# ZhenlongYuan/TSAR-MVS

Measured on AMD Instinct MI355X. Metric: depthmap Mpixels/sec (ETH3D full-res, 8 iters), higher is better.
Workload: dtype f32

## Files before the change

include/tsar.h:

```cpp
#ifndef TSAR_H_
#define TSAR_H_

#include <stddef.h>
#include <stdint.h>

#ifdef __cplusplus
extern "C" {
#endif

#define TSAR_MAX_VIEWS 64
#define TSAR_MAXCOST 2.0f

#define TSAR_OK 0
#define TSAR_ERR_INVALID (-1)
#define TSAR_ERR_HIP (-2)
#define TSAR_ERR_STATE (-3)
#define TSAR_ERR_NOMEM (-4)

#define TSAR_MEM_HOST 0
#define TSAR_MEM_DEVICE 1

#define TSAR_COMB_ALL 0
#define TSAR_COMB_BEST_N 1
#define TSAR_COMB_ANGLE 2
#define TSAR_COMB_GOOD 3

#define TSAR_FLAG_FIX_DOWN_FAR_SEED  (1u << 0)
#define TSAR_FLAG_FIX_RIGHT_FAR_CMP  (1u << 1)
#define TSAR_FLAG_STRICT_DIV         (1u << 2)
#define TSAR_FLAG_NO_LINE_CLOSING    (1u << 4)

#define TSAR_FLAG_TEX_FILTER_8BIT    (1u << 5)

#define TSAR_FLAG_FIX_INIT_RADIUS     (1u << 6)

typedef struct tsar_ctx tsar_ctx;

typedef struct tsar_camera {
    float K[9];
    float R[9];
    float t[3];
} tsar_camera;

typedef struct tsar_params {
    int32_t box_hsize;
    int32_t box_vsize;
    int32_t n_best;
    int32_t cost_comb;
    float depth_min;
    float depth_max;
    float cam_scale;
    uint32_t flags;
    uint64_t seed;
} tsar_params;

typedef struct tsar_slic_settings {
    int32_t spixel_size;
    int32_t no_iters;
    float coh_weight;
    int32_t do_enforce_connectivity;
    int32_t color_space;
} tsar_slic_settings;

typedef struct tsar_kernel_timing {
    char name[48];
    int32_t launches;
    float total_ms;
} tsar_kernel_timing;

int tsar_create(int device, tsar_ctx** out);
int tsar_destroy(tsar_ctx* ctx);
const char* tsar_last_error(const tsar_ctx* ctx);
const char* tsar_version(void);
int tsar_get_stream(tsar_ctx* ctx, void** stream_out);
int tsar_synchronize(tsar_ctx* ctx);

void tsar_default_params(tsar_params* p);
int tsar_set_params(tsar_ctx* ctx, const tsar_params* p);
int tsar_set_views(tsar_ctx* ctx, int n_views, int w, int h, const float* const* gray, int mem,
                   const tsar_camera* cams);
int tsar_set_views_u8(tsar_ctx* ctx, int n_views, int w, int h, const uint8_t* const* gray, int mem,
                      const tsar_camera* cams);
int tsar_set_view_subset(tsar_ctx* ctx, int n, const int32_t* view_idx);

int tsar_pm_init(tsar_ctx* ctx);
int tsar_pm_iterate(tsar_ctx* ctx, int iters);
int tsar_pm_iterate_final(tsar_ctx* ctx, int iters, const float* text, int mem);
int tsar_pm_cost_planes(tsar_ctx* ctx, const float* planes, int mem, float* cost_out,
                        int32_t* beview_out, float* ratio_out);
int tsar_set_plane(tsar_ctx* ctx, const float* planes, const float* cost, int mem);
int tsar_pm_sweep(tsar_ctx* ctx, int colour, int do_prop, int do_refine);
int tsar_set_sweep_counter(tsar_ctx* ctx, int n);
int tsar_get_plane(tsar_ctx* ctx, float* planes, float* cost, int32_t* beview, float* ratio, int mem);

int tsar_load_planes(tsar_ctx* ctx, const float* depth, const float* normal_world, int mem);
int tsar_compute_disp(tsar_ctx* ctx);
int tsar_compute_disp_final(tsar_ctx* ctx, const float* resize_planes, const float* text, int mem);
int tsar_depth_to_plane(tsar_ctx* ctx);

int tsar_pyramid_views(tsar_ctx* coarse, const tsar_ctx* fine);
int tsar_upsample_planes(tsar_ctx* fine, const tsar_ctx* coarse);
int tsar_compute_disp_final_upsampled(tsar_ctx* ctx, const float* text, int mem);
int tsar_get_view_image(tsar_ctx* ctx, int view, float* out, int mem);

int tsar_set_geom_depths(tsar_ctx* ctx, int n_views, const float* const* depth, int mem, float weight, float clip);
int tsar_clear_geom(tsar_ctx* ctx);
int tsar_pm_rescore(tsar_ctx* ctx);
int tsar_get_geom_matrices(tsar_ctx* ctx, int view, float* forward, float* back);

int tsar_geom_pyramid(tsar_ctx* coarse, const tsar_ctx* fine);
int tsar_pyramid_planes(tsar_ctx* coarse, const tsar_ctx* fine);
int tsar_upsample_merge(tsar_ctx* fine, const tsar_ctx* coarse);

int tsar_get_result(tsar_ctx* ctx, float* depth, float* normal_world, float* cost, float* confid,
                    int mem);

int tsar_set_reliable_mask(tsar_ctx* ctx, const float* scale, int mem);
int tsar_get_reliable_mask(tsar_ctx* ctx, float* scale, int mem);
int tsar_lrdiff(tsar_ctx* ctx);
int tsar_getview(tsar_ctx* ctx);
int tsar_wmf(tsar_ctx* ctx, int iters, int final_pass);
int tsar_set_regions(tsar_ctx* ctx, const int32_t* labels, int n_regions, const float* region_text,
                     const float* region_size, int mem);
int tsar_detect_weak_texture(tsar_ctx* ctx, int32_t* labels_out, int mem, int* n_regions_out, float* text_out,
                             float* size_out, int cap);
int tsar_ransac_regions(tsar_ctx* ctx, float* region_planes_out, float* inlier_ratio_out);
int tsar_set_region_planes(tsar_ctx* ctx, const float* region_planes);
int tsar_fake_depth(tsar_ctx* ctx, float* fakedepth_out, int mem);
int tsar_fill_textureless(tsar_ctx* ctx);

void tsar_default_slic_settings(tsar_slic_settings* s);
int tsar_slic(tsar_ctx* ctx, const uint8_t* bgra, int w, int h, const tsar_slic_settings* s,
              int32_t* labels_out, int mem);

typedef struct tsar_fusion_params {
    int32_t num_consistent;
    float reproj_error;
    float depth_diff;
    float angle_deg;
    int32_t used_list;
} tsar_fusion_params;
void tsar_default_fusion_params(tsar_fusion_params* p);
int tsar_fuse_ctx(tsar_ctx* ctx, int n_views, int w, int h, const tsar_camera* cams, const float* const* depth,
                  const float* const* normal_world, const float* const* gray, int mem, const int32_t* src_off,
                  const int32_t* src_idx, const tsar_fusion_params* params, float* points_out, int64_t cap,
                  int64_t* n_points_out);
int tsar_fuse(int device, int n_views, int w, int h, const tsar_camera* cams, const float* const* depth,
              const float* const* normal_world, const float* const* gray, int mem, const int32_t* src_off,
              const int32_t* src_idx, const tsar_fusion_params* params, float* points_out, int64_t cap,
              int64_t* n_points_out);

void* tsar_host_alloc(size_t bytes);
void tsar_host_free(void* p);

void* tsar_device_alloc(int device, size_t bytes);
void tsar_device_free(int device, void* p);
int tsar_device_write(int device, void* dst, const void* host_src, size_t bytes);
int tsar_peer_copy(int dst_device, void* dst, int src_device, const void* src, size_t bytes);

int tsar_enable_kernel_timing(tsar_ctx* ctx, int enable);
int tsar_reset_kernel_timing(tsar_ctx* ctx);
int tsar_get_kernel_timing(tsar_ctx* ctx, tsar_kernel_timing* out, int cap, int* n_out);

int tsar_selftest_sqrt(tsar_ctx* ctx, int mode, uint64_t seed, uint64_t* mismatches_out);
int tsar_selftest_divide(tsar_ctx* ctx, const float* X, const float* Y, const float* Z, size_t n, float* u_out, float* v_out, int ieee);
int tsar_selftest_divide_random(tsar_ctx* ctx, int log2_triples, uint64_t seed, int mode, int guarded, uint64_t* mismatches_out,
                                uint64_t* outside_guard_out);
int tsar_selftest_sweep_census(tsar_ctx* ctx, int colour, uint64_t* out8);
int tsar_selftest_sweep_repeat(tsar_ctx* ctx, int colour, void* memo_dev, uint64_t* out8);
int tsar_selftest_slic_stage(tsar_ctx* ctx, int stage, int w, int h, int mw, int mh, const tsar_slic_settings* s, const void* in0,
                             const void* in1, void* inout);

#ifdef __cplusplus
}
#endif
#endif
```

tsar-mvs_amd/api.py:

```python
from __future__ import annotations

import ctypes as C
import os

import numpy as np

_HERE = os.path.dirname(os.path.abspath(__file__))
LIB_PATH = os.environ.get("TSAR_LIB") or os.path.join(_HERE, "libtsar_hip.so")

TSAR_OK = 0
TSAR_ERR_INVALID, TSAR_ERR_HIP, TSAR_ERR_STATE, TSAR_ERR_NOMEM = -1, -2, -3, -4
MEM_HOST, MEM_DEVICE = 0, 1
COMB_ALL, COMB_BEST_N, COMB_ANGLE, COMB_GOOD = 0, 1, 2, 3
FLAG_FIX_DOWN_FAR_SEED, FLAG_FIX_RIGHT_FAR_CMP, FLAG_STRICT_DIV = 1, 2, 4
FLAG_NO_LINE_CLOSING = 16
FLAG_TEX_FILTER_8BIT = 32
FLAG_FIX_INIT_RADIUS = 64
MAXCOST = 2.0
MAX_VIEWS = 64


class TsarError(RuntimeError):
    def __init__(self, code, msg):
        super().__init__(f"tsar error {code}: {msg}")
        self.code = code


class Camera(C.Structure):
    _fields_ = [("K", C.c_float * 9), ("R", C.c_float * 9), ("t", C.c_float * 3)]


class Params(C.Structure):
    _fields_ = [("box_hsize", C.c_int32), ("box_vsize", C.c_int32), ("n_best", C.c_int32), ("cost_comb", C.c_int32),
                ("depth_min", C.c_float), ("depth_max", C.c_float), ("cam_scale", C.c_float), ("flags", C.c_uint32),
                ("seed", C.c_uint64)]


class SlicSettings(C.Structure):
    _fields_ = [("spixel_size", C.c_int32), ("no_iters", C.c_int32), ("coh_weight", C.c_float),
                ("do_enforce_connectivity", C.c_int32), ("color_space", C.c_int32)]


class FusionParams(C.Structure):
    _fields_ = [("num_consistent", C.c_int32), ("reproj_error", C.c_float), ("depth_diff", C.c_float), ("angle_deg", C.c_float),
                ("used_list", C.c_int32)]


class KernelTiming(C.Structure):
    _fields_ = [("name", C.c_char * 48), ("launches", C.c_int32), ("total_ms", C.c_float)]


SPIXEL_DTYPE = np.dtype([("center", np.float32, 2), ("color", np.float32, 4), ("id", np.int32), ("n", np.int32)])

ABI_SYMBOLS = [
    "tsar_create", "tsar_destroy", "tsar_last_error", "tsar_version", "tsar_get_stream", "tsar_synchronize",
    "tsar_default_params", "tsar_set_params", "tsar_set_views", "tsar_set_views_u8", "tsar_set_view_subset",
    "tsar_pm_init", "tsar_pm_iterate", "tsar_pm_iterate_final", "tsar_pm_sweep", "tsar_set_sweep_counter", "tsar_pm_cost_planes", "tsar_set_plane", "tsar_get_plane",
    "tsar_load_planes", "tsar_compute_disp", "tsar_compute_disp_final", "tsar_depth_to_plane", "tsar_get_result",
    "tsar_pyramid_views", "tsar_upsample_planes", "tsar_compute_disp_final_upsampled", "tsar_get_view_image",
    "tsar_set_geom_depths", "tsar_clear_geom", "tsar_pm_rescore", "tsar_get_geom_matrices",
    "tsar_geom_pyramid", "tsar_pyramid_planes", "tsar_upsample_merge",
    "tsar_set_reliable_mask", "tsar_get_reliable_mask", "tsar_lrdiff", "tsar_getview", "tsar_wmf", "tsar_set_regions", "tsar_detect_weak_texture", "tsar_ransac_regions",
    "tsar_set_region_planes", "tsar_fake_depth", "tsar_fill_textureless",
    "tsar_default_slic_settings", "tsar_slic", "tsar_default_fusion_params", "tsar_fuse", "tsar_fuse_ctx",
    "tsar_host_alloc", "tsar_host_free", "tsar_device_alloc", "tsar_device_free", "tsar_device_write", "tsar_peer_copy", "tsar_enable_kernel_timing", "tsar_reset_kernel_timing", "tsar_get_kernel_timing",
    "tsar_selftest_divide", "tsar_selftest_divide_random", "tsar_selftest_sqrt", "tsar_selftest_sweep_census", "tsar_selftest_sweep_repeat", "tsar_selftest_slic_stage",
]

_lib = None


def load_library(path: str = LIB_PATH):
    global _lib
    if _lib is not None:
        return _lib
    if not os.path.exists(path):
        raise ImportError(f"{path} not found: build it with `make -C tsar-mvs_amd/csrc` "
                          "(or __graft_entry__.build()); there is no CPU fallback")
    L = C.CDLL(path)
    L.tsar_last_error.restype = C.c_char_p
    L.tsar_last_error.argtypes = [C.c_void_p]
    L.tsar_version.restype = C.c_char_p
    L.tsar_create.argtypes = [C.c_int, C.POINTER(C.c_void_p)]
    L.tsar_destroy.argtypes = [C.c_void_p]
    L.tsar_default_params.restype = None
    L.tsar_default_params.argtypes = [C.POINTER(Params)]
    L.tsar_default_slic_settings.restype = None
    L.tsar_default_slic_settings.argtypes = [C.POINTER(SlicSettings)]
    L.tsar_set_params.argtypes = [C.c_void_p, C.POINTER(Params)]
    L.tsar_set_views.argtypes = [C.c_void_p, C.c_int, C.c_int, C.c_int, C.POINTER(C.c_void_p), C.c_int, C.POINTER(Camera)]
    L.tsar_set_views_u8.argtypes = L.tsar_set_views.argtypes
    L.tsar_set_view_subset.argtypes = [C.c_void_p, C.c_int, C.c_void_p]
    L.tsar_pm_init.argtypes = [C.c_void_p]
    L.tsar_pm_iterate.argtypes = [C.c_void_p, C.c_int]
    L.tsar_pm_iterate_final.argtypes = [C.c_void_p, C.c_int, C.c_void_p, C.c_int]
    L.tsar_pm_sweep.argtypes = [C.c_void_p, C.c_int, C.c_int, C.c_int]
    L.tsar_set_sweep_counter.argtypes = [C.c_void_p, C.c_int]
    L.tsar_pm_cost_planes.argtypes = [C.c_void_p, C.c_void_p, C.c_int, C.c_void_p, C.c_void_p, C.c_void_p]
    L.tsar_set_plane.argtypes = [C.c_void_p, C.c_void_p, C.c_void_p, C.c_int]
    L.tsar_get_plane.argtypes = [C.c_void_p, C.c_void_p, C.c_void_p, C.c_void_p, C.c_void_p, C.c_int]
    L.tsar_load_planes.argtypes = [C.c_void_p, C.c_void_p, C.c_void_p, C.c_int]
    L.tsar_compute_disp.argtypes = [C.c_void_p]
    L.tsar_compute_disp_final.argtypes = [C.c_void_p, C.c_void_p, C.c_void_p, C.c_int]
    L.tsar_depth_to_plane.argtypes = [C.c_void_p]
    L.tsar_pyramid_views.argtypes = [C.c_void_p, C.c_void_p]
    L.tsar_upsample_planes.argtypes = [C.c_void_p, C.c_void_p]
    L.tsar_compute_disp_final_upsampled.argtypes = [C.c_void_p, C.c_void_p, C.c_int]
    L.tsar_get_view_image.argtypes = [C.c_void_p, C.c_int, C.c_void_p, C.c_int]
    L.tsar_set_geom_depths.argtypes = [C.c_void_p, C.c_int, C.POINTER(C.c_void_p), C.c_int, C.c_float, C.c_float]
    L.tsar_clear_geom.argtypes = [C.c_void_p]
    L.tsar_pm_rescore.argtypes = [C.c_void_p]
    L.tsar_get_geom_matrices.argtypes = [C.c_void_p, C.c_int, C.c_void_p, C.c_void_p]
    L.tsar_geom_pyramid.argtypes = [C.c_void_p, C.c_void_p]
    L.tsar_pyramid_planes.argtypes = [C.c_void_p, C.c_void_p]
    L.tsar_upsample_merge.argtypes = [C.c_void_p, C.c_void_p]
    L.tsar_get_result.argtypes = [C.c_void_p, C.c_void_p, C.c_void_p, C.c_void_p, C.c_void_p, C.c_int]
    L.tsar_set_reliable_mask.argtypes = [C.c_void_p, C.c_void_p, C.c_int]
    L.tsar_get_reliable_mask.argtypes = [C.c_void_p, C.c_void_p, C.c_int]
    L.tsar_host_alloc.restype = C.c_void_p
    L.tsar_host_alloc.argtypes = [C.c_size_t]
    L.tsar_host_free.restype = None
    L.tsar_host_free.argtypes = [C.c_void_p]
    L.tsar_device_alloc.restype = C.c_void_p
    L.tsar_device_alloc.argtypes = [C.c_int, C.c_size_t]
    L.tsar_device_free.restype = None
    L.tsar_device_free.argtypes = [C.c_int, C.c_void_p]
    L.tsar_device_write.argtypes = [C.c_int, C.c_void_p, C.c_void_p, C.c_size_t]
    L.tsar_peer_copy.argtypes = [C.c_int, C.c_void_p, C.c_int, C.c_void_p, C.c_size_t]
    L.tsar_lrdiff.argtypes = [C.c_void_p]
    L.tsar_getview.argtypes = [C.c_void_p]
    L.tsar_wmf.argtypes = [C.c_void_p, C.c_int, C.c_int]
    L.tsar_set_regions.argtypes = [C.c_void_p, C.c_void_p, C.c_int, C.c_void_p, C.c_void_p, C.c_int]
    L.tsar_detect_weak_texture.argtypes = [C.c_void_p, C.c_void_p, C.c_int, C.POINTER(C.c_int), C.c_void_p, C.c_void_p, C.c_int]
    L.tsar_ransac_regions.argtypes = [C.c_void_p, C.c_void_p, C.c_void_p]
    L.tsar_set_region_planes.argtypes = [C.c_void_p, C.c_void_p]
    L.tsar_fake_depth.argtypes = [C.c_void_p, C.c_void_p, C.c_int]
    L.tsar_fill_textureless.argtypes = [C.c_void_p]
    L.tsar_slic.argtypes = [C.c_void_p, C.c_void_p, C.c_int, C.c_int, C.POINTER(SlicSettings), C.c_void_p, C.c_int]
    L.tsar_default_fusion_params.restype = None
    L.tsar_default_fusion_params.argtypes = [C.POINTER(FusionParams)]
    L.tsar_fuse.argtypes = [C.c_int, C.c_int, C.c_int, C.c_int, C.POINTER(Camera), C.POINTER(C.c_void_p), C.POINTER(C.c_void_p), C.POINTER(C.c_void_p), C.c_int,
                            C.c_void_p, C.c_void_p, C.POINTER(FusionParams), C.c_void_p, C.c_int64, C.POINTER(C.c_int64)]
    L.tsar_fuse_ctx.argtypes = [C.c_void_p] + list(L.tsar_fuse.argtypes[1:])
    L.tsar_get_stream.argtypes = [C.c_void_p, C.POINTER(C.c_void_p)]
    L.tsar_synchronize.argtypes = [C.c_void_p]
    L.tsar_enable_kernel_timing.argtypes = [C.c_void_p, C.c_int]
    L.tsar_reset_kernel_timing.argtypes = [C.c_void_p]
    L.tsar_get_kernel_timing.argtypes = [C.c_void_p, C.POINTER(KernelTiming), C.c_int, C.POINTER(C.c_int)]
    L.tsar_selftest_divide.argtypes = [C.c_void_p, C.c_void_p, C.c_void_p, C.c_void_p, C.c_size_t, C.c_void_p, C.c_void_p, C.c_int]
    L.tsar_selftest_sweep_census.argtypes = [C.c_void_p, C.c_int, C.POINTER(C.c_uint64)]
    L.tsar_selftest_sweep_repeat.argtypes = [C.c_void_p, C.c_int, C.c_void_p, C.POINTER(C.c_uint64)]
    L.tsar_selftest_sqrt.argtypes = [C.c_void_p, C.c_int, C.c_uint64, C.POINTER(C.c_uint64)]
    L.tsar_selftest_divide_random.argtypes = [C.c_void_p, C.c_int, C.c_uint64, C.c_int, C.c_int, C.POINTER(C.c_uint64), C.POINTER(C.c_uint64)]
    L.tsar_selftest_slic_stage.argtypes = [C.c_void_p, C.c_int, C.c_int, C.c_int, C.c_int, C.c_int, C.POINTER(SlicSettings), C.c_void_p, C.c_void_p, C.c_void_p]
    _lib = L
    return L


def default_params(**kw) -> Params:
    p = Params()
    load_library().tsar_default_params(C.byref(p))
    for k, v in kw.items():
        setattr(p, k, v)
    return p


def _is_torch(a) -> bool:
    return type(a).__module__.startswith("torch")


def _ptr(a):
    if a is None:
        return None, MEM_HOST
    if _is_torch(a):
        assert a.is_contiguous(), "tensor must be contiguous"
        if a.is_cuda:
            import torch
            torch.cuda.current_stream(a.device).synchronize()
        return C.c_void_p(a.data_ptr()), (MEM_DEVICE if a.is_cuda else MEM_HOST)
    assert a.flags["C_CONTIGUOUS"], "array must be C-contiguous"
    return a.ctypes.data_as(C.c_void_p), MEM_HOST


class Matcher:

    def __init__(self, device: int = 0):
        self.L = load_library()
        self._ctx = C.c_void_p()
        rc = self.L.tsar_create(device, C.byref(self._ctx))
        if rc != TSAR_OK:
            raise TsarError(rc, "tsar_create failed (is a HIP device visible?)")
        self.w = self.h = self.n_views = 0
        self.device = device
        self._keep = []

    def close(self):
        if self._ctx:
            self.L.tsar_destroy(self._ctx)
            self._ctx = C.c_void_p()

    def __del__(self):
        try:
            self.close()
        except Exception:
            pass

    def _chk(self, rc):
        if rc != TSAR_OK:
            raise TsarError(rc, self.L.tsar_last_error(self._ctx).decode())

    def set_params(self, params: Params):
        self._chk(self.L.tsar_set_params(self._ctx, C.byref(params)))
        self.params = params

    def set_views(self, images, K, R, t, u8: bool = False):
        n = len(images)
        first = images[0]
        h, w = int(first.shape[0]), int(first.shape[1])
        ptrs = (C.c_void_p * n)()
        kinds = set()
        for i, im in enumerate(images):
            assert tuple(im.shape) == (h, w)
            if not _is_torch(im):
                im = np.ascontiguousarray(im, dtype=np.uint8 if u8 else np.float32)
                self._keep.append(im)
            elif u8:
                assert str(im.dtype) == "torch.uint8" and im.is_contiguous()
            p, kind = _ptr(im)
            ptrs[i] = p
            kinds.add(kind)
        assert len(kinds) == 1, "all images must live in the same memory space"
        cams = (Camera * n)()
        K = np.asarray(K, np.float32).reshape(n, 9)
        R = np.asarray(R, np.float32).reshape(n, 9)
        t = np.asarray(t, np.float32).reshape(n, 3)
        for i in range(n):
            cams[i].K[:] = K[i].tolist()
            cams[i].R[:] = R[i].tolist()
            cams[i].t[:] = t[i].tolist()
        self._chk((self.L.tsar_set_views_u8 if u8 else self.L.tsar_set_views)(self._ctx, n, w, h, ptrs, kinds.pop(), cams))
        self._keep.clear()
        self.w, self.h, self.n_views = w, h, n

    def set_view_subset(self, idx):
        a = np.ascontiguousarray(idx, np.int32)
        self._chk(self.L.tsar_set_view_subset(self._ctx, len(a), a.ctypes.data_as(C.c_void_p)))

    def pm_init(self):
        self._chk(self.L.tsar_pm_init(self._ctx))

    def pm_iterate(self, iters: int):
        self._chk(self.L.tsar_pm_iterate(self._ctx, iters))

    def pm_iterate_final(self, iters: int, text):
        t = text if _is_torch(text) else np.ascontiguousarray(text, np.float32)
        p, kind = _ptr(t)
        self._chk(self.L.tsar_pm_iterate_final(self._ctx, iters, p, kind))

    def pm_sweep(self, colour: int, do_prop: bool = True, do_refine: bool = True):
        self._chk(self.L.tsar_pm_sweep(self._ctx, colour, int(do_prop), int(do_refine)))

    def set_sweep_counter(self, n: int):
        self._chk(self.L.tsar_set_sweep_counter(self._ctx, n))

    def pm_cost_planes(self, planes):
        planes = np.ascontiguousarray(planes, np.float32)
        cost = np.empty((self.h, self.w), np.float32)
        bv = np.empty((self.h, self.w), np.int32)
        rt = np.empty((self.h, self.w), np.float32)
        self._chk(self.L.tsar_pm_cost_planes(self._ctx, _ptr(planes)[0], MEM_HOST, _ptr(cost)[0], _ptr(bv)[0], _ptr(rt)[0]))
        return cost, bv, rt

    def set_plane(self, planes, cost):
        planes = np.ascontiguousarray(planes, np.float32)
        cost = np.ascontiguousarray(cost, np.float32)
        self._chk(self.L.tsar_set_plane(self._ctx, _ptr(planes)[0], _ptr(cost)[0], MEM_HOST))

    def get_plane(self):
        planes = np.empty((self.h, self.w, 4), np.float32)
        cost = np.empty((self.h, self.w), np.float32)
        bv = np.empty((self.h, self.w), np.int32)
        rt = np.empty((self.h, self.w), np.float32)
        self._chk(self.L.tsar_get_plane(self._ctx, _ptr(planes)[0], _ptr(cost)[0], _ptr(bv)[0], _ptr(rt)[0], MEM_HOST))
        return planes, cost, bv, rt

    def load_planes(self, depth, normal_world):
        d, kd = _ptr(depth if _is_torch(depth) else np.ascontiguousarray(depth, np.float32))
        depth_keep = depth if _is_torch(depth) else np.ascontiguousarray(depth, np.float32)
        normal_keep = normal_world if _is_torch(normal_world) else np.ascontiguousarray(normal_world, np.float32)
        d, kd = _ptr(depth_keep)
        n, kn = _ptr(normal_keep)
        assert kd == kn
        self._chk(self.L.tsar_load_planes(self._ctx, d, n, kd))

    def compute_disp(self):
        self._chk(self.L.tsar_compute_disp(self._ctx))

    def compute_disp_final(self, resize_planes, text):
        r = np.ascontiguousarray(resize_planes, np.float32)
        t = np.ascontiguousarray(text, np.float32)
        self._chk(self.L.tsar_compute_disp_final(self._ctx, _ptr(r)[0], _ptr(t)[0], MEM_HOST))

    def depth_to_plane(self):
        self._chk(self.L.tsar_depth_to_plane(self._ctx))

    def pyramid_from(self, fine: "Matcher"):
        self._chk(self.L.tsar_pyramid_views(self._ctx, fine._ctx))
        self.w, self.h, self.n_views = (fine.w + 1) // 2, (fine.h + 1) // 2, fine.n_views
        self.params = fine.params

    def upsample_planes(self, coarse: "Matcher"):
        self._chk(self.L.tsar_upsample_planes(self._ctx, coarse._ctx))

    def get_view_image(self, view: int):
        out = np.empty((self.h, self.w), np.float32)
        self._chk(self.L.tsar_get_view_image(self._ctx, view, _ptr(out)[0], MEM_HOST))
        return out

    def compute_disp_final_upsampled(self, text):
        t = text if _is_torch(text) else np.ascontiguousarray(text, np.float32)
        p, kind = _ptr(t)
        self._chk(self.L.tsar_compute_disp_final_upsampled(self._ctx, p, kind))

    def set_geom_depths(self, depths, weight: float = 0.2, clip: float = 3.0):
        n = len(depths)
        ptrs = (C.c_void_p * n)()
        keep, kinds = [], set()
        for v, d in enumerate(depths):
            if v == 0 or d is None:
                continue
            if not _is_torch(d):
                d = np.ascontiguousarray(d, np.float32)
            assert tuple(d.shape) == (self.h, self.w), "depth map %d has shape %s, the views are %dx%d" % (v, tuple(d.shape), self.w, self.h)
            keep.append(d)
            p, kind = _ptr(d)
            ptrs[v] = p
            kinds.add(kind)
        assert len(kinds) <= 1, "all depth maps must live in the same memory space"
        self._chk(self.L.tsar_set_geom_depths(self._ctx, n, ptrs, kinds.pop() if kinds else MEM_HOST, float(weight), float(clip)))

    def clear_geom(self):
        self._chk(self.L.tsar_clear_geom(self._ctx))

    def rescore(self):
        self._chk(self.L.tsar_pm_rescore(self._ctx))

    def get_geom_matrices(self, view: int):
        f = np.empty((3, 4), np.float32)
        b = np.empty((3, 4), np.float32)
        self._chk(self.L.tsar_get_geom_matrices(self._ctx, view, _ptr(f)[0], _ptr(b)[0]))
        return f, b

    def geom_pyramid_from(self, fine: "Matcher"):
        self._chk(self.L.tsar_geom_pyramid(self._ctx, fine._ctx))

    def pyramid_planes_from(self, fine: "Matcher"):
        self._chk(self.L.tsar_pyramid_planes(self._ctx, fine._ctx))

    def upsample_merge(self, coarse: "Matcher"):
        self._chk(self.L.tsar_upsample_merge(self._ctx, coarse._ctx))

    def get_result(self, want=("depth", "normal", "cost", "confid"), pinned=False, out=None):
        shapes = {"depth": (self.h, self.w), "normal": (self.h, self.w, 3), "cost": (self.h, self.w), "confid": (self.h, self.w)}
        empty = pinned_empty if pinned else np.empty
        res = {}
        for k in ("depth", "normal", "cost", "confid"):
            if out is not None and k in out:
                a = out[k]
                assert a.dtype == np.float32 and tuple(a.shape) == shapes[k] and a.flags["C_CONTIGUOUS"]
                res[k] = a
            elif out is None and k in want:
                res[k] = empty(shapes[k], np.float32)
        self._chk(self.L.tsar_get_result(self._ctx, _ptr(res.get("depth"))[0], _ptr(res.get("normal"))[0], _ptr(res.get("cost"))[0],
                                         _ptr(res.get("confid"))[0], MEM_HOST))
        return res

    def get_result_device(self, depth=None, normal=None, cost=None, confid=None):
        self._chk(self.L.tsar_get_result(self._ctx, _ptr(depth)[0], _ptr(normal)[0], _ptr(cost)[0], _ptr(confid)[0], MEM_DEVICE))

    def set_reliable_mask(self, scale):
        s = np.ascontiguousarray(scale, np.float32)
        self._chk(self.L.tsar_set_reliable_mask(self._ctx, _ptr(s)[0], MEM_HOST))

    def get_reliable_mask(self):
        s = np.empty((self.h, self.w), np.float32)
        self._chk(self.L.tsar_get_reliable_mask(self._ctx, _ptr(s)[0], MEM_HOST))
        return s

    def lrdiff(self):
        self._chk(self.L.tsar_lrdiff(self._ctx))

    def selftest_divide(self, X, Y, Z, ieee: bool = False, mode: int | None = None):
        X, Y, Z = (np.ascontiguousarray(a, dtype=np.float32) for a in (X, Y, Z))
        assert X.shape == Y.shape == Z.shape
        u, v = np.empty_like(X), np.empty_like(X)
        self._chk(self.L.tsar_selftest_divide(self._ctx, _ptr(X)[0], _ptr(Y)[0], _ptr(Z)[0], X.size, _ptr(u)[0], _ptr(v)[0], int(ieee) if mode is None else mode))
        return u, v

    def selftest_sqrt(self, mode: int, seed: int = 0) -> int:
        bad = C.c_uint64(0)
        self._chk(self.L.tsar_selftest_sqrt(self._ctx, mode, seed, C.byref(bad)))
        return bad.value

    def selftest_sweep_census(self, colour: int) -> dict:
        out = (C.c_uint64 * 8)()
        self._chk(self.L.tsar_selftest_sweep_census(self._ctx, colour, out))
        keys = ("waves", "arms_any_lane", "max_lane_survivors", "max_lane_survivors_nodup", "lane_survivors", "lane_survivors_nodup", "pixels", "arms_present")
        return dict(zip(keys, [int(v) for v in out]))

    def selftest_divide_random(self, log2_triples: int, seed: int, mode: int, guarded: bool = True):
        bad, out = C.c_uint64(0), C.c_uint64(0)
        self._chk(self.L.tsar_selftest_divide_random(self._ctx, log2_triples, seed, mode, int(guarded), C.byref(bad), C.byref(out)))
        return bad.value, out.value

    def _slic_stage(self, stage, w, h, mw, mh, settings, in0, in1, inout):
        p1 = _ptr(in1)[0] if in1 is not None else None
        self._chk(self.L.tsar_selftest_slic_stage(self._ctx, stage, w, h, mw, mh, C.byref(settings), _ptr(in0)[0], p1, _ptr(inout)[0]))
        return inout

    def slic_convert(self, bgra, color_space=0):
        img = np.ascontiguousarray(bgra, np.uint8).reshape(-1, 4)
        return self._slic_stage(0, img.shape[0], 1, 0, 0, SlicSettings(20, 0, 5.0, 0, color_space), img, None, np.zeros((img.shape[0], 4), np.float32))

    def slic_init_centers(self, lab, mw, mh, S):
        lab = np.ascontiguousarray(lab, np.float32)
        h, w = lab.shape[:2]
        return self._slic_stage(1, w, h, mw, mh, SlicSettings(S, 0, 5.0, 0, 0), lab, None, np.zeros(mw * mh, SPIXEL_DTYPE))

    def slic_find_association(self, lab, centres, mw, mh, S, weight, labels_before=None):
        lab = np.ascontiguousarray(lab, np.float32)
        h, w = lab.shape[:2]
        labels = np.zeros((h, w), np.int32) if labels_before is None else np.ascontiguousarray(labels_before, np.int32).copy()
        return self._slic_stage(2, w, h, mw, mh, SlicSettings(S, 0, weight, 0, 0), lab, np.ascontiguousarray(centres), labels)

    def slic_update_centers(self, lab, labels, S):
        lab = np.ascontiguousarray(lab, np.float32)
        h, w = lab.shape[:2]
        return self._slic_stage(3, w, h, w // S, h // S, SlicSettings(S, 0, 5.0, 0, 0), lab, np.ascontiguousarray(labels, np.int32), np.zeros((w // S) * (h // S), SPIXEL_DTYPE))

    def slic_connectivity(self, labels):
        labels = np.ascontiguousarray(labels, np.int32)
        h, w = labels.shape
        return self._slic_stage(4, w, h, 0, 0, SlicSettings(20, 0, 5.0, 0, 0), labels, None, np.zeros((h, w), np.int32))

    def getview(self):
        self._chk(self.L.tsar_getview(self._ctx))

    def wmf(self, iters: int, final_pass: bool):
        self._chk(self.L.tsar_wmf(self._ctx, iters, int(final_pass)))

    def set_regions(self, labels, region_text, region_size=None):
        tx = np.ascontiguousarray(region_text, np.float32)
        sz = np.ascontiguousarray(region_size, np.float32) if region_size is not None else None
        if _is_torch(labels) and labels.is_cuda:
            import torch
            assert labels.dtype == torch.int32
            txd = torch.from_numpy(tx).to(labels.device)
            szd = torch.from_numpy(sz).to(labels.device) if sz is not None else None
            self._chk(self.L.tsar_set_regions(self._ctx, _ptr(labels)[0], len(tx), _ptr(txd)[0], _ptr(szd)[0], MEM_DEVICE))
        else:
            lb = np.ascontiguousarray(labels, np.int32)
            self._chk(self.L.tsar_set_regions(self._ctx, _ptr(lb)[0], len(tx), _ptr(tx)[0], _ptr(sz)[0], MEM_HOST))
        self.n_regions = len(tx)

    def detect_weak_texture(self, cap: int = 1 << 16, want_labels: bool = True):
        labels = np.empty((self.h, self.w), np.int32) if want_labels else None
        text = np.empty(cap, np.float32)
        size = np.empty(cap, np.float32)
        n = C.c_int(0)
        self._chk(self.L.tsar_detect_weak_texture(self._ctx, _ptr(labels)[0] if want_labels else None, MEM_HOST, C.byref(n), _ptr(text)[0], _ptr(size)[0], cap))
        self.n_regions = n.value
        k = min(n.value, cap)
        return labels, text[:k].copy(), size[:k].copy()

    def ransac_regions(self):
        planes = np.empty((self.n_regions, 4), np.float32)
        ratio = np.empty((self.n_regions,), np.float32)
        self._chk(self.L.tsar_ransac_regions(self._ctx, _ptr(planes)[0], _ptr(ratio)[0]))
        return planes, ratio

    def set_region_planes(self, planes):
        pl = np.ascontiguousarray(planes, np.float32)
        self._chk(self.L.tsar_set_region_planes(self._ctx, _ptr(pl)[0]))

    def fake_depth(self):
        out = np.empty((self.h, self.w), np.float32)
        self._chk(self.L.tsar_fake_depth(self._ctx, _ptr(out)[0], MEM_HOST))
        return out

    def fill_textureless(self):
        self._chk(self.L.tsar_fill_textureless(self._ctx))

    def slic(self, bgra, settings: SlicSettings | None = None):
        img = np.ascontiguousarray(bgra, np.uint8)
        h, w = img.shape[:2]
        if settings is None:
            settings = SlicSettings()
            self.L.tsar_default_slic_settings(C.byref(settings))
        labels = np.empty((h, w), np.int32)
        self._chk(self.L.tsar_slic(self._ctx, _ptr(img)[0], w, h, C.byref(settings), _ptr(labels)[0], MEM_HOST))
        return labels

    @property
    def stream(self) -> int:
        s = C.c_void_p()
        self._chk(self.L.tsar_get_stream(self._ctx, C.byref(s)))
        return s.value or 0

    def synchronize(self):
        self._chk(self.L.tsar_synchronize(self._ctx))

    def enable_kernel_timing(self, on: bool = True):
        self._chk(self.L.tsar_enable_kernel_timing(self._ctx, int(on)))

    def reset_kernel_timing(self):
        self._chk(self.L.tsar_reset_kernel_timing(self._ctx))

    def kernel_timing(self):
        buf = (KernelTiming * 32)()
        n = C.c_int(0)
        self._chk(self.L.tsar_get_kernel_timing(self._ctx, buf, 32, C.byref(n)))
        return {buf[i].name.decode(): (buf[i].launches, buf[i].total_ms) for i in range(min(n.value, 32))}


def matcher_from_scene(scene, box=11, n_best=1, cost_comb=COMB_BEST_N, flags=0, seed=2024, device=0, subset=None, box_v=None) -> Matcher:
    m = Matcher(device)
    m.set_params(default_params(box_hsize=box, box_vsize=box if box_v is None else box_v, n_best=n_best, cost_comb=cost_comb, depth_min=scene.depth_min,
                                depth_max=scene.depth_max, flags=flags, seed=seed))
    m.set_views(scene.images, scene.K, scene.R, scene.t)
    if subset is not None:
        m.set_view_subset(subset)
    return m


def run_multiscale(matcher: Matcher, levels: int, coarse_iters: int, fine_iters: int, coarse=None):
    if levels < 0 or coarse_iters < 0 or fine_iters < 0:
        raise ValueError("levels and iteration counts must be >= 0")
    coarse = list(coarse or [])
    while len(coarse) < levels:
        coarse.append(Matcher(matcher.device))
    chain = [matcher] + coarse[:levels]
    for finer, coarser in zip(chain[:-1], chain[1:]):
        coarser.pyramid_from(finer)
    chain[-1].pm_init()
    chain[-1].pm_iterate(coarse_iters)
    for k in range(levels - 1, -1, -1):
        chain[k].upsample_planes(chain[k + 1])
        chain[k].pm_iterate(fine_iters)
    return coarse


def run_geom_pass(matcher: Matcher, own_depth, own_normal_world, src_depths, iters: int, weight: float = 0.2, clip: float = 3.0):
    if iters < 0:
        raise ValueError("iters must be >= 0")
    matcher.load_planes(own_depth, own_normal_world)
    matcher.set_geom_depths(src_depths, weight=weight, clip=clip)
    matcher.rescore()
    matcher.pm_iterate(iters)
    matcher.compute_disp()


def run_geom_pass_multiscale(matcher: Matcher, own_depth, own_normal_world, src_depths, levels: int, coarse_iters: int, fine_iters: int,
                             weight: float = 0.2, clip: float = 3.0, coarse=None):
    if levels < 0 or coarse_iters < 0 or fine_iters < 0:
        raise ValueError("levels and iteration counts must be >= 0")
    if levels == 0:
        run_geom_pass(matcher, own_depth, own_normal_world, src_depths, fine_iters, weight=weight, clip=clip)
        return list(coarse or [])
    coarse = list(coarse or [])
    while len(coarse) < levels:
        coarse.append(Matcher(matcher.device))
    chain = [matcher] + coarse[:levels]
    for m in chain:
        m.clear_geom()
    for finer, coarser in zip(chain[:-1], chain[1:]):
        coarser.pyramid_from(finer)
    matcher.load_planes(own_depth, own_normal_world)
    matcher.set_geom_depths(src_depths, weight=weight, clip=clip)
    for finer, coarser in zip(chain[:-1], chain[1:]):
        coarser.geom_pyramid_from(finer)
        coarser.pyramid_planes_from(finer)
    chain[-1].pm_iterate(coarse_iters)
    for k in range(levels - 1, -1, -1):
        chain[k].upsample_merge(chain[k + 1])
        chain[k].pm_iterate(fine_iters)
    matcher.compute_disp()
    return coarse


def fuse(depths, normals, grays, K, R, t, pairs, params: FusionParams | None = None, cap: int | None = None, device: int = 0, matcher=None):
    L = load_library()
    n = len(depths)
    h, w = int(depths[0].shape[0]), int(depths[0].shape[1])
    if params is None:
        params = FusionParams()
        L.tsar_default_fusion_params(C.byref(params))
    keep, kinds = [], set()

    def ptrs(seq, shape):
        arr = (C.c_void_p * n)()
        for i, a in enumerate(seq):
            if not _is_torch(a):
                a = np.ascontiguousarray(a, np.float32)
                keep.append(a)
            assert tuple(a.shape) == shape
            p, kind = _ptr(a)
            arr[i] = p
            kinds.add(kind)
        return arr
    pd, pn, pg = ptrs(depths, (h, w)), ptrs(normals, (h, w, 3)), ptrs(grays, (h, w))
    assert len(kinds) == 1
    cams = (Camera * n)()
    K = np.asarray(K, np.float32).reshape(n, 9); R = np.asarray(R, np.float32).reshape(n, 9); t = np.asarray(t, np.float32).reshape(n, 3)
    for i in range(n):
        cams[i].K[:] = K[i].tolist(); cams[i].R[:] = R[i].tolist(); cams[i].t[:] = t[i].tolist()
    lists = [list(pairs[v]) for v in range(n)]
    off = np.zeros(n + 1, np.int32)
    off[1:] = np.cumsum([len(x) for x in lists])
    idx = np.asarray([s for x in lists for s in x] or [0], np.int32)
    if cap is None:
        cap = n * h * w
    out = np.empty((cap, 9), np.float32)
    cnt = C.c_int64(0)
    tail = (n, w, h, cams, pd, pn, pg, kinds.pop(), off.ctypes.data_as(C.c_void_p), idx.ctypes.data_as(C.c_void_p), C.byref(params),
            out.ctypes.data_as(C.c_void_p), cap, C.byref(cnt))
    rc = L.tsar_fuse_ctx(matcher._ctx, *tail) if matcher is not None else L.tsar_fuse(device, *tail)
    if rc != TSAR_OK:
        raise TsarError(rc, L.tsar_last_error(matcher._ctx).decode() if matcher is not None else "tsar_fuse failed")
    return out[: min(cnt.value, cap)].copy()


def pinned_empty(shape, dtype=np.float32):
    import weakref
    L = load_library()
    dt = np.dtype(dtype)
    n = int(np.prod(shape)) * dt.itemsize
    p = L.tsar_host_alloc(n)
    if not p:
        raise MemoryError(f"tsar_host_alloc({n}) failed")
    buf = (C.c_char * n).from_address(p)
    weakref.finalize(buf, L.tsar_host_free, p)
    return np.frombuffer(buf, dtype=dt).reshape(shape)
```

tsar-mvs_amd/csrc/pm_core.h:

```cpp
#pragma once
#include <type_traits>

#include "tsar_device_math.h"

#define PM_BLOCK 256
#define PM_RW 32

typedef const uint32_t __attribute__((address_space(1)))* global_u32_ptr;
typedef const float __attribute__((address_space(1)))* global_f32_ptr;

template <bool QUAD, bool DIFF = false>
DEVFN float sample_bilinear(const DevView& vw, int w, int h, int qpitch, float u, float v, bool q8 = false) {
    u = fminf(fmaxf(u, -1.0f), (float)w);
    v = fminf(fmaxf(v, -1.0f), (float)h);
    const float fu = floorf(u), fv = floorf(v);
    float ax = u - fu, ay = v - fv;
    if (q8) { ax = rintf(ax * 256.0f) * 0.00390625f; ay = rintf(ay * 256.0f) * 0.00390625f; }
    const int iu = (int)fu, iv = (int)fv;
    float t00, t10, t01, t11;
    if (QUAD) {
        const uint32_t off = (uint32_t)(__mul24(iv + 1, qpitch) + iu + 1) * 4u;
        const uint32_t q = *(global_u32_ptr)((const char __attribute__((address_space(1)))*)vw.quad + off);
        t00 = (float)(q & 0xffu);
        t10 = (float)((q >> 8) & 0xffu);
        t01 = (float)((q >> 16) & 0xffu);
        t11 = (float)(q >> 24);
    } else {
        const int x0 = min(max(iu, 0), w - 1), x1 = min(max(iu + 1, 0), w - 1);
        const int y0 = min(max(iv, 0), h - 1), y1 = min(max(iv + 1, 0), h - 1);
        const global_f32_ptr r0 = (global_f32_ptr)vw.img + (size_t)y0 * w;
        const global_f32_ptr r1 = (global_f32_ptr)vw.img + (size_t)y1 * w;
        t00 = r0[x0]; t10 = r0[x1]; t01 = r1[x0]; t11 = r1[x1];
    }
    if (DIFF) {
        const float d1 = t10 - t00, d2 = t01 - t00, d3 = (t11 - t01) - d1;
        return fma_(ay, fma_(ax, d3, d2), fma_(ax, d1, t00));
    }
    const float top = fma_(ax, t10 - t00, t00);
    const float bot = fma_(ax, t11 - t01, t01);
    return fma_(ay, bot - top, top);
}

struct PixelRef {
    float inv_wsum;
    float mean_ref;
    float var_ref;
    bool textured;
};

template <bool QUAD> struct TileOf { typedef float type; };
template <> struct TileOf<true> { typedef unsigned short type; };
DEVFN float tile_value(float t) { return t; }
DEVFN float tile_value(unsigned short t) { return __uint_as_float((uint32_t)t << 16); }
DEVFN void tile_store(float* t, float v) { *t = v; }
DEVFN void tile_store(unsigned short* t, float v) { *t = (unsigned short)(__float_as_uint(v) >> 16); }
template <bool QUAD>
__host__ __device__ constexpr size_t tile_bytes(int tw, int th) {
    return ((size_t)tw * th * sizeof(typename TileOf<QUAD>::type) + 15) & ~(size_t)15;
}

template <int RH, typename TileT, int BLK = PM_BLOCK, int RW = PM_RW>
DEVFN void stage_ref_tile(const DevScene* __restrict__ sc, TileT* tile, int x0, int y0, int hr, int vr, int pad_rows = 0) {
    const int tw = RW + 2 * hr, th = RH + 2 * vr + pad_rows;
    const global_f32_ptr img = (global_f32_ptr)sc->view[0].img;
    const int w = sc->w, h = sc->h;
    for (int k = threadIdx.x; k < tw * th; k += BLK) {
        const int ty = k / tw, tx = k - ty * tw;
        const int gx = min(max(x0 + tx - hr, 0), w - 1), gy = min(max(y0 + ty - vr, 0), h - 1);
        tile_store(&tile[k], img[(size_t)gy * w + gx]);
    }
}

template <int HR, typename TileT, int BLK = PM_BLOCK>
DEVFN PixelRef hoist_reference(const TileT* tile, int tw, int own, float* wts, int hr_rt, int vr_rt) {
    const int hr = HR > 0 ? HR : hr_rt, vr = HR > 0 ? HR : vr_rt;
    const float cen = tile_value(tile[own]);
    float sum_ref = 0.f, sum_ref_ref = 0.f, wsum = 0.f;
    int tap = 0;
#pragma unroll
    for (int i = -hr; i <= hr; i += 2) {
#pragma unroll
        for (int j = -vr; j <= vr; j += 2) {
            const float r = tile_value(tile[own + j * tw + i]);
            const float sd = sqrtf((float)(i * i + j * j));
            const float cd = fabsf(r - cen);
            const float wt = tsar_expf(-sd / 50.0f - cd / 18.0f);
            wts[tap * BLK] = wt;
            const float wr = wt * r;
            sum_ref += wr;
            sum_ref_ref = fma_(wr, r, sum_ref_ref);
            wsum += wt;
            ++tap;
        }
    }
    PixelRef pr;
    pr.inv_wsum = 1.0f / wsum;
    sum_ref *= pr.inv_wsum;
    sum_ref_ref *= pr.inv_wsum;
    pr.mean_ref = sum_ref;
    pr.var_ref = sum_ref_ref - sum_ref * sum_ref;
    pr.textured = !(pr.var_ref < 1e-5f);
    return pr;
}

template <int HR, bool STRICT, bool QUAD, int BLK = PM_BLOCK>
DEVFN float view_cost_generic(const DevScene* __restrict__ sc, const DevView& vw, const typename TileOf<QUAD>::type* tile, int tw, int own, const float* wts,
                              const PixelRef& pr, int x, int y, const float4& n4) {
    const int hr = HR > 0 ? HR : sc->hrad, vr = HR > 0 ? HR : sc->vrad;
    const int w = sc->w, h = sc->h, qp = sc->quad_pitch;
    float H[9];
    if (STRICT) plane_homography(sc->ref, vw, n4, H, sc->k_sparse != 0);
    else plane_homography_fast(sc->ref, vw, n4, H);
    float sum_src = 0.f, sum_src_src = 0.f, sum_ref_src = 0.f;
    int tap = 0;
#pragma unroll 1
    for (int i = -hr; i <= hr; i += 2) {
        const float xi = (float)(x + i);
        const float bx = STRICT ? H[0] * xi : fma_(H[0], xi, H[2]), by = STRICT ? H[3] * xi : fma_(H[3], xi, H[5]), bz = STRICT ? H[6] * xi : fma_(H[6], xi, H[8]);
#pragma unroll
        for (int j = -vr; j <= vr; j += 2) {
            const float yj = (float)(y + j);
            float X = fma_(H[1], yj, bx), Y = fma_(H[4], yj, by), Z = fma_(H[7], yj, bz);
            if (STRICT) { X += H[2]; Y += H[5]; Z += H[8]; }
            float u, v;
            if (STRICT) {
                persp_divide_exact<true>(X, Y, Z, u, v);
            } else {
                const float rz = __builtin_amdgcn_rcpf(Z);
                u = X * rz;
                v = Y * rz;
            }
            const float s = sample_bilinear<QUAD, !STRICT>(vw, w, h, qp, u, v, (sc->flags & TSAR_FLAG_TEX_FILTER_8BIT) != 0);
            const float r = tile_value(tile[own + j * tw + i]);
            const float wt = wts[tap * BLK];
            const float ws = wt * s;
            sum_src += ws;
            sum_src_src = fma_(ws, s, sum_src_src);
            if (STRICT) sum_ref_src = fma_(wt * r, s, sum_ref_src);
            else sum_ref_src = fma_(ws, r, sum_ref_src);
            ++tap;
        }
    }
    sum_src *= pr.inv_wsum;
    sum_src_src *= pr.inv_wsum;
    sum_ref_src *= pr.inv_wsum;
    const float var_src = sum_src_src - sum_src * sum_src;
    if (var_src < 1e-5f) return TSAR_MAXCOST;
    const float covar = sum_ref_src - pr.mean_ref * sum_src;
    const float vrs = sqrtf(pr.var_ref * var_src);
    return fmaxf(0.0f, fminf(TSAR_MAXCOST, 1.0f - covar / vrs));
}

#include "pm_tap_r5.h"
#include "pm_core_lut.h"

DEVFN float geom_term(const DevScene* __restrict__ sc, const DevView& vw, int vi, int x, int y, float D) {
    const float* dm = sc->geom_depth[vi];
    if (dm == nullptr) return 0.0f;
    const int w = sc->w, h = sc->h;
    const float xf = (float)x, yf = (float)y;
    const float xd = xf * D, yd = yf * D;
    const float a = ((vw.A[0] * xd + vw.A[1] * yd) + vw.A[2] * D) + vw.b[0];
    const float b = ((vw.A[3] * xd + vw.A[4] * yd) + vw.A[5] * D) + vw.b[1];
    const float s = ((vw.A[6] * xd + vw.A[7] * yd) + vw.A[8] * D) + vw.b[2];
    float u, v;
    persp_divide_exact<true>(a, b, s, u, v);
    const float cf = floorf(u + 0.5f), rf = floorf(v + 0.5f);
    const bool inside = s > 0.0f && cf >= 0.0f && cf <= (float)(w - 1) && rf >= 0.0f && rf <= (float)(h - 1);
    float Dv = 0.0f;
    if (inside) Dv = ((global_f32_ptr)dm)[(int)rf * w + (int)cf];
    const float* M = sc->geom_back[vi];
    const float cd = cf * Dv, rd = rf * Dv;
    const float p0 = ((M[0] * cd + M[1] * rd) + M[2] * Dv) + M[3];
    const float p1 = ((M[4] * cd + M[5] * rd) + M[6] * Dv) + M[7];
    const float p2 = ((M[8] * cd + M[9] * rd) + M[10] * Dv) + M[11];
    float xq, yq;
    persp_divide_exact<true>(p0, p1, p2, xq, yq);
    const float dx = xq - xf, dy = yq - yf;
    const float e2 = dx * dx + dy * dy;
    const float tau = sc->geom_clip;
    const float r = sqrt_rsq_exact(fminf(fmaxf(e2, 0x1p-100f), 0x1p100f));
    float e = e2 < 0x1p-100f ? 0.0f : r;
    e = (inside && Dv > 0.0f && p2 > 0.0f && e2 < sc->geom_clip_sq) ? fminf(e, tau) : tau;
    return sc->geom_weight * e;
}

template <int NB, int HR, bool STRICT, bool QUAD, int V = 0, int BLK = PM_BLOCK>
DEVFN float multiview_cost(const DevScene* __restrict__ sc, const typename TileOf<QUAD>::type* tile, int tw, int own, const float* wts, const PixelRef& pr,
                           int x, int y, const float4& n4, int& beview, float& ratio) {
    constexpr bool GEOM = (V & TSAR_V_GEOM) != 0;
    constexpr int VT = V & ~(TSAR_V_GEOM | TSAR_V_REDRAW);
    float best[NB];
#pragma unroll
    for (int k = 0; k < NB; k++) best[k] = __builtin_inff();
    const int num = sc->n_sel;
    int valid = 0, bv = -1;
    float cmin = __builtin_inff();
    float depth_h = 0.0f;
    if constexpr (GEOM) depth_h = plane_depth(sc->ref, n4, x, y);
    int vi_next = sc->sel[0];
    for (int i = 0; i < num; i++) {
        const int vi = vi_next;
        vi_next = sc->sel[i + 1 < num ? i + 1 : i];
        float c;
        if constexpr ((VT & 1024) != 0) c = view_cost_lut<STRICT, (VT >> 11) & 7, (VT & 131072) != 0 && !STRICT, (VT & 2097152) != 0 && !STRICT>(sc, sc->view[vi], tile, tw, own, wts, pr, x, y, n4);
        else if constexpr (QUAD && HR == 5 && r5_production_variant(VT))
            c = view_cost_r5<STRICT, (VT & 128) != 0 && !STRICT, (VT & 8) != 0, (VT & 131072) != 0, (VT & 2097152) != 0, BLK>(sc, sc->view[vi], tile, tw, own, wts, pr, x, y, n4);
#ifdef TSAR_EXPERIMENTS
        else if constexpr (QUAD && HR == 5 && r5_diag_variant(VT))
            c = view_cost_r5<false, true, true, true, true, BLK, (VT & 4194304) ? 1 : 2>(sc, sc->view[vi], tile, tw, own, wts, pr, x, y, n4);
#endif
        else {
            static_assert(VT == 0, "unknown tap-loop variant");
            c = view_cost_generic<HR, STRICT, QUAD, BLK>(sc, sc->view[vi], tile, tw, own, wts, pr, x, y, n4);
        }
        auto vmin = [](float a, float b) { float r; asm("v_min_f32 %0, %1, %2" : "=v"(r) : "v"(a), "v"(b)); return r; };
        auto vmax = [](float a, float b) { float r; asm("v_max_f32 %0, %1, %2" : "=v"(r) : "v"(a), "v"(b)); return r; };
        c = vmin(c, TSAR_MAXCOST);
        valid -= (int32_t)__float_as_uint(c - TSAR_MAXCOST) >> 31;
        if constexpr (GEOM) c = c + geom_term(sc, sc->view[vi], vi, x, y, depth_h);
        {
            const uint32_t worse = (uint32_t)((int32_t)__float_as_uint(cmin - c) >> 31);
            asm("v_bfi_b32 %0, %1, %2, %3" : "=v"(bv) : "v"(worse), "v"(bv), "s"(vi));
            cmin = vmin(cmin, c);
        }
        float v = c;
#pragma unroll
        for (int k = 0; k < NB; k++) {
            const float lo = vmin(best[k], v), hi = vmax(best[k], v);
            best[k] = lo;
            v = hi;
        }
    }
    int nb = valid;
    if (sc->cost_comb == TSAR_COMB_BEST_N) nb = min(nb, sc->n_best);
    if (nb <= 0) { beview = -1; ratio = 0.f; return TSAR_MAXCOST; }
    float cost = 0.f;
#pragma unroll
    for (int k = 0; k < NB; k++)
        if (k < nb) cost += best[k];
    cost = cost / (float)nb;
    ratio = num >= 2 ? best[0] / best[1] : 0.f;
    beview = bv;
    return cost;
}

DEVFN void strip_tile(int t, int tiles_x, int tiles_y, int sw, int& tx, int& ty) {
    if (sw <= 0) { ty = t / tiles_x; tx = t - ty * tiles_x; return; }
    const int per_strip = sw * tiles_y;
    const int strip = t / per_strip, within = t - strip * per_strip;
    const int width = min(sw, tiles_x - strip * sw);
    ty = within / width;
    tx = strip * sw + within - ty * width;
}

static inline int strip_width(int requested, int tiles_x) {
    if (requested >= 0) return requested;
    const int sw = (tiles_x + 7) / 8;
    return sw < 8 ? 8 : sw;
}

DEVFN int xcd_tile(int bid, int n) {
    const int chunk = n >> 3, rem = n & 7;
    const int xcd = bid & 7, slot = bid >> 3;
    return xcd * chunk + min(xcd, rem) + slot;
}
```

tsar-mvs_amd/csrc/pm_sweep_impl.h:

```cpp
#pragma once
#include "pm_core.h"

#define SWEEP_SMALL_IMAGE_TILES 3072

#define CAND_SAME (1 << 30)

DEVFN void select_candidates(const DevScene* __restrict__ sc, const float* __restrict__ c_same, const float* __restrict__ c_other,
                             int x, int y, int cand[8]) {
    const int col = sc->w, row = sc->h;
    const int p = y * col + x;
    const bool fix_seed = sc->flags & TSAR_FLAG_FIX_DOWN_FAR_SEED, fix_cmp = sc->flags & TSAR_FLAG_FIX_RIGHT_FAR_CMP;
    float cmin;
    int cp, cs;
#pragma unroll
    for (int k = 0; k < 8; k++) cand[k] = -1;
    if (y > 2) {
        cp = p - 3 * col; cmin = c_other[cp];
#pragma unroll
        for (int i = 1; i < 11; ++i)
            if (y > 2 + 2 * i) { const int q = p - (3 + 2 * i) * col; const float v = c_other[q]; if (v < cmin) { cmin = v; cp = q; } }
        cand[0] = cp;
    }
    if (y < row - 3) {
        cp = p + 3 * col;
        cmin = (fix_seed || y <= 2) ? c_other[cp] : c_other[p - 3 * col];
#pragma unroll
        for (int i = 1; i < 11; ++i)
            if (y < row - 3 - 2 * i) { const int q = p + (3 + 2 * i) * col; const float v = c_other[q]; if (v < cmin) { cmin = v; cp = q; } }
        cand[1] = cp;
    }
    if (x > 2) {
        cp = p - 3; cmin = c_other[cp];
#pragma unroll
        for (int i = 1; i < 11; ++i)
            if (x > 2 + 2 * i) { const int q = p - 3 - 2 * i; const float v = c_other[q]; if (v < cmin) { cmin = v; cp = q; } }
        cand[2] = cp;
    }
    if (x < col - 3) {
        cp = p + 3; cmin = c_other[cp];
#pragma unroll
        for (int i = 1; i < 11; ++i)
            if (x < col - 3 - 2 * i) {
                const int q = p + 3 + 2 * i;
                const float v = c_other[q];
                const bool take = fix_cmp ? (v < cmin) : (cmin < v);
                if (take) { cmin = v; cp = q; }
            }
        cand[3] = cp;
    }
    if (y > 0) {
        cp = p - col; cs = 0; cmin = c_other[cp];
#pragma unroll
        for (int i = 0; i < 3; ++i) {
            if (y > 1 + i && x > i) { const int q = p - (2 + i) * col - i; const float v = c_same[q]; if (v < cmin) { cmin = v; cp = q; cs = 1; } }
            if (y > 1 + i && x < col - 1 - i) { const int q = p - (2 + i) * col + i; const float v = c_same[q]; if (v < cmin) { cmin = v; cp = q; cs = 1; } }
        }
        cand[4] = cs ? (cp | CAND_SAME) : cp;
    }
    if (y < row - 1) {
        cp = p + col; cs = 0; cmin = c_other[cp];
#pragma unroll
        for (int i = 0; i < 3; ++i) {
            if (y < row - 2 - i && x > i) { const int q = p + (2 + i) * col - i; const float v = c_same[q]; if (v < cmin) { cmin = v; cp = q; cs = 1; } }
            if (y < row - 2 - i && x < col - 1 - i) { const int q = p + (2 + i) * col + i; const float v = c_same[q]; if (v < cmin) { cmin = v; cp = q; cs = 1; } }
        }
        cand[5] = cs ? (cp | CAND_SAME) : cp;
    }
    if (x > 0) {
        cp = p - 1; cs = 0; cmin = c_other[cp];
#pragma unroll
        for (int i = 0; i < 3; ++i) {
            if (x > 1 + i && y > i) { const int q = p - (2 + i) - i * col; const float v = c_same[q]; if (v < cmin) { cmin = v; cp = q; cs = 1; } }
            if (x > 1 + i && y < row - 1 - i) { const int q = p - (2 + i) + i * col; const float v = c_same[q]; if (v < cmin) { cmin = v; cp = q; cs = 1; } }
        }
        cand[6] = cs ? (cp | CAND_SAME) : cp;
    }
    if (x < col - 1) {
        cp = p + 1; cs = 0; cmin = c_other[cp];
#pragma unroll
        for (int i = 0; i < 3; ++i) {
            if (x < col - 2 - i && y > i) { const int q = p + (2 + i) - i * col; const float v = c_same[q]; if (v < cmin) { cmin = v; cp = q; cs = 1; } }
            if (x < col - 2 - i && y < row - 1 - i) { const int q = p + (2 + i) + i * col; const float v = c_same[q]; if (v < cmin) { cmin = v; cp = q; cs = 1; } }
        }
        cand[7] = cs ? (cp | CAND_SAME) : cp;
    }
}

DEVFN bool same_bits(const float4& a, const float4& b) {
    return __float_as_uint(a.x) == __float_as_uint(b.x) && __float_as_uint(a.y) == __float_as_uint(b.y) &&
           __float_as_uint(a.z) == __float_as_uint(b.z) && __float_as_uint(a.w) == __float_as_uint(b.w);
}

struct SweepMemo {
    int32_t* cand;
    uint32_t* seq;
    uint32_t* changed;
    uint32_t launch, valid_from;
    int mode;
    int slot_off;
};

template <int NB, int HR, bool STRICT, bool QUAD, int V = 0, int BLK = PM_BLOCK, bool CMP = false>
__global__ __launch_bounds__(BLK) void pm_sweep_kernel(const DevScene* __restrict__ sc, int colour,
                                                            const float* __restrict__ c_same, const float4* __restrict__ n_same,
                                                            const float* __restrict__ c_other, const float4* __restrict__ n_other,
                                                            float* c_out, float4* n_out, float* __restrict__ ratio_out,
                                                            int32_t* __restrict__ beview_out, uint32_t stream_id, int do_prop,
                                                            int do_refine, int tiles_x, int n_tiles, int cost_consistent, int strip_w,
                                                            const float* __restrict__ final_text, SweepMemo memo) {
    extern __shared__ __attribute__((aligned(16))) unsigned char lds_raw[];
    typedef typename TileOf<QUAD>::type TileT;
    constexpr int RW = PM_RW;
    constexpr int SWEEP_RH = 2 * BLK / RW;
    const int hr = HR > 0 ? HR : sc->hrad, vr = HR > 0 ? HR : sc->vrad;
    const int tw = RW + 2 * hr, th = SWEEP_RH + 2 * vr;
    constexpr bool LUTW = (V & 1024) != 0;
    const size_t lut_bytes = LUTW ? (size_t)(sc->lut_classes + 1) * 1024 : 0;
    TileT* tile = (TileT*)(lds_raw + lut_bytes);
    float* const wts_base = LUTW ? (float*)lds_raw : (float*)(lds_raw + tile_bytes<QUAD>(tw, th));
    float* wts = LUTW ? wts_base : wts_base + threadIdx.x;
    if constexpr (LUTW) build_weight_lut<BLK>(sc, wts);

    const int t = xcd_tile(blockIdx.x, n_tiles);
    int tix, tiy;
    strip_tile(t, tiles_x, n_tiles / tiles_x, strip_w, tix, tiy);
    const int ty0 = tiy * SWEEP_RH, tx0 = tix * RW;
    stage_ref_tile<SWEEP_RH, TileT, BLK, RW>(sc, tile, tx0, ty0, hr, vr, LUTW ? LUT_TILE_PAD_ROWS : 0);
    __syncthreads();

    const int ly = threadIdx.x >> 4, k = threadIdx.x & 15;
    const int y = ty0 + ly;
    const int lx = 2 * k + ((colour + y) & 1);
    const int x = tx0 + lx;
    const int w = sc->w, h = sc->h;
    bool mine = x < w && y < h;
    if (!CMP && !mine) return;
    const int p = mine ? y * w + x : 0;
    const int own = (ly + vr) * tw + lx + hr;

    float cost_now = TSAR_MAXCOST;
    float4 n_now = {0.f, 0.f, 0.f, 0.f};
    if (mine) { cost_now = c_same[p]; n_now = n_same[p]; }
    if (mine && final_text && final_text[p] == -1.0f) {
        c_out[p] = cost_now; n_out[p] = n_now;
        if (!CMP) return;
        mine = false;
    }
    PixelRef pr;
    pr.inv_wsum = 0.f; pr.mean_ref = 0.f; pr.var_ref = 0.f; pr.textured = false;
    if (mine) {
        if constexpr (LUTW) pr = hoist_reference_lut(sc, tile, tw, own, wts);
        else pr = hoist_reference<HR, TileT, BLK>(tile, tw, own, wts, hr, vr);
    }
    bool wrote = false;
    float ratio_w = 0.f;
    int beview_w = 0;
    const DevRef& rf = sc->ref;
    const bool work = mine && pr.textured;
    int cand[8] = {-1, -1, -1, -1, -1, -1, -1, -1};
    if (work && do_prop) {
        select_candidates(sc, c_same, c_other, x, y, cand);
        if (memo.mode) {
            const uint32_t m_seq = memo.seq[p];
            const bool have = m_seq >= memo.valid_from && cost_consistent;
            const int4* mc = (const int4*)(memo.cand + (size_t)p * 8);
            int prev[8];
            if (have) {
                const int4 a0 = mc[0], a1 = mc[1];
                prev[0] = a0.x; prev[1] = a0.y; prev[2] = a0.z; prev[3] = a0.w; prev[4] = a1.x; prev[5] = a1.y; prev[6] = a1.z; prev[7] = a1.w;
            }
            int4 w0, w1;
            w0.x = cand[0]; w0.y = cand[1]; w0.z = cand[2]; w0.w = cand[3]; w1.x = cand[4]; w1.y = cand[5]; w1.z = cand[6]; w1.w = cand[7];
            ((int4*)(memo.cand + (size_t)p * 8))[0] = w0;
            ((int4*)(memo.cand + (size_t)p * 8))[1] = w1;
            memo.seq[p] = memo.launch;
            if (have) {
#pragma unroll
                for (int a = 0; a < 8; a++)
                    if (cand[a] >= 0 && cand[a] == prev[a] && memo.changed[cand[a] & 0x3fffffff] < m_seq) cand[a] = -1;
            }
        }
    }
    float depth_now = 0.f;
    float vv[3] = {0.f, 0.f, 0.f};
    if (work) { depth_now = plane_depth(rf, n_now, x, y); view_vector(rf, x, y, vv); }
    const float4 n_first = n_now;
    float deltaN = 1.0f;
    float deltaZ = sc->max_disp / 2.0f;
    const float fb = rf.f * rf.baseline;
    const int n_ref = do_refine ? sc->refine_steps : 0;

    if constexpr (!CMP) {
        if (work) {
            const int h_end = 8 + n_ref;
#pragma unroll 1
            for (int h = do_prop ? 0 : 8; h < h_end; h++) {
                float4 n_t;
                float depth_t;
                if (h < 8) {
                    int ci = cand[0];
#pragma unroll
                    for (int a = 1; a < 8; a++) ci = (h == a) ? cand[a] : ci;
                    if (ci < 0) continue;
                    const int idx = ci & 0x3fffffff;
                    n_t = (ci >> 30) ? n_same[idx] : n_other[idx];
                    if (cost_consistent && (same_bits(n_t, n_now) || same_bits(n_t, n_first))) continue;
                    depth_t = plane_depth(rf, n_t, x, y);
                    if (!(depth_t >= rf.depthMin && depth_t <= rf.depthMax)) continue;
                } else {
                    const Rand4 rn = philox_uniform4((uint32_t)p, stream_id, (uint32_t)(h - 8), sc->seed_lo, sc->seed_hi);
                    const float disp = fb / depth_now;
                    const float minDelta = -fminf(deltaZ, sc->min_disp + disp);
                    const float maxDelta = fminf(deltaZ, sc->max_disp - disp);
                    const float dz = between(rn.u[0], minDelta, maxDelta);
                    const float dispOut = fminf(fmaxf(disp + dz, sc->min_disp), sc->max_disp);
                    depth_t = fb / dispOut;
                    float nt[3];
                    nt[0] = n_now.x + between(rn.u[1], -deltaN, deltaN);
                    nt[1] = n_now.y + between(rn.u[2], -deltaN, deltaN);
                    nt[2] = n_now.z + between(rn.u[3], -deltaN, deltaN);
                    const float inv = 1.0f / sqrtf(dot3(nt, nt));
                    nt[0] *= inv; nt[1] *= inv; nt[2] *= inv;
                    if (dot3(nt, vv) > 0.0f) { nt[0] = -nt[0]; nt[1] = -nt[1]; nt[2] = -nt[2]; }
                    n_t.x = nt[0]; n_t.y = nt[1]; n_t.z = nt[2];
                    n_t.w = plane_offset(rf, nt, x, y, depth_t);
                    deltaN = deltaN / 4.0f;
                    deltaZ = deltaZ / 10.0f;
                }
                int bv; float rt;
                const float cost_t = multiview_cost<NB, HR, STRICT, QUAD, V, BLK>(sc, tile, tw, own, wts, pr, x, y, n_t, bv, rt);
                if (cost_t < cost_now) {
                    cost_now = cost_t; n_now = n_t; depth_now = depth_t;
                    ratio_w = rt; beview_w = bv; wrote = true;
                }
            }
        }
    } else {
        const int lane = threadIdx.x & 63, wave0 = threadIdx.x & ~63;
        volatile int32_t* slot_ci = (volatile int32_t*)(lds_raw + memo.slot_off) + wave0;
        volatile unsigned short* slot_src = (volatile unsigned short*)(lds_raw + memo.slot_off + 4 * BLK) + wave0;
        auto pixel_of = [&](int tid, int& px, int& py, int& pown) {
            const int sly = tid >> 4, sk = tid & 15;
            py = ty0 + sly;
            const int slx = 2 * sk + ((colour + py) & 1);
            px = tx0 + slx;
            pown = (sly + vr) * tw + slx + hr;
        };
        auto my_tid = []() { int t = threadIdx.x; asm volatile("" : "+v"(t)); return t; };
        uint32_t fresh = 0;
        if (work && do_prop) {
#pragma unroll
            for (int a = 0; a < 8; a++)
                if (cand[a] >= 0) fresh |= 1u << a;
        }
        if (!work) fresh = 0;
        uint32_t flags = fresh | (work ? 256u : 0u) | (mine ? 512u : 0u);
        int total = 0;
#pragma unroll
        for (int a = 0; a < 8; a++) total += __popcll(__ballot((flags >> a) & 1u));
        const int trips = (total + 63) >> 6;
        auto arms_of_trip = [&](int lo, auto&& f) {
            asm volatile("" : "+v"(flags));
            int b0 = 0;
#pragma unroll
            for (int a = 0; a < 8; a++) {
                const uint64_t bal = __ballot((flags >> a) & 1u);
                const int n = __popcll(bal);
                if (b0 + n > lo && b0 < lo + 64) {
                    const int j = b0 + (int)__builtin_amdgcn_mbcnt_hi((uint32_t)(bal >> 32), __builtin_amdgcn_mbcnt_lo((uint32_t)bal, 0u)) - lo;
                    f(a, j, ((flags >> a) & 1u) && j >= 0 && j < 64);
                }
                b0 += n;
            }
        };
        int acc_arm = -1;
        const float start_dz = sc->max_disp / 2.0f;
#pragma unroll 1
        for (int it = 0; it < trips + n_ref; it++) {
            float4 n_t = {0.f, 0.f, 0.f, 0.f};
            float depth_t = 0.f;
            int ex, ey, eown, etid = my_tid();
            PixelRef epr = pr;
            bool go;
            const int lo = it << 6;
            if (it < trips) {
                {
                    int mx, my, mown;
                    pixel_of(my_tid(), mx, my, mown);
                    const int32_t* mc = memo.cand + (size_t)(my * w + mx) * 8;
                    arms_of_trip(lo, [&](int a, int j, bool has) {
                        if (has) { slot_ci[j] = mc[a]; slot_src[j] = (unsigned short)(lane | (a << 6)); }
                    });
                }
                __builtin_amdgcn_wave_barrier();
                go = lane < total - lo;
                int src = 0, ci = 0;
                if (go) { src = slot_src[lane]; ci = slot_ci[lane]; }
                __builtin_amdgcn_wave_barrier();
                const int s = src & 63;
                epr.inv_wsum = __int_as_float(__builtin_amdgcn_ds_bpermute(s << 2, __float_as_int(pr.inv_wsum)));
                epr.mean_ref = __int_as_float(__builtin_amdgcn_ds_bpermute(s << 2, __float_as_int(pr.mean_ref)));
                epr.var_ref = __int_as_float(__builtin_amdgcn_ds_bpermute(s << 2, __float_as_int(pr.var_ref)));
                if (go) {
                    const int idx = ci & 0x3fffffff;
                    n_t = (ci >> 30) ? n_same[idx] : n_other[idx];
                    etid = wave0 + s;
                }
                pixel_of(etid, ex, ey, eown);
                if (go) {
                    const float d = plane_depth(rf, n_t, ex, ey);
                    go = d >= rf.depthMin && d <= rf.depthMax;
                }
            } else {
                pixel_of(etid, ex, ey, eown);
                if (it == trips && acc_arm >= 0) {
                    const int ci = memo.cand[(size_t)(ey * w + ex) * 8 + acc_arm];
                    const int idx = ci & 0x3fffffff;
                    n_now = (ci >> 30) ? n_same[idx] : n_other[idx];
                    depth_now = plane_depth(rf, n_now, ex, ey);
                    acc_arm = -1;
                }
                go = (flags >> 8) & 1u;
                if (go) {
                    const int step = it - trips;
                    float dN = 1.0f, dZ = start_dz;
                    for (int q = 0; q < step; q++) { dN = dN / 4.0f; dZ = dZ / 10.0f; }
                    float ev[3];
                    view_vector(rf, ex, ey, ev);
                    const Rand4 rn = philox_uniform4((uint32_t)(ey * w + ex), stream_id, (uint32_t)step, sc->seed_lo, sc->seed_hi);
                    const float disp = fb / depth_now;
                    const float minDelta = -fminf(dZ, sc->min_disp + disp);
                    const float maxDelta = fminf(dZ, sc->max_disp - disp);
                    const float dz = between(rn.u[0], minDelta, maxDelta);
                    const float dispOut = fminf(fmaxf(disp + dz, sc->min_disp), sc->max_disp);
                    depth_t = fb / dispOut;
                    float nt[3];
                    nt[0] = n_now.x + between(rn.u[1], -dN, dN);
                    nt[1] = n_now.y + between(rn.u[2], -dN, dN);
                    nt[2] = n_now.z + between(rn.u[3], -dN, dN);
                    const float inv = 1.0f / sqrtf(dot3(nt, nt));
                    nt[0] *= inv; nt[1] *= inv; nt[2] *= inv;
                    if (dot3(nt, ev) > 0.0f) { nt[0] = -nt[0]; nt[1] = -nt[1]; nt[2] = -nt[2]; }
                    n_t.x = nt[0]; n_t.y = nt[1]; n_t.z = nt[2];
                    n_t.w = plane_offset(rf, nt, ex, ey, depth_t);
                }
            }
            const float* ewts = LUTW ? wts_base : wts_base + etid;
            int bv = -1;
            float rt = 0.f, cost_t = TSAR_MAXCOST;
            if (go) cost_t = multiview_cost<NB, HR, STRICT, QUAD, V, BLK>(sc, tile, tw, eown, ewts, epr, ex, ey, n_t, bv, rt);
            if (it < trips) {
                arms_of_trip(lo, [&](int a, int j, bool has) {
                    const float c = __int_as_float(__builtin_amdgcn_ds_bpermute((j & 63) << 2, __float_as_int(cost_t)));
                    const float r = __int_as_float(__builtin_amdgcn_ds_bpermute((j & 63) << 2, __float_as_int(rt)));
                    const int b = __builtin_amdgcn_ds_bpermute((j & 63) << 2, bv);
                    if (has && c < cost_now) {
                        cost_now = c; acc_arm = a;
                        ratio_w = r; beview_w = b;
                    }
                });
            } else if (go && cost_t < cost_now) {
                cost_now = cost_t; n_now = n_t; depth_now = depth_t;
                ratio_w = rt; beview_w = bv;
            }
        }
        {
            int mx, my, mown;
            pixel_of(my_tid(), mx, my, mown);
            if (!((flags >> 9) & 1u)) return;
            const int pp = my * w + mx;
            if (acc_arm >= 0) {
                const int ci = memo.cand[(size_t)pp * 8 + acc_arm];
                const int idx = ci & 0x3fffffff;
                n_now = (ci >> 30) ? n_same[idx] : n_other[idx];
            }
            const bool changed = cost_now < c_same[pp];
            c_out[pp] = cost_now;
            n_out[pp] = n_now;
            if (changed && !final_text) { ratio_out[pp] = ratio_w; beview_out[pp] = beview_w; }
            if (changed && memo.mode) memo.changed[pp] = memo.launch;
            return;
        }
    }
    c_out[p] = cost_now;
    n_out[p] = n_now;
    if (wrote && !final_text) { ratio_out[p] = ratio_w; beview_out[p] = beview_w; }
    if (wrote && memo.mode) memo.changed[p] = memo.launch;
}


template <int HR, bool QUAD, int V>
constexpr bool sweep_has_packed_form() { return QUAD && ((HR == 5 && r5_production_variant(V & ~TSAR_V_GEOM)) || (V & 1024) != 0); }

template <int NB, int HR, bool STRICT, bool QUAD, int V = 0, int BLK = PM_BLOCK>
static int launch_sweep_t(tsar_ctx* ctx, int colour, const PlaneBuf& same_in, const PlaneBuf& other, const PlaneBuf& same_out,
                          uint32_t stream_id, int do_prop, int do_refine) {
    const DevScene& hs = ctx->hscene;
    constexpr int RW = PM_RW;
    constexpr int SWEEP_RH = 2 * BLK / RW;
    const int tiles_x = (hs.w + RW - 1) / RW, tiles_y = (hs.h + SWEEP_RH - 1) / SWEEP_RH;
    const int n_tiles = tiles_x * tiles_y;
#ifdef TSAR_EXPERIMENTS
    const size_t lds_pad = ctx->lds_pad;
#else
    constexpr size_t lds_pad = 0;
#endif
    size_t lds = tile_bytes<QUAD>(RW + 2 * hs.hrad, SWEEP_RH + 2 * hs.vrad + ((V & 1024) ? LUT_TILE_PAD_ROWS : 0)) + lds_pad +
                 ((V & 1024) ? (size_t)(hs.lut_classes + 1) * 1024 : sizeof(float) * (size_t)(hs.hrad + 1) * (hs.vrad + 1) * BLK);
    SweepMemo memo;
    memo.cand = ctx->memo_cand; memo.seq = ctx->memo_seq; memo.changed = ctx->changed_seq;
    memo.launch = ctx->launch_seq; memo.valid_from = ctx->memo_valid_from;
    memo.mode = (ctx->memo_mode && ctx->memo_cand && ctx->cost_consistent && !ctx->final_text) ? 1 : 0;
    memo.slot_off = 0;
    bool packed = false;
    if constexpr (sweep_has_packed_form<HR, QUAD, V>())
        packed = memo.mode && do_prop && ctx->compact_from >= 0 && ctx->call_launch >= ctx->compact_from;
    auto kern = pm_sweep_kernel<NB, HR, STRICT, QUAD, V, BLK, false>;
    if constexpr (sweep_has_packed_form<HR, QUAD, V>()) {
        if (packed) {
            kern = pm_sweep_kernel<NB, HR, STRICT, QUAD, V, BLK, true>;
            memo.slot_off = (int)lds;
            lds += 6 * (size_t)BLK;
        }
    }
    if (lds > 64 * 1024) TSAR_HIP_TRY(ctx, hipFuncSetAttribute((const void*)kern, hipFuncAttributeMaxDynamicSharedMemorySize, (int)lds));
    {
        ScopedKernelTimer tm(ctx, (V & TSAR_V_GEOM) ? "pm_sweep_geom" : "pm_sweep");
        ScopedKernelTimer tm_packed(ctx, packed ? "pm_sweep_packed" : nullptr);
        hipLaunchKernelGGL(kern, dim3(n_tiles), dim3(BLK), lds, ctx->stream, ctx->dscene, colour, same_in.c, same_in.n4, other.c,
                           other.n4, same_out.c, same_out.n4, ctx->ratio, ctx->beview, stream_id, do_prop, do_refine, tiles_x, n_tiles,
                           ctx->cost_consistent ? 1 : 0, strip_width(ctx->strip_w, tiles_x), ctx->final_text, memo);
    }
    TSAR_HIP_TRY(ctx, hipGetLastError());
    return TSAR_OK;
}

template <int NB, int HR, bool STRICT, bool QUAD, int V = 0, int BLK = PM_BLOCK>
static int launch_sweep_g(tsar_ctx* ctx, int colour, const PlaneBuf& same_in, const PlaneBuf& other, const PlaneBuf& same_out,
                          uint32_t stream_id, int do_prop, int do_refine) {
    if (ctx->hscene.geom_on) return launch_sweep_t<NB, HR, STRICT, QUAD, V | TSAR_V_GEOM, BLK>(ctx, colour, same_in, other, same_out, stream_id, do_prop, do_refine);
    return launch_sweep_t<NB, HR, STRICT, QUAD, V, BLK>(ctx, colour, same_in, other, same_out, stream_id, do_prop, do_refine);
}
```

tsar-mvs_amd/csrc/pm_tap_r5.h:

```cpp
#pragma once

template <bool STRICT, bool ROW, bool D16, bool BUF, bool MIX, int BLK, int DIAG = 0>
DEVFN float view_cost_r5(const DevScene* __restrict__ sc, const DevView& vw, const unsigned short* tile, int tw, int own, const float* wts,
                         const PixelRef& pr, int x, int y, const float4& n4) {
    static_assert(!(STRICT && ROW), "the row-wise walk changes the summation order: fast mode only");
    static_assert(!MIX || (BUF && !STRICT), "the half-float difference texture serves the fast arithmetic's blend through buffer loads");
    const int w = sc->w, h = sc->h, qp = sc->quad_pitch;
    const int qorg = (qp + 1) << 2;
    float H[9];
    if (STRICT) plane_homography(sc->ref, vw, n4, H, sc->k_sparse != 0);
    else plane_homography_fast(sc->ref, vw, n4, H);
    float sum_src = 0.f, sum_src_src = 0.f, sum_ref_src = 0.f;
    bool need_clamp;
    if (!STRICT) {
        const float xc = (float)x, yc = (float)y;
        const float Xc = fma_(H[1], yc, fma_(H[0], xc, H[2])), Yc = fma_(H[4], yc, fma_(H[3], xc, H[5])), Zc = fma_(H[7], yc, fma_(H[6], xc, H[8]));
        const float a = fabsf(H[0]) + fabsf(H[1]), b = fabsf(H[3]) + fabsf(H[4]), c = fabsf(H[6]) + fabsf(H[7]);
        const float Zmin = fma_(-5.0f, c, Zc);
        const float r = __builtin_amdgcn_rcpf(Zmin * Zc);
        const float r5 = 5.0f * r, rc = Zmin * r;
        const float du = fma_(a, Zc, fabsf(Xc) * c) * r5, dv = fma_(b, Zc, fabsf(Yc) * c) * r5;
        const float uc = Xc * rc, vc = Yc * rc;
        const bool inside = Zmin > 0.0f && fminf(uc - du, vc - dv) >= 1.5f && uc + du <= (float)(w - 1) - 1.5f && vc + dv <= (float)(h - 1) - 1.5f;
        need_clamp = !__all(inside);
    } else {
        bool inside = true;
        float zmin = __builtin_inff(), zmax = 0.0f;
#pragma unroll
        for (int c = 0; c < 4; c++) {
            const float xi = (float)(x + ((c & 1) ? 5 : -5)), yj = (float)(y + ((c & 2) ? 5 : -5));
            const float X = fma_(H[1], yj, fma_(H[0], xi, H[2])), Y = fma_(H[4], yj, fma_(H[3], xi, H[5])), Z = fma_(H[7], yj, fma_(H[6], xi, H[8]));
            const float rz = __builtin_amdgcn_rcpf(Z);
            const float u = X * rz, v = Y * rz;
            inside = inside && Z > 0.0f && u >= 1.0f && u <= (float)(w - 1) - 1.0f && v >= 1.0f && v <= (float)(h - 1) - 1.0f;
            if (STRICT) { zmin = fminf(zmin, Z); zmax = fmaxf(zmax, Z); }
        }
        if (STRICT) {
            const float cm = (float)(max(w, h) + 32);
            const float sz = fma_(fabsf(H[6]) + fabsf(H[7]), cm, fabsf(H[8]));
            const float sx = fma_(fabsf(H[0]) + fabsf(H[1]), cm, fabsf(H[2]));
            const float sy = fma_(fabsf(H[3]) + fabsf(H[4]), cm, fabsf(H[5]));
            inside = inside && zmin >= 3.814697265625e-06f && zmax <= 131072.0f && sz * cm <= 524288.0f * zmin && fmaxf(sx, sy) <= 262144.0f * zmin;
        }
        need_clamp = !__all(inside);
    }
    uint32_t qb_lo = 0, qb_hi = 0;
    if (!BUF) {
        const uint64_t qa = (uint64_t)(uintptr_t)vw.quad + (uint32_t)qorg;
        qb_lo = __builtin_amdgcn_readfirstlane((uint32_t)qa);
        qb_hi = __builtin_amdgcn_readfirstlane((uint32_t)(qa >> 32));
        asm volatile("" : "+s"(qb_lo), "+s"(qb_hi));
    }
    typedef uint32_t u32x4s __attribute__((ext_vector_type(4)));
    u32x4s rsrc = {0u, 0u, 0u, 0u};
    if (BUF) {
        if (MIX) {
            const uint64_t da = (uint64_t)(uintptr_t)vw.dquad + 2 * (uint64_t)(uint32_t)qorg;
            rsrc.x = __builtin_amdgcn_readfirstlane((uint32_t)da);
            rsrc.y = __builtin_amdgcn_readfirstlane(((uint32_t)(da >> 32) & 0xffffu) | (8u << 16));
        } else {
        const uint64_t qa = (uint64_t)(uintptr_t)vw.quad + (uint32_t)qorg;
        rsrc.x = __builtin_amdgcn_readfirstlane((uint32_t)qa);
        rsrc.y = __builtin_amdgcn_readfirstlane(((uint32_t)(qa >> 32) & 0xffffu) | (4u << 16));
        }
        rsrc.z = __builtin_amdgcn_readfirstlane((uint32_t)(qp * (h + 1) - 1));
        rsrc.w = 0x00020000u;
        asm volatile("" : "+s"(rsrc));
    }
    typedef float f32x2 __attribute__((ext_vector_type(2)));
    auto line6 = [&](int i, auto clamp_tag, auto unr_tag) {
        constexpr bool CLAMP = decltype(clamp_tag)::value;
        constexpr bool UNR = decltype(unr_tag)::value;
        static_assert(!UNR || (ROW && D16), "the unrolled form is written for the row-wise walk with D16 window loads");
        const float xi = (float)((ROW ? y : x) + i);
        const float bx = STRICT ? H[0] * xi : fma_(H[ROW ? 1 : 0], xi, H[2]), by = STRICT ? H[3] * xi : fma_(H[ROW ? 4 : 3], xi, H[5]),
                    bz = STRICT ? H[6] * xi : fma_(H[ROW ? 7 : 6], xi, H[8]);
        const int line = (i + 5) >> 1;
        float rcol[6];
        f32x2 wcol[3];
        {
            constexpr int U = BLK / 64, S = ROW ? 6 : 1;
            const uint32_t wa = (uint32_t)(uintptr_t)(const __attribute__((address_space(3))) float*)(wts + (UNR ? 0 : (ROW ? line : 6 * line) * BLK));
#pragma unroll
            for (int k = 0; k < 3; k++)
                asm("ds_read2st64_b32 %0, %1 offset0:%2 offset1:%3" : "=v"(wcol[k]) : "v"(wa), "n"(2 * U * S * k + (UNR ? U * line : 0)), "n"(2 * U * S * k + U * S + (UNR ? U * line : 0)), "v"(bz));
        }
        if (D16) {
            const uint32_t a0 = (uint32_t)(uintptr_t)(const __attribute__((address_space(3))) unsigned short*)(UNR ? tile + own - 5 * tw - 5 : ROW ? tile + own + i * tw - 5 : tile + own + i - 5 * tw);
#pragma unroll
            for (int jj = 0; jj < 6; jj++)
                asm("ds_read_u16_d16_hi %0, %1 offset:%2" : "=v"(rcol[jj]) : "v"(a0), "n"((ROW ? jj * 4 : jj * 2 * (PM_RW + 10) * 2) + (UNR ? line * 2 * (PM_RW + 10) * 2 : 0)), "v"(bz));
        }
        float ax[6], ay[6];
        uint32_t q[6];
        uint64_t q2[6];
        __builtin_amdgcn_s_setprio(3);
#pragma unroll
        for (int jj = 0; jj < 6; jj++) {
            const float yj = (float)((ROW ? x : y) + 2 * jj - 5);
            float X = fma_(H[ROW ? 0 : 1], yj, bx), Y = fma_(H[ROW ? 3 : 4], yj, by), Z = fma_(H[ROW ? 6 : 7], yj, bz);
            if (STRICT) { X += H[2]; Y += H[5]; Z += H[8]; }
            float u, v;
            const float uhi = (float)(w - 1), vhi = (float)(h - 1);
            if (STRICT) {
                persp_divide_exact<CLAMP>(X, Y, Z, u, v);
                if (CLAMP) {
                    u = fminf(fmaxf(u, 0.0f), uhi);
                    v = fminf(fmaxf(v, 0.0f), vhi);
                }
            } else {
                const float rz = __builtin_amdgcn_rcpf(Z);
                u = X * rz;
                v = Y * rz;
                if (CLAMP) {
                    u = __builtin_amdgcn_fmed3f(u, 0.0f, uhi);
                    v = __builtin_amdgcn_fmed3f(v, 0.0f, vhi);
                }
            }
            int iu, iv;
            ax[jj] = __builtin_amdgcn_fractf(u);
            ay[jj] = __builtin_amdgcn_fractf(v);
            asm("v_cvt_flr_i32_f32 %0, %1" : "=v"(iu) : "v"(u));
            asm("v_cvt_flr_i32_f32 %0, %1" : "=v"(iv) : "v"(v));
            int lin;
            asm("v_mad_i32_i24 %0, %1, %2, %3" : "=v"(lin) : "v"(iv), "s"(qp), "v"(iu));
            if (MIX && DIAG == 1) {
                q2[jj] = ((uint64_t)(uint32_t)~lin << 32) | (uint32_t)lin;
            } else if (MIX && DIAG == 2) {
                uint32_t la;
                asm("v_bfe_u32 %0, %1, 0, 12" : "=v"(la) : "v"(lin));
                asm volatile("ds_read_b64 %0, %1" : "=v"(q2[jj]) : "v"(la << 3));
            } else if (MIX) {
                asm volatile("buffer_load_dwordx2 %0, %1, %2, 0 idxen" : "=v"(q2[jj]) : "v"(lin), "s"(rsrc));
            } else if (BUF) {
                asm volatile("buffer_load_dword %0, %1, %2, 0 idxen" : "=v"(q[jj]) : "v"(lin), "s"(rsrc));
            } else {
                const uint32_t off2 = (uint32_t)lin << 2;
                q[jj] = *(global_u32_ptr)((const char __attribute__((address_space(1)))*)(uintptr_t)(((uint64_t)qb_hi << 32) | qb_lo) + off2);
            }
        }
        __builtin_amdgcn_sched_barrier(0);
        __builtin_amdgcn_s_setprio(0);
        __builtin_amdgcn_sched_barrier(0);
#pragma unroll
        for (int jj = 0; jj < 6; jj++) {
            float t00, t10, t01, t11;
            if (MIX && DIAG == 1) {
            } else if (MIX && DIAG == 2) {
                if (jj == 0) asm("s_waitcnt lgkmcnt(5)" : "+v"(q2[0]), "+v"(rcol[0]), "+v"(rcol[1]), "+v"(rcol[2]), "+v"(rcol[3]), "+v"(rcol[4]), "+v"(rcol[5]),
                                 "+v"(wcol[0]), "+v"(wcol[1]), "+v"(wcol[2]) : "v"(q2[5]));
                else asm("s_waitcnt lgkmcnt(%2)" : "+v"(q2[jj]), "+v"(sum_src_src) : "n"(5 - jj), "v"(q2[5]));
            } else if (MIX) {
                if (jj == 0) asm("s_waitcnt vmcnt(5)" : "+v"(q2[0]) : "v"(q2[5]));
                if (jj == 1) asm("s_waitcnt vmcnt(4)" : "+v"(q2[1]), "+v"(sum_src_src) : "v"(q2[5]));
                if (jj == 2) asm("s_waitcnt vmcnt(3)" : "+v"(q2[2]), "+v"(sum_src_src) : "v"(q2[5]));
                if (jj == 3) asm("s_waitcnt vmcnt(2)" : "+v"(q2[3]), "+v"(sum_src_src) : "v"(q2[5]));
                if (jj == 4) asm("s_waitcnt vmcnt(1)" : "+v"(q2[4]), "+v"(sum_src_src) : "v"(q2[5]));
                if (jj == 5) asm("s_waitcnt vmcnt(0)" : "+v"(q2[5]), "+v"(sum_src_src));
            } else if (BUF) {
                if (jj == 0) asm("s_waitcnt vmcnt(5)" : "+v"(q[0]) : "v"(q[5]));
                if (jj == 1) asm("s_waitcnt vmcnt(4)" : "+v"(q[1]), "+v"(sum_src_src) : "v"(q[5]));
                if (jj == 2) asm("s_waitcnt vmcnt(3)" : "+v"(q[2]), "+v"(sum_src_src) : "v"(q[5]));
                if (jj == 3) asm("s_waitcnt vmcnt(2)" : "+v"(q[3]), "+v"(sum_src_src) : "v"(q[5]));
                if (jj == 4) asm("s_waitcnt vmcnt(1)" : "+v"(q[4]), "+v"(sum_src_src) : "v"(q[5]));
                if (jj == 5) asm("s_waitcnt vmcnt(0)" : "+v"(q[5]), "+v"(sum_src_src));
            }
            float s;
            if (MIX) {
                const uint32_t lo = (uint32_t)q2[jj], hi = (uint32_t)(q2[jj] >> 32);
                float ta, tb;
                asm("v_fma_mix_f32 %0, %1, %2, %2 op_sel:[0,1,0] op_sel_hi:[0,1,1]" : "=v"(ta) : "v"(ax[jj]), "v"(lo));
                asm("v_fma_mix_f32 %0, %1, %2, %2 op_sel:[0,1,0] op_sel_hi:[0,1,1]" : "=v"(tb) : "v"(ax[jj]), "v"(hi));
                s = fma_(ay[jj], tb, ta);
            } else {
            asm("v_cvt_f32_ubyte0 %0, %1" : "=v"(t00) : "v"(q[jj]));
            asm("v_cvt_f32_ubyte1 %0, %1" : "=v"(t10) : "v"(q[jj]));
            asm("v_cvt_f32_ubyte2 %0, %1" : "=v"(t01) : "v"(q[jj]));
            asm("v_cvt_f32_ubyte3 %0, %1" : "=v"(t11) : "v"(q[jj]));
            if (STRICT) {
                const float top = fma_(ax[jj], t10 - t00, t00);
                const float bot = fma_(ax[jj], t11 - t01, t01);
                s = fma_(ay[jj], bot - top, top);
            } else {
                const float d1 = t10 - t00, d2 = t01 - t00, d3 = (t11 - t01) - d1;
                s = fma_(ay[jj], fma_(ax[jj], d3, d2), fma_(ax[jj], d1, t00));
            }
            }
            if (jj == 0 && DIAG != 2) {
                if (D16)
                    asm("s_waitcnt lgkmcnt(0)" : "+v"(rcol[0]), "+v"(rcol[1]), "+v"(rcol[2]), "+v"(rcol[3]), "+v"(rcol[4]), "+v"(rcol[5]),
                        "+v"(wcol[0]), "+v"(wcol[1]), "+v"(wcol[2]), "+v"(s));
                else
                    asm("s_waitcnt lgkmcnt(0)" : "+v"(wcol[0]), "+v"(wcol[1]), "+v"(wcol[2]), "+v"(s));
            }
            const float r = D16 ? rcol[jj] : tile_value(ROW ? tile[own + i * tw + (2 * jj - 5)] : tile[own + (2 * jj - 5) * tw + i]);
            const float wt = wcol[jj >> 1][jj & 1];
            const float ws = wt * s;
            sum_src += ws;
            sum_src_src = fma_(ws, s, sum_src_src);
            if (STRICT) sum_ref_src = fma_(wt * r, s, sum_ref_src);
            else sum_ref_src = fma_(ws, r, sum_ref_src);
        }
    };
    if (need_clamp) {
#pragma unroll 1
        for (int i = -5; i <= 5; i += 2) line6(i, std::true_type(), std::false_type());
    } else if constexpr (MIX) {
#pragma unroll
        for (int i = -5; i <= 5; i += 2) line6(i, std::false_type(), std::true_type());
    } else {
#pragma unroll 1
        for (int i = -5; i <= 5; i += 2) line6(i, std::false_type(), std::false_type());
    }
    sum_src *= pr.inv_wsum;
    sum_src_src *= pr.inv_wsum;
    sum_ref_src *= pr.inv_wsum;
    const float var_src = sum_src_src - sum_src * sum_src;
    if (var_src < 1e-5f) return TSAR_MAXCOST;
    const float covar = sum_ref_src - pr.mean_ref * sum_src;
    const float vrs = sqrt_rsq_exact(pr.var_ref * var_src);
    return fmaxf(0.0f, fminf(TSAR_MAXCOST, 1.0f - covar / vrs));
}

__host__ __device__ constexpr bool r5_diag_variant(int V) { return V == (250 | 131072 | 2097152 | 4194304) || V == (250 | 131072 | 2097152 | 8388608); }
__host__ __device__ constexpr bool r5_production_variant(int V) { return V == 114 || V == 122 || V == 250 || V == (114 | 131072) || V == (122 | 131072) || V == (250 | 131072) || V == (250 | 131072 | 2097152); }
```

tsar-mvs_amd/csrc/selftest_kernels.hip:

```cpp
#include "tsar_device_math.h"

#define ST_BLOCK 256

__global__ __launch_bounds__(ST_BLOCK) void divide_arrays_kernel(const float* __restrict__ X, const float* __restrict__ Y, const float* __restrict__ Z,
                                                                 size_t n, float* __restrict__ u, float* __restrict__ v, int ieee) {
    const size_t i = (size_t)blockIdx.x * ST_BLOCK + threadIdx.x;
    if (i >= n) return;
    float a, b;
    if (ieee == 2) { const float rz = __builtin_amdgcn_rcpf(Z[i]); a = X[i] * rz; b = Y[i] * rz; }
    else if (ieee) { a = X[i] / Z[i]; b = Y[i] / Z[i]; }
    else persp_divide_exact<true>(X[i], Y[i], Z[i], a, b);
    u[i] = a;
    v[i] = b;
}

DEVFN bool same_quotient(float a, float b) { return __float_as_uint(a) == __float_as_uint(b) || (a != a && b != b); }

__global__ __launch_bounds__(ST_BLOCK) void divide_random_kernel(uint32_t per_thread, uint32_t seed_lo, uint32_t seed_hi, int mode, int guarded,
                                                                 unsigned long long* out) {
    const uint32_t tid = blockIdx.x * ST_BLOCK + threadIdx.x;
    uint32_t bad = 0, fell_back = 0;
    for (uint32_t k = 0; k < per_thread; k++) {
        const Rand4 rn = philox_uniform4(tid, k, 0x5eedu, seed_lo, seed_hi);
        const Rand4 rm = philox_uniform4(tid, k, 0x5eeeu, seed_lo, seed_hi);
        float X, Y, Z;
        if (mode == 0) {
            Z = __builtin_ldexpf(1.0f + rn.u[0], (int)(rn.u[1] * 8.0f) - 4);
            X = between(rn.u[2], -64.0f, 8256.0f) * Z;
            Y = between(rn.u[3], -64.0f, 8256.0f) * Z;
        } else {
            const uint32_t b0 = (uint32_t)(rn.u[0] * 16777216.0f) - 1u, b1 = (uint32_t)(rn.u[1] * 16777216.0f) - 1u, b2 = (uint32_t)(rn.u[2] * 16777216.0f) - 1u;
            const uint32_t e0 = (uint32_t)(rm.u[0] * 16777216.0f) - 1u, e1 = (uint32_t)(rm.u[1] * 16777216.0f) - 1u, e2 = (uint32_t)(rm.u[2] * 16777216.0f) - 1u;
            auto make = [&](uint32_t m, uint32_t e) {
                const uint32_t ex = mode == 1 ? 107u + (e >> 1) % 58u : (e >> 1) & 0xffu;
                return __uint_as_float(((e & 1u) << 31) | (ex << 23) | (m & 0x7fffffu));
            };
            X = make(b0, e0); Y = make(b1, e1); Z = make(b2, e2);
        }
        float a, b;
        if (guarded) persp_divide_exact<true>(X, Y, Z, a, b);
        else div_pair_rcp_exact(X, Y, Z, a, b);
        bad += !same_quotient(a, X / Z);
        bad += !same_quotient(b, Y / Z);
        fell_back += !div_guard_ok(X, Y, Z);
    }
    for (int o = 32; o; o >>= 1) { bad += __shfl_down(bad, o); fell_back += __shfl_down(fell_back, o); }
    if ((threadIdx.x & 63) == 0) {
        atomicAdd(&out[0], (unsigned long long)bad);
        atomicAdd(&out[1], (unsigned long long)fell_back);
    }
}

__global__ __launch_bounds__(ST_BLOCK) void sqrt_enumerate_kernel(int mode, uint32_t seed_lo, uint32_t seed_hi, unsigned long long* out) {
    const uint32_t i = blockIdx.x * ST_BLOCK + threadIdx.x;
    float x;
    if (mode == 0 || mode == 2) x = __uint_as_float(0x3f800000u + i);
    else if (mode == 3) {
        const Rand4 rn = philox_uniform4(i, 0u, 0x5a18u, seed_lo, seed_hi);
        const uint32_t m = (uint32_t)(rn.u[0] * 16777216.0f) - 1u, e = 93u + i % 67u;
        x = __uint_as_float((e << 23) | (m & 0x7fffffu));
    } else {
        const Rand4 rn = philox_uniform4(i, 0u, 0x5a17u, seed_lo, seed_hi);
        const uint32_t m = (uint32_t)(rn.u[0] * 16777216.0f) - 1u, e = 27u + (uint32_t)(rn.u[1] * 200.0f) % 200u;
        x = __uint_as_float((e << 23) | (m & 0x7fffffu));
    }
    const float got = mode == 2 ? x * __builtin_amdgcn_rsqf(x) : sqrt_rsq_exact(x);
    uint32_t bad = __float_as_uint(got) != __float_as_uint(sqrtf(x));
    for (int o = 32; o; o >>= 1) bad += __shfl_down(bad, o);
    if ((threadIdx.x & 63) == 0 && bad) atomicAdd(&out[0], (unsigned long long)bad);
}
int launch_selftest_sqrt(tsar_ctx* ctx, int mode, uint64_t seed, unsigned long long* dcounts) {
    hipLaunchKernelGGL(sqrt_enumerate_kernel, dim3((1u << 24) / ST_BLOCK), dim3(ST_BLOCK), 0, ctx->stream, mode, (uint32_t)seed, (uint32_t)(seed >> 32), dcounts);
    TSAR_HIP_TRY(ctx, hipGetLastError());
    return TSAR_OK;
}

int launch_selftest_divide(tsar_ctx* ctx, const float* X, const float* Y, const float* Z, size_t n, float* u, float* v, int ieee) {
    hipLaunchKernelGGL(divide_arrays_kernel, dim3((unsigned)((n + ST_BLOCK - 1) / ST_BLOCK)), dim3(ST_BLOCK), 0, ctx->stream, X, Y, Z, n, u, v, ieee);
    TSAR_HIP_TRY(ctx, hipGetLastError());
    return TSAR_OK;
}

int launch_selftest_divide_random(tsar_ctx* ctx, int log2_pairs, uint64_t seed, int mode, int guarded, unsigned long long* dcounts) {
    const int lt = log2_pairs < 20 ? log2_pairs : 20;
    const uint32_t threads = 1u << lt, per_thread = 1u << (log2_pairs - lt);
    hipLaunchKernelGGL(divide_random_kernel, dim3((threads + ST_BLOCK - 1) / ST_BLOCK), dim3(threads < ST_BLOCK ? threads : ST_BLOCK), 0, ctx->stream, per_thread,
                       (uint32_t)seed, (uint32_t)(seed >> 32), mode, guarded, dcounts);
    TSAR_HIP_TRY(ctx, hipGetLastError());
    return TSAR_OK;
}

#include "pm_sweep_impl.h"
__global__ __launch_bounds__(256) void sweep_census_kernel(const DevScene* __restrict__ sc, int colour, const float* __restrict__ c, const float4* __restrict__ n4,
                                                           int tiles_x, int cost_consistent, unsigned long long* out) {
    const int tix = blockIdx.x % tiles_x, tiy = blockIdx.x / tiles_x;
    const int ly = threadIdx.x >> 4, k = threadIdx.x & 15;
    const int y = tiy * 16 + ly;
    const int x = tix * 32 + 2 * k + ((colour + y) & 1);
    const int w = sc->w, h = sc->h;
    const bool live = x < w && y < h;
    uint32_t alive = 0, alive_nodup = 0, present = 0;
    if (live) {
        const DevRef& rf = sc->ref;
        int cand[8];
        select_candidates(sc, c, c, x, y, cand);
        const float4 n_first = n4[y * w + x];
        float4 pl[8];
#pragma unroll
        for (int a = 0; a < 8; a++) {
            if (cand[a] < 0) continue;
            present |= 1u << a;
            pl[a] = n4[cand[a] & 0x3fffffff];
            if (cost_consistent && same_bits(pl[a], n_first)) continue;
            const float d = plane_depth(rf, pl[a], x, y);
            if (!(d >= rf.depthMin && d <= rf.depthMax)) continue;
            alive |= 1u << a;
            bool dup = false;
#pragma unroll
            for (int b = 0; b < 8; b++)
                if (b < a && ((alive_nodup >> b) & 1u) && same_bits(pl[a], pl[b])) dup = true;
            if (!dup) alive_nodup |= 1u << a;
        }
    }
    int arms_any = 0;
#pragma unroll
    for (int a = 0; a < 8; a++) arms_any += __any((alive >> a) & 1u) ? 1 : 0;
    int mx = __popc(alive), mxn = __popc(alive_nodup), sm = mx, smn = mxn, px = live ? 1 : 0, pr = __popc(present);
    for (int o = 32; o; o >>= 1) {
        mx = max(mx, __shfl_xor(mx, o)); mxn = max(mxn, __shfl_xor(mxn, o));
        sm += __shfl_xor(sm, o); smn += __shfl_xor(smn, o); px += __shfl_xor(px, o); pr += __shfl_xor(pr, o);
    }
    if ((threadIdx.x & 63) == 0 && px > 0) {
        atomicAdd(&out[0], 1ull); atomicAdd(&out[1], (unsigned long long)arms_any); atomicAdd(&out[2], (unsigned long long)mx);
        atomicAdd(&out[3], (unsigned long long)mxn); atomicAdd(&out[4], (unsigned long long)sm); atomicAdd(&out[5], (unsigned long long)smn);
        atomicAdd(&out[6], (unsigned long long)px); atomicAdd(&out[7], (unsigned long long)pr);
    }
}

__global__ __launch_bounds__(256) void sweep_repeat_kernel(const DevScene* __restrict__ sc, int colour, const float* __restrict__ c, const float4* __restrict__ n4,
                                                           int tiles_x, int cost_consistent, unsigned long long* __restrict__ memo, unsigned long long* out) {
    const int tix = blockIdx.x % tiles_x, tiy = blockIdx.x / tiles_x;
    const int ly = threadIdx.x >> 4, k = threadIdx.x & 15;
    const int y = tiy * 16 + ly;
    const int x = tix * 32 + 2 * k + ((colour + y) & 1);
    const int w = sc->w, h = sc->h;
    const bool live = x < w && y < h;
    uint32_t alive = 0, rep_same = 0, rep_any = 0;
    if (live) {
        const DevRef& rf = sc->ref;
        int cand[8];
        select_candidates(sc, c, c, x, y, cand);
        const size_t p = (size_t)y * w + x;
        const float4 n_first = n4[p];
        unsigned long long prev[8], now[8];
#pragma unroll
        for (int a = 0; a < 8; a++) { prev[a] = memo[p * 8 + a]; now[a] = 0; }
#pragma unroll
        for (int a = 0; a < 8; a++) {
            if (cand[a] < 0) continue;
            const float4 pl = n4[cand[a] & 0x3fffffff];
            if (cost_consistent && same_bits(pl, n_first)) continue;
            const float d = plane_depth(rf, pl, x, y);
            if (!(d >= rf.depthMin && d <= rf.depthMax)) continue;
            alive |= 1u << a;
            unsigned long long hsh = ((unsigned long long)__float_as_uint(pl.x) | ((unsigned long long)__float_as_uint(pl.y) << 32)) * 0x9E3779B97F4A7C15ull;
            hsh ^= ((unsigned long long)__float_as_uint(pl.z) | ((unsigned long long)__float_as_uint(pl.w) << 32)) * 0xC2B2AE3D27D4EB4Full;
            hsh |= 1ull;
            now[a] = hsh;
            if (prev[a] == hsh) rep_same |= 1u << a;
#pragma unroll
            for (int b = 0; b < 8; b++)
                if (prev[b] == hsh) rep_any |= 1u << a;
        }
#pragma unroll
        for (int a = 0; a < 8; a++) memo[p * 8 + a] = now[a];
    }
    int pairs = 0, pairs_skippable = 0;
#pragma unroll
    for (int a = 0; a < 8; a++) {
        const bool al = (alive >> a) & 1u, fresh = al && !((rep_any >> a) & 1u);
        if (__any(al)) { pairs++; if (!__any(fresh)) pairs_skippable++; }
    }
    int sa = __popc(alive), ss = __popc(rep_same), sy = __popc(rep_any), mx = sa, mf = __popc(alive & ~rep_any), sf = mf;
    for (int o = 32; o; o >>= 1) {
        sa += __shfl_xor(sa, o); ss += __shfl_xor(ss, o); sy += __shfl_xor(sy, o); sf += __shfl_xor(sf, o);
        mx = max(mx, __shfl_xor(mx, o)); mf = max(mf, __shfl_xor(mf, o));
    }
    if ((threadIdx.x & 63) == 0) {
        atomicAdd(&out[0], (unsigned long long)sa); atomicAdd(&out[1], (unsigned long long)ss); atomicAdd(&out[2], (unsigned long long)sy);
        atomicAdd(&out[3], (unsigned long long)pairs); atomicAdd(&out[4], (unsigned long long)pairs_skippable);
        atomicAdd(&out[5], (unsigned long long)mx); atomicAdd(&out[6], (unsigned long long)mf);
        atomicAdd(&out[7], (unsigned long long)((sf + 63) >> 6));
    }
}
int launch_sweep_repeat(tsar_ctx* ctx, int colour, unsigned long long* memo, unsigned long long* dout) {
    const DevScene& hs = ctx->hscene;
    const int tiles_x = (hs.w + 31) / 32, tiles_y = (hs.h + 15) / 16;
    hipLaunchKernelGGL(sweep_repeat_kernel, dim3(tiles_x * tiles_y), dim3(256), 0, ctx->stream, ctx->dscene, colour, ctx->buf[0].c, ctx->buf[0].n4, tiles_x,
                       ctx->cost_consistent ? 1 : 0, memo, dout);
    TSAR_HIP_TRY(ctx, hipGetLastError());
    return TSAR_OK;
}

int launch_sweep_census(tsar_ctx* ctx, int colour, unsigned long long* dout) {
    const DevScene& hs = ctx->hscene;
    const int tiles_x = (hs.w + 31) / 32, tiles_y = (hs.h + 15) / 16;
    hipLaunchKernelGGL(sweep_census_kernel, dim3(tiles_x * tiles_y), dim3(256), 0, ctx->stream, ctx->dscene, colour, ctx->buf[0].c, ctx->buf[0].n4, tiles_x,
                       ctx->cost_consistent ? 1 : 0, dout);
    TSAR_HIP_TRY(ctx, hipGetLastError());
    return TSAR_OK;
}
```

tsar-mvs_amd/csrc/tsar_api.hip:

```cpp
#include <math.h>
#include <stdio.h>
#include <stdlib.h>
#include <string.h>

#include <algorithm>

#include "tsar_dev.h"

ScopedKernelTimer::ScopedKernelTimer(tsar_ctx* c, const char* name) : ctx(c) {
    if (!ctx->timing || !name) return;
    for (size_t k = 0; k < ctx->timers.size(); k++)
        if (ctx->timers[k].name == name) ti = (int)k;
    if (ti < 0) {
        ctx->timers.emplace_back();
        ctx->timers.back().name = name;
        ti = (int)ctx->timers.size() - 1;
    }
    if (hipEventCreate(&e0) != hipSuccess) { ti = -1; return; }
    if (hipEventCreate(&e1) != hipSuccess) { hipEventDestroy(e0); ti = -1; return; }
    hipEventRecord(e0, ctx->stream);
}
ScopedKernelTimer::~ScopedKernelTimer() {
    if (ti < 0) return;
    hipEventRecord(e1, ctx->stream);
    ctx->timers[ti].pending.emplace_back(e0, e1);
}
static void drain_timers(tsar_ctx* ctx) {
    for (auto& k : ctx->timers) {
        for (auto& pr : k.pending) {
            float ms = 0.f;
            if (hipEventSynchronize(pr.second) == hipSuccess && hipEventElapsedTime(&ms, pr.first, pr.second) == hipSuccess) {
                k.total_ms += ms;
                k.launches++;
            }
            hipEventDestroy(pr.first);
            hipEventDestroy(pr.second);
        }
        k.pending.clear();
    }
}

static int fail(tsar_ctx* ctx, int code, const char* msg) {
    if (ctx) ctx->err = msg;
    return code;
}
template <typename T>
static int dev_alloc(tsar_ctx* ctx, T** p, size_t n) {
    if (*p) { hipFree(*p); *p = nullptr; }
    hipError_t e = hipMalloc((void**)p, n * sizeof(T));
    if (e != hipSuccess) { ctx->err = std::string("hipMalloc: ") + hipGetErrorString(e); return e == hipErrorOutOfMemory ? TSAR_ERR_NOMEM : TSAR_ERR_HIP; }
    return TSAR_OK;
}
template <typename T>
static void dev_free(T*& p) {
    if (p) hipFree(p);
    p = nullptr;
}
static hipMemcpyKind in_kind(int mem) { return mem == TSAR_MEM_DEVICE ? hipMemcpyDeviceToDevice : hipMemcpyHostToDevice; }
static hipMemcpyKind out_kind(int mem) { return mem == TSAR_MEM_DEVICE ? hipMemcpyDeviceToDevice : hipMemcpyDeviceToHost; }
#define CHECK_CTX(ctx) \
    if (!(ctx)) return TSAR_ERR_INVALID; \
    if (hipSetDevice((ctx)->device) != hipSuccess) return fail(ctx, TSAR_ERR_HIP, "hipSetDevice failed")
#define NEED_VIEWS(ctx) if (!(ctx)->have_views) return fail(ctx, TSAR_ERR_STATE, "tsar_set_views has not been called")
#define NEED_SOURCES(ctx) if ((ctx)->hscene.n_sel < 1) return fail(ctx, TSAR_ERR_STATE, "no source views: tsar_set_views was given the reference view only")
#define NEED_STATE(ctx) if (!(ctx)->have_state) return fail(ctx, TSAR_ERR_STATE, "no plane state: call tsar_pm_init, tsar_load_planes or tsar_set_plane first")
#define TRY(expr) do { int rc_ = (expr); if (rc_ != TSAR_OK) return rc_; } while (0)

template <typename T>
struct TmpIn {
    tsar_ctx* ctx;
    const T* d = nullptr;
    T* owned = nullptr;
    int rc = TSAR_OK;
    TmpIn(tsar_ctx* c, const T* src, size_t n, int mem, ScratchScope* scratch = nullptr) : ctx(c) {
        if (!src) return;
        if (mem == TSAR_MEM_DEVICE) { d = src; return; }
        T* staging = nullptr;
        if (scratch) {
            staging = (T*)scratch->alloc(n * sizeof(T));
            if (!staging) rc = fail(ctx, TSAR_ERR_NOMEM, "hipMalloc failed");
        } else {
            rc = dev_alloc(ctx, &owned, n);
            staging = owned;
        }
        if (rc == TSAR_OK && hipMemcpyAsync(staging, src, n * sizeof(T), hipMemcpyHostToDevice, ctx->stream) != hipSuccess) rc = fail(ctx, TSAR_ERR_HIP, "H2D failed");
        d = staging;
    }
    ~TmpIn() {
        if (owned) { hipStreamSynchronize(ctx->stream); hipFree(owned); }
    }
};

static void inv3(const double* m, double* o) {
    const double c00 = m[4] * m[8] - m[5] * m[7], c01 = m[5] * m[6] - m[3] * m[8], c02 = m[3] * m[7] - m[4] * m[6];
    const double det = m[0] * c00 + m[1] * c01 + m[2] * c02;
    const double s = 1.0 / det;
    o[0] = c00 * s; o[1] = (m[2] * m[7] - m[1] * m[8]) * s; o[2] = (m[1] * m[5] - m[2] * m[4]) * s;
    o[3] = c01 * s; o[4] = (m[0] * m[8] - m[2] * m[6]) * s; o[5] = (m[2] * m[3] - m[0] * m[5]) * s;
    o[6] = c02 * s; o[7] = (m[1] * m[6] - m[0] * m[7]) * s; o[8] = (m[0] * m[4] - m[1] * m[3]) * s;
}
static void mul3(const double* a, const double* b, double* o) {
    for (int r = 0; r < 3; r++)
        for (int c = 0; c < 3; c++) o[3 * r + c] = a[3 * r] * b[c] + a[3 * r + 1] * b[3 + c] + a[3 * r + 2] * b[6 + c];
}
static void scale_k(const float* K, double s, double* o) {
    for (int i = 0; i < 9; i++) o[i] = K[i];
    o[0] /= s; o[4] /= s; o[2] /= s; o[5] /= s;
}

static void derive_cameras(tsar_ctx* ctx, const tsar_camera* cams) {
    DevScene& sc = ctx->hscene;
    const double s = ctx->params.cam_scale > 0 ? ctx->params.cam_scale : 1.0;
    double K0[9], R0t[9], t0[3];
    scale_k(cams[0].K, s, K0);
    for (int r = 0; r < 3; r++) {
        t0[r] = cams[0].t[r];
        for (int c = 0; c < 3; c++) R0t[3 * r + c] = cams[0].R[3 * c + r];
    }
    for (int v = 0; v < ctx->n_views; v++) {
        double Kv[9], Rv[9], Rrel[9], trel[3];
        scale_k(cams[v].K, s, Kv);
        for (int i = 0; i < 9; i++) Rv[i] = cams[v].R[i];
        mul3(Rv, R0t, Rrel);
        for (int r = 0; r < 3; r++) trel[r] = cams[v].t[r] - (Rrel[3 * r] * t0[0] + Rrel[3 * r + 1] * t0[1] + Rrel[3 * r + 2] * t0[2]);
        if (v == 0) {
            for (int i = 0; i < 9; i++) Rrel[i] = (i % 4 == 0) ? 1.0 : 0.0;
            trel[0] = trel[1] = trel[2] = 0.0;
        }
        DevView& dv = sc.view[v];
        for (int i = 0; i < 9; i++) { dv.K[i] = (float)Kv[i]; dv.R[i] = (float)Rrel[i]; }
        for (int r = 0; r < 3; r++) dv.t[r] = (float)trel[r];
        dv.t_abs_lo = std::min(std::min(fabsf(dv.t[0]), fabsf(dv.t[1])), fabsf(dv.t[2]));
        dv.t_abs_hi = std::max(std::max(fabsf(dv.t[0]), fabsf(dv.t[1])), fabsf(dv.t[2]));
        {
            double K0inv[9], KR[9], A[9];
            inv3(K0, K0inv);
            mul3(Kv, Rrel, KR);
            mul3(KR, K0inv, A);
            for (int i = 0; i < 9; i++) dv.A[i] = (float)A[i];
            for (int r = 0; r < 3; r++) dv.b[r] = (float)(Kv[3 * r] * trel[0] + Kv[3 * r + 1] * trel[1] + Kv[3 * r + 2] * trel[2]);
        }
        {
            double Kvinv[9], RT[9], K0RT[9], B[9];
            inv3(Kv, Kvinv);
            for (int r = 0; r < 3; r++)
                for (int c = 0; c < 3; c++) RT[3 * r + c] = Rrel[3 * c + r];
            mul3(K0, RT, K0RT);
            mul3(K0RT, Kvinv, B);
            float* G = sc.geom_back[v];
            for (int r = 0; r < 3; r++) {
                for (int c = 0; c < 3; c++) G[4 * r + c] = (float)B[3 * r + c];
                G[4 * r + 3] = (float)(-(K0RT[3 * r] * trel[0] + K0RT[3 * r + 1] * trel[1] + K0RT[3 * r + 2] * trel[2]));
            }
        }
        if (v == 0) {
            DevRef& rf = sc.ref;
            double Kinv[9], M[9], Minv[9];
            inv3(Kv, Kinv);
            mul3(K0, Rrel, M);
            inv3(M, Minv);
            for (int i = 0; i < 9; i++) {
                rf.K[i] = (float)Kv[i]; rf.Kinv[i] = (float)Kinv[i]; rf.Minv[i] = (float)Minv[i];
                rf.Rorig[i] = cams[0].R[i];
            }
            for (int r = 0; r < 3; r++)
                for (int c = 0; c < 3; c++) rf.RorigInv[3 * r + c] = cams[0].R[3 * c + r];
            for (int r = 0; r < 3; r++) {
                rf.P34[r] = (float)(K0[3 * r] * trel[0] + K0[3 * r + 1] * trel[1] + K0[3 * r + 2] * trel[2]);
                rf.C[r] = (float)(-(Rrel[r] * trel[0] + Rrel[3 + r] * trel[1] + Rrel[6 + r] * trel[2]));
            }
            rf.fx = (float)K0[0];
            rf.f = (float)K0[0];
            rf.alpha = (float)K0[0] / (float)K0[4];
            rf.baseline = 1.0f;
            rf.depthMin = ctx->params.depth_min;
            rf.depthMax = ctx->params.depth_max;
        }
    }
    auto sparse3 = [](const float* K) { return K[1] == 0.f && K[3] == 0.f && K[6] == 0.f && K[7] == 0.f && K[8] == 1.f; };
    sc.k_sparse = sparse3(sc.ref.Kinv) ? 1 : 0;
    for (int v = 0; v < ctx->n_views; v++) sc.k_sparse &= sparse3(sc.view[v].K) ? 1 : 0;
    sc.min_disp = sc.ref.f * sc.ref.baseline / ctx->params.depth_max;
    sc.max_disp = sc.ref.f * sc.ref.baseline / ctx->params.depth_min;
    int steps = 0;
    for (float dz = sc.max_disp / 2.0f; dz >= 0.01f; dz = dz / 10.0f) steps++;
    sc.refine_steps = steps;
}

static bool init_window_differs(const tsar_ctx* ctx) {
    const tsar_params& p = ctx->params;
    return !(p.flags & TSAR_FLAG_FIX_INIT_RADIUS) && (p.box_hsize / 2 != (p.box_hsize - 1) / 2 || p.box_vsize / 2 != (p.box_vsize - 1) / 2);
}
static void fill_scene_params(tsar_ctx* ctx, bool for_init = false) {
    DevScene& sc = ctx->hscene;
    const tsar_params& p = ctx->params;
    const bool init_radius = for_init && !(p.flags & TSAR_FLAG_FIX_INIT_RADIUS);
    sc.hrad = init_radius ? p.box_hsize / 2 : (p.box_hsize - 1) / 2;
    sc.vrad = init_radius ? p.box_vsize / 2 : (p.box_vsize - 1) / 2;
    sc.n_best = p.n_best;
    sc.cost_comb = p.cost_comb;
    sc.flags = p.flags;
    sc.seed_lo = (uint32_t)p.seed;
    sc.seed_hi = (uint32_t)(p.seed >> 32);
    sc.lut_row_major = (p.flags & TSAR_FLAG_STRICT_DIV) ? 0 : 1;
    std::vector<int> d2;
    for (int i = -sc.hrad; i <= sc.hrad; i += 2)
        for (int j = -sc.vrad; j <= sc.vrad; j += 2) d2.push_back(i * i + j * j);
    std::sort(d2.begin(), d2.end());
    d2.erase(std::unique(d2.begin(), d2.end()), d2.end());
    sc.lut_classes = (int)d2.size() <= TSAR_LUT_MAX_CLASSES ? (int)d2.size() : 0;
    for (int k = 0; k < sc.lut_classes; k++) sc.lut_d2[k] = d2[k];
    const int rl = sc.lut_row_major ? sc.vrad : sc.hrad, rt = sc.lut_row_major ? sc.hrad : sc.vrad;
    sc.lut_chunk = lut_chunk_taps(rt + 1);
    sc.lut_pad_taps = (rt + sc.lut_chunk) / sc.lut_chunk * sc.lut_chunk;
    for (uint32_t& r : sc.tap_row) r = (uint32_t)sc.lut_classes * 1024u;
    for (int l = 0; l <= rl && sc.lut_classes; l++)
        for (int t = 0; t <= rt; t++) {
            const int a = 2 * l - rl, b = 2 * t - rt;
            sc.tap_row[l * sc.lut_pad_taps + t] = 1024u * (uint32_t)(std::lower_bound(d2.begin(), d2.end(), a * a + b * b) - d2.begin());
        }
}
static int upload_scene(tsar_ctx* ctx) {
    if (!ctx->dscene) TRY(dev_alloc(ctx, &ctx->dscene, 1));
    TSAR_HIP_TRY(ctx, hipMemcpyAsync(ctx->dscene, &ctx->hscene, sizeof(DevScene), hipMemcpyHostToDevice, ctx->stream));
    TSAR_HIP_TRY(ctx, hipStreamSynchronize(ctx->stream));
    return TSAR_OK;
}

extern "C" const char* tsar_version(void) {
#ifdef TSAR_EXPERIMENTS
    return "tsar-mvs_amd 0.2.0 (gfx950) +experiments";
#else
    return "tsar-mvs_amd 0.2.0 (gfx950)";
#endif
}

static void read_knobs(tsar_ctx* ctx) {
    auto num = [](const char* name, int dflt) { const char* e = getenv(name); return e && e[0] ? atoi(e) : dflt; };
    auto on = [](const char* name, bool dflt) { const char* e = getenv(name); return e && e[0] ? e[0] != '0' : dflt; };
    ctx->variant = num("TSAR_VARIANT", ctx->variant);
    ctx->buffer_gather = on("TSAR_BUFFER_GATHER", true);
    ctx->mix_gather = on("TSAR_MIX_GATHER", true);
    ctx->strip_w = num("TSAR_STRIP", -1);
    ctx->buffer_from = num("TSAR_BUFFER_FROM", 1);
    ctx->force_block = num("TSAR_BLOCK", 0);
    ctx->memo_mode = num("TSAR_MEMO", 1);
    ctx->compact_from = num("TSAR_COMPACT_FROM", 6);
    ctx->lut_mode = num("TSAR_LUT", 1);
    ctx->ransac_wgs = num("TSAR_RANSAC_WGS", 8);
    ctx->ransac_chain = num("TSAR_RANSAC_CHAIN", 8);
    ctx->ransac_lookahead = num("TSAR_RANSAC_LOOKAHEAD", 0);
    ctx->ransac_poll_limit = num("TSAR_RANSAC_POLL_LIMIT", 1 << 15);
    ctx->ransac_cooperative = on("TSAR_RANSAC_COOPERATIVE", true);
    ctx->ransac_force_fallback = on("TSAR_RANSAC_FORCE_FALLBACK", false);
    ctx->trace_host = getenv("TSAR_TRACE_HOST") != nullptr;
#ifdef TSAR_EXPERIMENTS
    ctx->lds_pad = (size_t)num("TSAR_LDS_PAD", 0);
#endif
}

extern "C" int tsar_create(int device, tsar_ctx** out) {
    if (!out) return TSAR_ERR_INVALID;
    *out = nullptr;
    int n = 0;
    if (hipGetDeviceCount(&n) != hipSuccess || n <= 0) return TSAR_ERR_HIP;
    if (device < 0 || device >= n) return TSAR_ERR_INVALID;
    if (hipSetDevice(device) != hipSuccess) return TSAR_ERR_HIP;
    tsar_ctx* ctx = new (std::nothrow) tsar_ctx();
    if (!ctx) return TSAR_ERR_NOMEM;
    ctx->device = device;
    if (hipStreamCreateWithFlags(&ctx->stream, hipStreamNonBlocking) != hipSuccess) { delete ctx; return TSAR_ERR_HIP; }
    tsar_default_params(&ctx->params);
    ctx->variant = probe_d16_hi_zeroes(ctx) ? 250 : 114;
    read_knobs(ctx);
    *out = ctx;
    return TSAR_OK;
}

static void free_views(tsar_ctx* ctx) {
    for (auto& p : ctx->img) dev_free(p);
    for (auto& p : ctx->quad) dev_free(p);
    for (auto& p : ctx->dquad) dev_free(p);
    ctx->img.clear();
    ctx->quad.clear();
    ctx->dquad.clear();
}
static void free_geom(tsar_ctx* ctx) {
    for (auto& p : ctx->geom_maps) dev_free(p);
    ctx->geom_maps.clear();
    for (auto& p : ctx->hscene.geom_depth) p = nullptr;
    ctx->hscene.geom_on = 0;
}
static void free_planes(tsar_ctx* ctx) {
    for (int b = 0; b < 2; b++) { dev_free(ctx->buf[b].c); dev_free(ctx->buf[b].n4); }
    dev_free(ctx->ratio); dev_free(ctx->depth); dev_free(ctx->scale); dev_free(ctx->lrdiff); dev_free(ctx->confid);
    dev_free(ctx->fakedepth); dev_free(ctx->beview); dev_free(ctx->canny); dev_free(ctx->out4);
    dev_free(ctx->memo_cand); dev_free(ctx->memo_seq); dev_free(ctx->changed_seq);
    dev_free(ctx->resize4);
    ctx->have_resize = false;
}

extern "C" int tsar_destroy(tsar_ctx* ctx) {
    if (!ctx) return TSAR_OK;
    hipSetDevice(ctx->device);
    if (ctx->stream) hipStreamSynchronize(ctx->stream);
    drain_timers(ctx);
    free_views(ctx);
    free_planes(ctx);
    free_geom(ctx);
    dev_free(ctx->dscene); dev_free(ctx->region_text); dev_free(ctx->region_size); dev_free(ctx->region_n4);
    if (ctx->scratch.base) hipFree(ctx->scratch.base);
    if (ctx->stream) hipStreamDestroy(ctx->stream);
    delete ctx;
    return TSAR_OK;
}
extern "C" const char* tsar_last_error(const tsar_ctx* ctx) { return ctx ? ctx->err.c_str() : "null context"; }
extern "C" int tsar_get_stream(tsar_ctx* ctx, void** stream_out) {
    if (!ctx || !stream_out) return TSAR_ERR_INVALID;
    *stream_out = (void*)ctx->stream;
    return TSAR_OK;
}
extern "C" int tsar_synchronize(tsar_ctx* ctx) {
    CHECK_CTX(ctx);
    TSAR_HIP_TRY(ctx, hipStreamSynchronize(ctx->stream));
    return TSAR_OK;
}

extern "C" void tsar_default_params(tsar_params* p) {
    if (!p) return;
    memset(p, 0, sizeof(*p));
    p->box_hsize = 19;
    p->box_vsize = 19;
    p->n_best = 2;
    p->cost_comb = TSAR_COMB_BEST_N;
    p->depth_min = 2.0f;
    p->depth_max = 20.0f;
    p->cam_scale = 1.0f;
    p->flags = 0;
    p->seed = 0;
}

extern "C" int tsar_set_params(tsar_ctx* ctx, const tsar_params* p) {
    CHECK_CTX(ctx);
    if (!p) return fail(ctx, TSAR_ERR_INVALID, "params is NULL");
    if (p->box_hsize < 1 || p->box_vsize < 1 || p->box_hsize > 63 || p->box_vsize > 63) return fail(ctx, TSAR_ERR_INVALID, "box size must be in 1..63");
    if (p->n_best < 1 || p->n_best > TSAR_MAX_SELECTED) return fail(ctx, TSAR_ERR_INVALID, "n_best must be in 1..32 (the reference's costVector holds 32 views, gipuma.cu:467)");
    if (p->cost_comb < TSAR_COMB_ALL || p->cost_comb > TSAR_COMB_GOOD) return fail(ctx, TSAR_ERR_INVALID, "cost_comb must be one of TSAR_COMB_ALL / BEST_N / ANGLE / GOOD");
    if (!(p->depth_min > 0.f) || !(p->depth_max > p->depth_min)) return fail(ctx, TSAR_ERR_INVALID, "need 0 < depth_min < depth_max");
    if (!(p->cam_scale > 0.f)) return fail(ctx, TSAR_ERR_INVALID, "cam_scale must be > 0");
    ctx->params = *p;
    ctx->have_params = true;
    fill_scene_params(ctx);
    if (ctx->have_views) {
        ctx->have_views = false;
        ctx->have_state = false;
    }
    return TSAR_OK;
}

static int probe_exact_divide(tsar_ctx* ctx) {
    if (ctx->exact_div_probe != 0) return ctx->exact_div_probe;
    uint64_t bad = 0, total = 0;
    for (int mode = 0; mode < 2; mode++) {
        if (tsar_selftest_divide_random(ctx, 22, 0x5EEDD1F1DE5ull + (uint64_t)mode, mode, 0, &bad, nullptr) != TSAR_OK) return 0;
        total += bad;
    }
    ctx->exact_div_probe = total == 0 ? 1 : -1;
    return ctx->exact_div_probe;
}
static int probe_exact_sqrt(tsar_ctx* ctx) {
    if (ctx->exact_sqrt_probe != 0) return ctx->exact_sqrt_probe;
    uint64_t bad = 0, bad_range = 0;
    if (tsar_selftest_sqrt(ctx, 0, 0, &bad) != TSAR_OK) return 0;
    if (tsar_selftest_sqrt(ctx, 3, 0x5EED5A17ull, &bad_range) != TSAR_OK) return 0;
    ctx->exact_sqrt_probe = (bad | bad_range) == 0 ? 1 : -1;
    return ctx->exact_sqrt_probe;
}

static int set_views_impl(tsar_ctx* ctx, int n_views, int w, int h, const void* const* gray, int elem, int mem, const tsar_camera* cams) {
    CHECK_CTX(ctx);
    if (!ctx->have_params) return fail(ctx, TSAR_ERR_STATE, "tsar_set_params must be called before tsar_set_views");
    if (ctx->params.flags & TSAR_FLAG_STRICT_DIV) {
        const int pr = probe_exact_divide(ctx);
        if (pr == 0) return TSAR_ERR_HIP;
        if (pr < 0) return fail(ctx, TSAR_ERR_HIP, "TSAR_FLAG_STRICT_DIV: this device's v_rcp_f32 does not give correctly rounded quotients through the short division "
                                                   "sequence (tsar_selftest_divide_random found mismatches against IEEE division); strict mode is refused rather than run inexactly");
    }
    if (n_views < 1 || n_views > TSAR_MAX_VIEWS) return fail(ctx, TSAR_ERR_INVALID, "n_views must be in 1..TSAR_MAX_VIEWS");
    if (w < 8 || h < 8 || (int64_t)w * h > (int64_t)1 << 28) return fail(ctx, TSAR_ERR_INVALID, "image size out of range");
    if (w + 2 >= (1 << 23) || h + 2 >= (1 << 23)) return fail(ctx, TSAR_ERR_INVALID, "image side too long for the 24-bit quad addressing (w + 2, h + 2 < 2^23)");
    if (!gray || !cams) return fail(ctx, TSAR_ERR_INVALID, "gray/cams is NULL");
    for (int v = 0; v < n_views; v++)
        if (!gray[v]) return fail(ctx, TSAR_ERR_INVALID, "gray[v] is NULL");
    ctx->have_views = false;
    ctx->have_state = false;
    ctx->have_out = false;
    ctx->have_resize = false;
    free_geom(ctx);
    const size_t np = (size_t)w * h;
    if (w != ctx->w || h != ctx->h) { free_views(ctx); free_planes(ctx); }
    ctx->w = w; ctx->h = h; ctx->n_views = n_views;
    DevScene& sc = ctx->hscene;
    sc.w = w; sc.h = h; sc.quad_pitch = w + 2;
    if ((int)ctx->img.size() < n_views) ctx->img.resize(n_views, nullptr);
    if ((int)ctx->quad.size() < n_views) ctx->quad.resize(n_views, nullptr);
    if ((int)ctx->dquad.size() < n_views) ctx->dquad.resize(n_views, nullptr);
    struct DevInt {
        int* p = nullptr;
        ~DevInt() { if (p) hipFree(p); }
    } dflag_owner;
    TRY(dev_alloc(ctx, &dflag_owner.p, 1));
    int* const dflag = dflag_owner.p;
    hipMemsetAsync(dflag, 0, sizeof(int), ctx->stream);
    for (int v = 0; v < n_views; v++) {
        if (!ctx->img[v]) TRY(dev_alloc(ctx, &ctx->img[v], np));
        if (!ctx->quad[v]) TRY(dev_alloc(ctx, &ctx->quad[v], (size_t)(w + 2) * (h + 2)));
        if (elem == 4) {
            TSAR_HIP_TRY(ctx, hipMemcpyAsync(ctx->img[v], gray[v], np * sizeof(float), in_kind(mem), ctx->stream));
        } else if (mem == TSAR_MEM_DEVICE) {
            TRY(launch_expand_u8(ctx, (const uint8_t*)gray[v], ctx->img[v], np));
        } else {
            uint8_t* stage = (uint8_t*)ctx->quad[v];
            TSAR_HIP_TRY(ctx, hipMemcpyAsync(stage, gray[v], np, hipMemcpyHostToDevice, ctx->stream));
            TRY(launch_expand_u8(ctx, stage, ctx->img[v], np));
        }
        TRY(launch_build_quad(ctx, ctx->img[v], ctx->quad[v], w, h, dflag));
    }
    int hflag = 0;
    TSAR_HIP_TRY(ctx, hipMemcpyAsync(&hflag, dflag, sizeof(int), hipMemcpyDeviceToHost, ctx->stream));
    TSAR_HIP_TRY(ctx, hipStreamSynchronize(ctx->stream));
    sc.use_quad = hflag ? 0 : 1;
    if (sc.use_quad) {
        const int ps = probe_exact_sqrt(ctx);
        if (ps == 0) return TSAR_ERR_HIP;
        if (ps < 0) return fail(ctx, TSAR_ERR_HIP, "this device's v_rsq_f32 does not give correctly rounded square roots through the one-correction sequence of the cost's tail "
                                                   "(tsar_selftest_sqrt found mismatches against sqrtf): refused rather than run with costs that differ from the oracle's");
    }
    for (int v = 0; v < n_views; v++) { sc.view[v].img = ctx->img[v]; sc.view[v].quad = ctx->quad[v]; sc.view[v].dquad = nullptr; }
    if (!sc.use_quad)
        for (auto& q : ctx->quad) dev_free(q);
    const bool want_dquad = sc.use_quad && !(ctx->params.flags & TSAR_FLAG_STRICT_DIV) && ctx->buffer_gather && ctx->mix_gather && ctx->variant == 250;
    for (int v = 1; v < n_views; v++) {
        if (!want_dquad) { dev_free(ctx->dquad[v]); continue; }
        if (!ctx->dquad[v]) TRY(dev_alloc(ctx, &ctx->dquad[v], (size_t)(w + 2) * (h + 2)));
        TRY(launch_build_dquad(ctx, ctx->quad[v], ctx->dquad[v], w, h));
        sc.view[v].dquad = ctx->dquad[v];
    }
    TSAR_HIP_TRY(ctx, hipStreamSynchronize(ctx->stream));
    derive_cameras(ctx, cams);
    ctx->cams.assign(cams, cams + n_views);
    ctx->views_u8 = elem == 1;
    auto window_problem = [&](bool for_init) -> const char* {
        fill_scene_params(ctx, for_init);
        if (lut_path_applies(ctx)) return nullptr;
        const size_t lds = (size_t)(sc.hrad + 1) * (sc.vrad + 1) * 1024 + (size_t)(32 + 2 * sc.hrad) * (16 + 2 * sc.vrad) * 4 + 16;
        if (lds <= 160 * 1024) return nullptr;
        if (!sc.use_quad) return "box too large for images that are not 8-bit: the per-thread weight table does not fit the 160 KiB of LDS per CU (largest square box: 23)";
        if (sc.lut_classes == 0) return "this rectangular box has more than 144 distinct tap distances (radii of mixed parity): the shared weight table cannot hold them and the per-thread table does not fit LDS; use radii of equal parity, or a box of at most 23";
        return "box too large for fast mode on this device: the D16 LDS-load probe failed, so the general-window loop is not available; use TSAR_FLAG_STRICT_DIV, or a box of at most 23";
    };
    const char* problem = n_views > 1 ? window_problem(false) : nullptr;
    if (!problem && n_views > 1 && init_window_differs(ctx)) problem = window_problem(true);
    fill_scene_params(ctx);
    if (problem) return fail(ctx, TSAR_ERR_INVALID, problem);
    sc.n_sel = std::min(n_views - 1, TSAR_MAX_SELECTED);
    for (int i = 0; i < sc.n_sel; i++) sc.sel[i] = i + 1;
    for (int b = 0; b < 2; b++) {
        if (!ctx->buf[b].c) TRY(dev_alloc(ctx, &ctx->buf[b].c, np));
        if (!ctx->buf[b].n4) TRY(dev_alloc(ctx, &ctx->buf[b].n4, np));
    }
    float** fplanes[] = {&ctx->ratio, &ctx->depth, &ctx->scale, &ctx->lrdiff, &ctx->confid, &ctx->fakedepth};
    for (float** fp : fplanes) {
        if (!*fp) TRY(dev_alloc(ctx, fp, np));
        TSAR_HIP_TRY(ctx, hipMemsetAsync(*fp, 0, np * sizeof(float), ctx->stream));
    }
    if (!ctx->beview) TRY(dev_alloc(ctx, &ctx->beview, np));
    if (!ctx->canny) TRY(dev_alloc(ctx, &ctx->canny, np));
    if (!ctx->out4) TRY(dev_alloc(ctx, &ctx->out4, np));
    TSAR_HIP_TRY(ctx, hipMemsetAsync(ctx->beview, 0, np * sizeof(int32_t), ctx->stream));
    TSAR_HIP_TRY(ctx, hipMemsetAsync(ctx->canny, 0, np * sizeof(int32_t), ctx->stream));
    TRY(upload_scene(ctx));
    ctx->have_views = true;
    return TSAR_OK;
}

extern "C" int tsar_set_views(tsar_ctx* ctx, int n_views, int w, int h, const float* const* gray, int mem, const tsar_camera* cams) {
    return set_views_impl(ctx, n_views, w, h, (const void* const*)gray, 4, mem, cams);
}
extern "C" int tsar_set_views_u8(tsar_ctx* ctx, int n_views, int w, int h, const uint8_t* const* gray, int mem, const tsar_camera* cams) {
    return set_views_impl(ctx, n_views, w, h, (const void* const*)gray, 1, mem, cams);
}

extern "C" int tsar_set_view_subset(tsar_ctx* ctx, int n, const int32_t* view_idx) {
    CHECK_CTX(ctx);
    NEED_VIEWS(ctx);
    if (n < 1 || n > TSAR_MAX_SELECTED || !view_idx) return fail(ctx, TSAR_ERR_INVALID, "subset size must be in 1..32 (the reference's viewSelectionSubset / costVector hold 32, gipuma.cu:467)");
    for (int i = 0; i < n; i++)
        if (view_idx[i] < 1 || view_idx[i] >= ctx->n_views) return fail(ctx, TSAR_ERR_INVALID, "view index must be in 1..n_views-1");
    ctx->hscene.n_sel = n;
    for (int i = 0; i < n; i++) ctx->hscene.sel[i] = view_idx[i];
    if (ctx->have_state) ctx->cost_consistent = false;
    return upload_scene(ctx);
}

extern "C" int tsar_pm_init(tsar_ctx* ctx) {
    CHECK_CTX(ctx);
    NEED_VIEWS(ctx);
    NEED_SOURCES(ctx);
    const bool own_window = init_window_differs(ctx);
    int rc = TSAR_OK;
    if (own_window) {
        fill_scene_params(ctx, true);
        rc = upload_scene(ctx);
    }
    if (rc == TSAR_OK) rc = launch_pm_init(ctx);
    if (hipStreamSynchronize(ctx->stream) != hipSuccess && rc == TSAR_OK) rc = fail(ctx, TSAR_ERR_HIP, "hipStreamSynchronize failed");
    if (own_window) {
        fill_scene_params(ctx, false);
        const int rc2 = upload_scene(ctx);
        if (rc2 != TSAR_OK) ctx->have_views = false;
        if (rc == TSAR_OK) rc = rc2;
    }
    TRY(rc);
    ctx->have_state = true;
    ctx->have_out = false;
    ctx->sweeps_done = 0;
    ctx->cost_consistent = !own_window;
    return TSAR_OK;
}

static int pm_sweeps(tsar_ctx* ctx, int n_sweeps, int first_colour, int do_prop, int do_refine) {
    int cur[2] = {0, 0};
    ctx->memo_valid_from = ctx->launch_seq + 1;
    ctx->call_launch = 0;
    if (ctx->memo_mode && n_sweeps > 2 && !ctx->memo_cand) {
        const size_t np = (size_t)ctx->w * ctx->h;
        TRY(dev_alloc(ctx, &ctx->memo_cand, np * 8));
        TRY(dev_alloc(ctx, &ctx->memo_seq, np));
        TRY(dev_alloc(ctx, &ctx->changed_seq, np));
        TSAR_HIP_TRY(ctx, hipMemsetAsync(ctx->memo_seq, 0, np * sizeof(uint32_t), ctx->stream));
        TSAR_HIP_TRY(ctx, hipMemsetAsync(ctx->changed_seq, 0, np * sizeof(uint32_t), ctx->stream));
    }
    for (int s = 0; s < n_sweeps; s++) {
        ctx->launch_seq++;
        const int colour = (first_colour + s) & 1;
        const PlaneBuf& same_in = ctx->buf[cur[colour]];
        const PlaneBuf& other = ctx->buf[cur[colour ^ 1]];
        const PlaneBuf& same_out = ctx->buf[cur[colour] ^ 1];
        TRY(launch_pm_sweep(ctx, colour, same_in, other, same_out, 1u + (uint32_t)ctx->sweeps_done, do_prop, do_refine));
        cur[colour] ^= 1;
// ... 374 lines not shown
    coarse->memo_valid_from = coarse->launch_seq + 1;
    return upload_scene(coarse);
}

extern "C" int tsar_pyramid_planes(tsar_ctx* coarse, const tsar_ctx* fine_in) {
    CHECK_CTX(coarse);
    tsar_ctx* fine = const_cast<tsar_ctx*>(fine_in);
    if (!fine || fine == coarse) return fail(coarse, TSAR_ERR_INVALID, "tsar_pyramid_planes: fine must be another context");
    if (!fine->have_state) return fail(coarse, TSAR_ERR_INVALID, "tsar_pyramid_planes: the fine context has no plane state");
    if (!coarse->have_views || fine->device != coarse->device || coarse->w != (fine->w + 1) / 2 || coarse->h != (fine->h + 1) / 2)
        return fail(coarse, TSAR_ERR_INVALID, "tsar_pyramid_planes: the coarse context must hold views of ((w + 1) / 2, (h + 1) / 2) of the fine one on the same device");
    NEED_SOURCES(coarse);
    TRY(stream_after(coarse, fine));
    TRY(launch_pyramid_planes(coarse, fine->buf[0].n4, fine->w, fine->h, coarse->buf[0].n4));
    TRY(launch_pm_rescore(coarse, coarse->buf[0].n4, coarse->buf[1].c, coarse->buf[1].n4, coarse->beview, coarse->ratio));
    TSAR_HIP_TRY(coarse, hipStreamSynchronize(coarse->stream));
    std::swap(coarse->buf[0], coarse->buf[1]);
    coarse->have_state = true;
    coarse->have_out = false;
    coarse->sweeps_done = 0;
    coarse->cost_consistent = true;
    coarse->memo_valid_from = coarse->launch_seq + 1;
    return TSAR_OK;
}

extern "C" int tsar_upsample_merge(tsar_ctx* fine, const tsar_ctx* coarse_in) {
    CHECK_CTX(fine);
    tsar_ctx* coarse = const_cast<tsar_ctx*>(coarse_in);
    if (!coarse || coarse == fine) return fail(fine, TSAR_ERR_INVALID, "tsar_upsample_merge: coarse must be another context");
    if (!fine->have_state) return fail(fine, TSAR_ERR_INVALID, "tsar_upsample_merge: the fine context has no plane state");
    NEED_SOURCES(fine);
    if (coarse->device != fine->device || !coarse->have_state || coarse->w != (fine->w + 1) / 2 || coarse->h != (fine->h + 1) / 2)
        return fail(fine, TSAR_ERR_INVALID, "tsar_upsample_merge: the coarse context must hold a plane state of ((w + 1) / 2, (h + 1) / 2) on the same device");
    TRY(stream_after(fine, coarse));
    TRY(launch_pm_upsample_merge(fine, coarse->buf[0].n4, coarse->w, coarse->h));
    TSAR_HIP_TRY(fine, hipStreamSynchronize(fine->stream));
    std::swap(fine->buf[0], fine->buf[1]);
    fine->have_out = false;
    fine->sweeps_done = 0;
    fine->cost_consistent = true;
    fine->memo_valid_from = fine->launch_seq + 1;
    return TSAR_OK;
}

extern "C" int tsar_depth_to_plane(tsar_ctx* ctx) {
    CHECK_CTX(ctx);
    NEED_STATE(ctx);
    ctx->cost_consistent = false;
    TRY(launch_depth_to_plane(ctx));
    TSAR_HIP_TRY(ctx, hipStreamSynchronize(ctx->stream));
    return TSAR_OK;
}
extern "C" int tsar_get_result(tsar_ctx* ctx, float* depth, float* normal_world, float* cost, float* confid, int mem) {
    CHECK_CTX(ctx);
    NEED_STATE(ctx);
    if (!ctx->have_out) return fail(ctx, TSAR_ERR_STATE, "call tsar_compute_disp / tsar_fill_textureless first");
    const size_t np = (size_t)ctx->w * ctx->h;
    if (depth || normal_world) {
        if (mem == TSAR_MEM_DEVICE) {
            TRY(launch_split_out4(ctx, depth, normal_world));
        } else {
            ScratchScope scratch(ctx);
            float *dd = nullptr, *dn = nullptr;
            int rc = TSAR_OK;
            if (depth && !(dd = (float*)scratch.alloc(np * 4))) rc = fail(ctx, TSAR_ERR_NOMEM, "hipMalloc failed");
            if (rc == TSAR_OK && normal_world && !(dn = (float*)scratch.alloc(np * 12))) rc = fail(ctx, TSAR_ERR_NOMEM, "hipMalloc failed");
            if (rc == TSAR_OK) rc = launch_split_out4(ctx, dd, dn);
            if (rc == TSAR_OK && depth && hipMemcpyAsync(depth, dd, np * 4, hipMemcpyDeviceToHost, ctx->stream) != hipSuccess) rc = fail(ctx, TSAR_ERR_HIP, "D2H failed");
            if (rc == TSAR_OK && normal_world && hipMemcpyAsync(normal_world, dn, np * 12, hipMemcpyDeviceToHost, ctx->stream) != hipSuccess) rc = fail(ctx, TSAR_ERR_HIP, "D2H failed");
            hipStreamSynchronize(ctx->stream);
            scratch.release();
            TRY(rc);
        }
    }
    if (cost) TSAR_HIP_TRY(ctx, hipMemcpyAsync(cost, ctx->buf[0].c, np * 4, out_kind(mem), ctx->stream));
    if (confid) TSAR_HIP_TRY(ctx, hipMemcpyAsync(confid, ctx->confid, np * 4, out_kind(mem), ctx->stream));
    TSAR_HIP_TRY(ctx, hipStreamSynchronize(ctx->stream));
    return TSAR_OK;
}

extern "C" int tsar_set_reliable_mask(tsar_ctx* ctx, const float* scale, int mem) {
    CHECK_CTX(ctx);
    NEED_VIEWS(ctx);
    if (!scale) return fail(ctx, TSAR_ERR_INVALID, "scale is NULL");
    TSAR_HIP_TRY(ctx, hipMemcpyAsync(ctx->scale, scale, (size_t)ctx->w * ctx->h * 4, in_kind(mem), ctx->stream));
    TSAR_HIP_TRY(ctx, hipStreamSynchronize(ctx->stream));
    return TSAR_OK;
}
extern "C" int tsar_get_reliable_mask(tsar_ctx* ctx, float* scale, int mem) {
    CHECK_CTX(ctx);
    NEED_VIEWS(ctx);
    if (!scale) return fail(ctx, TSAR_ERR_INVALID, "scale is NULL");
    TSAR_HIP_TRY(ctx, hipMemcpyAsync(scale, ctx->scale, (size_t)ctx->w * ctx->h * 4, out_kind(mem), ctx->stream));
    TSAR_HIP_TRY(ctx, hipStreamSynchronize(ctx->stream));
    return TSAR_OK;
}
extern "C" int tsar_getview(tsar_ctx* ctx) {
    CHECK_CTX(ctx);
    NEED_STATE(ctx);
    TRY(launch_getview(ctx));
    TSAR_HIP_TRY(ctx, hipStreamSynchronize(ctx->stream));
    return TSAR_OK;
}
extern "C" int tsar_lrdiff(tsar_ctx* ctx) {
    CHECK_CTX(ctx);
    NEED_STATE(ctx);
    NEED_SOURCES(ctx);
    TRY(launch_lrdiff(ctx));
    TSAR_HIP_TRY(ctx, hipStreamSynchronize(ctx->stream));
    return TSAR_OK;
}
extern "C" int tsar_set_regions(tsar_ctx* ctx, const int32_t* labels, int n_regions, const float* region_text, const float* region_size, int mem) {
    CHECK_CTX(ctx);
    NEED_VIEWS(ctx);
    if (!labels || !region_text || n_regions < 1) return fail(ctx, TSAR_ERR_INVALID, "labels/region_text is NULL or n_regions < 1");
    const size_t np = (size_t)ctx->w * ctx->h;
    {
        int32_t lo = 0, hi = 0;
        if (mem == TSAR_MEM_DEVICE) {
            TRY(launch_label_range(ctx, labels, np, &lo, &hi));
        } else {
            lo = hi = labels[0];
            for (size_t i = 1; i < np; i++) { lo = std::min(lo, labels[i]); hi = std::max(hi, labels[i]); }
        }
        if (lo < 0 || hi >= n_regions) return fail(ctx, TSAR_ERR_INVALID, "a label is outside [0, n_regions)");
    }
    TSAR_HIP_TRY(ctx, hipMemcpyAsync(ctx->canny, labels, np * 4, in_kind(mem), ctx->stream));
    TRY(dev_alloc(ctx, &ctx->region_text, (size_t)n_regions));
    TRY(dev_alloc(ctx, &ctx->region_size, (size_t)n_regions));
    TRY(dev_alloc(ctx, &ctx->region_n4, (size_t)n_regions));
    TSAR_HIP_TRY(ctx, hipMemcpyAsync(ctx->region_text, region_text, (size_t)n_regions * 4, in_kind(mem), ctx->stream));
    if (region_size) TSAR_HIP_TRY(ctx, hipMemcpyAsync(ctx->region_size, region_size, (size_t)n_regions * 4, in_kind(mem), ctx->stream));
    else TSAR_HIP_TRY(ctx, hipMemsetAsync(ctx->region_size, 0, (size_t)n_regions * 4, ctx->stream));
    TSAR_HIP_TRY(ctx, hipMemsetAsync(ctx->region_n4, 0, (size_t)n_regions * 16, ctx->stream));
    TSAR_HIP_TRY(ctx, hipStreamSynchronize(ctx->stream));
    ctx->n_regions = n_regions;
    return TSAR_OK;
}
extern "C" int tsar_set_region_planes(tsar_ctx* ctx, const float* region_planes) {
    CHECK_CTX(ctx);
    if (ctx->n_regions < 1) return fail(ctx, TSAR_ERR_STATE, "tsar_set_regions has not been called");
    if (!region_planes) return fail(ctx, TSAR_ERR_INVALID, "region_planes is NULL");
    TSAR_HIP_TRY(ctx, hipMemcpyAsync(ctx->region_n4, region_planes, (size_t)ctx->n_regions * 16, hipMemcpyHostToDevice, ctx->stream));
    TSAR_HIP_TRY(ctx, hipStreamSynchronize(ctx->stream));
    return TSAR_OK;
}
extern "C" int tsar_fake_depth(tsar_ctx* ctx, float* fakedepth_out, int mem) {
    CHECK_CTX(ctx);
    NEED_VIEWS(ctx);
    if (ctx->n_regions < 1) return fail(ctx, TSAR_ERR_STATE, "tsar_set_regions has not been called");
    TRY(launch_fake_depth(ctx));
    if (fakedepth_out) TSAR_HIP_TRY(ctx, hipMemcpyAsync(fakedepth_out, ctx->fakedepth, (size_t)ctx->w * ctx->h * 4, out_kind(mem), ctx->stream));
    TSAR_HIP_TRY(ctx, hipStreamSynchronize(ctx->stream));
    return TSAR_OK;
}
extern "C" int tsar_fill_textureless(tsar_ctx* ctx) {
    CHECK_CTX(ctx);
    NEED_STATE(ctx);
    if (ctx->n_regions < 1) return fail(ctx, TSAR_ERR_STATE, "tsar_set_regions has not been called");
    ctx->cost_consistent = false;
    TRY(launch_update_scale(ctx));
    TRY(launch_compute_disp(ctx));
    TSAR_HIP_TRY(ctx, hipStreamSynchronize(ctx->stream));
    ctx->have_out = true;
    return TSAR_OK;
}

extern "C" void* tsar_host_alloc(size_t bytes) {
    void* p = nullptr;
    if (bytes == 0 || hipHostMalloc(&p, bytes, hipHostMallocDefault) != hipSuccess) return nullptr;
    return p;
}
extern "C" void tsar_host_free(void* p) {
    if (p) hipHostFree(p);
}

extern "C" void* tsar_device_alloc(int device, size_t bytes) {
    void* p = nullptr;
    if (bytes == 0 || hipSetDevice(device) != hipSuccess || hipMalloc(&p, bytes) != hipSuccess) return nullptr;
    return p;
}
extern "C" void tsar_device_free(int device, void* p) {
    if (p && hipSetDevice(device) == hipSuccess) hipFree(p);
}
extern "C" int tsar_device_write(int device, void* dst, const void* host_src, size_t bytes) {
    if (!dst || !host_src) return TSAR_ERR_INVALID;
    if (hipSetDevice(device) != hipSuccess || hipMemcpy(dst, host_src, bytes, hipMemcpyHostToDevice) != hipSuccess) return TSAR_ERR_HIP;
    return TSAR_OK;
}
extern "C" int tsar_peer_copy(int dst_device, void* dst, int src_device, const void* src, size_t bytes) {
    if (!dst || !src) return TSAR_ERR_INVALID;
    if (hipSetDevice(dst_device) != hipSuccess) return TSAR_ERR_HIP;
    if (dst_device != src_device) {
        int can = 0;
        if (hipDeviceCanAccessPeer(&can, dst_device, src_device) == hipSuccess && can) {
            const hipError_t e = hipDeviceEnablePeerAccess(src_device, 0);
            if (e != hipSuccess && e != hipErrorPeerAccessAlreadyEnabled) return TSAR_ERR_HIP;
            (void)hipGetLastError();
        }
    }
    if (hipMemcpyPeer(dst, dst_device, src, src_device, bytes) != hipSuccess) return TSAR_ERR_HIP;
    return TSAR_OK;
}

extern "C" int tsar_enable_kernel_timing(tsar_ctx* ctx, int enable) {
    if (!ctx) return TSAR_ERR_INVALID;
    ctx->timing = enable != 0;
    return TSAR_OK;
}
extern "C" int tsar_reset_kernel_timing(tsar_ctx* ctx) {
    CHECK_CTX(ctx);
    hipStreamSynchronize(ctx->stream);
    drain_timers(ctx);
    ctx->timers.clear();
    return TSAR_OK;
}
extern "C" int tsar_get_kernel_timing(tsar_ctx* ctx, tsar_kernel_timing* out, int cap, int* n_out) {
    CHECK_CTX(ctx);
    if (!n_out) return fail(ctx, TSAR_ERR_INVALID, "n_out is NULL");
    TSAR_HIP_TRY(ctx, hipStreamSynchronize(ctx->stream));
    drain_timers(ctx);
    *n_out = (int)ctx->timers.size();
    for (int i = 0; i < *n_out && i < cap && out; i++) {
        memset(&out[i], 0, sizeof(out[i]));
        strncpy(out[i].name, ctx->timers[i].name.c_str(), sizeof(out[i].name) - 1);
        out[i].launches = ctx->timers[i].launches;
        out[i].total_ms = ctx->timers[i].total_ms;
    }
    return TSAR_OK;
}

extern "C" int tsar_selftest_divide(tsar_ctx* ctx, const float* X, const float* Y, const float* Z, size_t n, float* u_out, float* v_out, int ieee) {
    CHECK_CTX(ctx);
    if (!X || !Y || !Z || !u_out || !v_out || n == 0 || n > ((size_t)1 << 28)) return fail(ctx, TSAR_ERR_INVALID, "NULL argument or n out of range (1..2^28)");
    ScratchScope scratch(ctx);
    float* d[5];
    for (auto& p : d)
        if (!(p = (float*)scratch.alloc(n * sizeof(float)))) { scratch.release(); return fail(ctx, TSAR_ERR_NOMEM, "device allocation failed"); }
    const float* src[3] = {X, Y, Z};
    int rc = TSAR_OK;
    for (int k = 0; k < 3 && rc == TSAR_OK; k++)
        if (hipMemcpyAsync(d[k], src[k], n * sizeof(float), hipMemcpyHostToDevice, ctx->stream) != hipSuccess) rc = fail(ctx, TSAR_ERR_HIP, "hipMemcpyAsync failed");
    if (rc == TSAR_OK) rc = launch_selftest_divide(ctx, d[0], d[1], d[2], n, d[3], d[4], ieee);
    if (rc == TSAR_OK && (hipMemcpyAsync(u_out, d[3], n * sizeof(float), hipMemcpyDeviceToHost, ctx->stream) != hipSuccess ||
                          hipMemcpyAsync(v_out, d[4], n * sizeof(float), hipMemcpyDeviceToHost, ctx->stream) != hipSuccess))
        rc = fail(ctx, TSAR_ERR_HIP, "hipMemcpyAsync failed");
    if (hipStreamSynchronize(ctx->stream) != hipSuccess && rc == TSAR_OK) rc = fail(ctx, TSAR_ERR_HIP, "hipStreamSynchronize failed");
    scratch.release();
    return rc;
}
extern "C" int tsar_selftest_divide_random(tsar_ctx* ctx, int log2_triples, uint64_t seed, int mode, int guarded, uint64_t* mismatches_out,
                                           uint64_t* outside_guard_out) {
    CHECK_CTX(ctx);
    if (log2_triples < 6 || log2_triples > 36 || mode < 0 || mode > 2 || !mismatches_out) return fail(ctx, TSAR_ERR_INVALID, "log2_triples in 6..36, mode in 0..2");
    if (!guarded && mode == 2) return fail(ctx, TSAR_ERR_INVALID, "the unguarded form is only defined inside the guard (modes 0, 1)");
    ScratchScope scratch(ctx);
    unsigned long long* dc = (unsigned long long*)scratch.alloc(2 * sizeof(unsigned long long));
    if (!dc) { scratch.release(); return fail(ctx, TSAR_ERR_NOMEM, "device allocation failed"); }
    unsigned long long hc[2] = {0, 0};
    int rc = TSAR_OK;
    if (hipMemsetAsync(dc, 0, sizeof hc, ctx->stream) != hipSuccess) rc = fail(ctx, TSAR_ERR_HIP, "hipMemsetAsync failed");
    for (int done = 0; rc == TSAR_OK && done < (1 << (log2_triples > 30 ? log2_triples - 30 : 0)); done++)
        rc = launch_selftest_divide_random(ctx, log2_triples > 30 ? 30 : log2_triples, seed + 0x9E3779B97F4A7C15ull * (uint64_t)done, mode, guarded, dc);
    if (rc == TSAR_OK && hipMemcpyAsync(hc, dc, sizeof hc, hipMemcpyDeviceToHost, ctx->stream) != hipSuccess) rc = fail(ctx, TSAR_ERR_HIP, "hipMemcpyAsync failed");
    if (hipStreamSynchronize(ctx->stream) != hipSuccess && rc == TSAR_OK) rc = fail(ctx, TSAR_ERR_HIP, "hipStreamSynchronize failed");
    scratch.release();
    *mismatches_out = hc[0];
    if (outside_guard_out) *outside_guard_out = hc[1];
    return rc;
}
extern "C" int tsar_selftest_sqrt(tsar_ctx* ctx, int mode, uint64_t seed, uint64_t* mismatches_out) {
    CHECK_CTX(ctx);
    if (mode < 0 || mode > 3 || !mismatches_out) return fail(ctx, TSAR_ERR_INVALID, "mode in 0..3");
    ScratchScope scratch(ctx);
    unsigned long long* dc = (unsigned long long*)scratch.alloc(sizeof(unsigned long long));
    if (!dc) { scratch.release(); return fail(ctx, TSAR_ERR_NOMEM, "device allocation failed"); }
    unsigned long long hc = 0;
    int rc = TSAR_OK;
    if (hipMemsetAsync(dc, 0, sizeof hc, ctx->stream) != hipSuccess) rc = fail(ctx, TSAR_ERR_HIP, "hipMemsetAsync failed");
    if (rc == TSAR_OK) rc = launch_selftest_sqrt(ctx, mode, seed, dc);
    if (rc == TSAR_OK && hipMemcpyAsync(&hc, dc, sizeof hc, hipMemcpyDeviceToHost, ctx->stream) != hipSuccess) rc = fail(ctx, TSAR_ERR_HIP, "hipMemcpyAsync failed");
    if (hipStreamSynchronize(ctx->stream) != hipSuccess && rc == TSAR_OK) rc = fail(ctx, TSAR_ERR_HIP, "hipStreamSynchronize failed");
    scratch.release();
    *mismatches_out = hc;
    return rc;
}
int launch_sweep_repeat(tsar_ctx* ctx, int colour, unsigned long long* memo, unsigned long long* dout);
extern "C" int tsar_selftest_sweep_repeat(tsar_ctx* ctx, int colour, void* memo_dev, uint64_t* out8) {
    CHECK_CTX(ctx);
    if (!memo_dev || !out8) return fail(ctx, TSAR_ERR_INVALID, "memo_dev / out8 is NULL");
    NEED_VIEWS(ctx);
    NEED_STATE(ctx);
    ScratchScope scratch(ctx);
    unsigned long long* dc = (unsigned long long*)scratch.alloc(8 * sizeof(unsigned long long));
    if (!dc) { scratch.release(); return fail(ctx, TSAR_ERR_NOMEM, "device allocation failed"); }
    int rc = TSAR_OK;
    if (hipMemsetAsync(dc, 0, 64, ctx->stream) != hipSuccess) rc = fail(ctx, TSAR_ERR_HIP, "hipMemsetAsync failed");
    if (rc == TSAR_OK) rc = launch_sweep_repeat(ctx, colour & 1, (unsigned long long*)memo_dev, dc);
    if (rc == TSAR_OK && hipMemcpyAsync(out8, dc, 64, hipMemcpyDeviceToHost, ctx->stream) != hipSuccess) rc = fail(ctx, TSAR_ERR_HIP, "hipMemcpyAsync failed");
    if (hipStreamSynchronize(ctx->stream) != hipSuccess && rc == TSAR_OK) rc = fail(ctx, TSAR_ERR_HIP, "hipStreamSynchronize failed");
    scratch.release();
    return rc;
}
extern "C" int tsar_selftest_sweep_census(tsar_ctx* ctx, int colour, uint64_t* out8) {
    CHECK_CTX(ctx);
    NEED_VIEWS(ctx);
    NEED_STATE(ctx);
    if (!out8) return fail(ctx, TSAR_ERR_INVALID, "out8 is NULL");
    ScratchScope scratch(ctx);
    unsigned long long* dc = (unsigned long long*)scratch.alloc(8 * sizeof(unsigned long long));
    if (!dc) { scratch.release(); return fail(ctx, TSAR_ERR_NOMEM, "device allocation failed"); }
    int rc = TSAR_OK;
    if (hipMemsetAsync(dc, 0, 64, ctx->stream) != hipSuccess) rc = fail(ctx, TSAR_ERR_HIP, "hipMemsetAsync failed");
    if (rc == TSAR_OK) rc = launch_sweep_census(ctx, colour & 1, dc);
    if (rc == TSAR_OK && hipMemcpyAsync(out8, dc, 64, hipMemcpyDeviceToHost, ctx->stream) != hipSuccess) rc = fail(ctx, TSAR_ERR_HIP, "hipMemcpyAsync failed");
    if (hipStreamSynchronize(ctx->stream) != hipSuccess && rc == TSAR_OK) rc = fail(ctx, TSAR_ERR_HIP, "hipStreamSynchronize failed");
    scratch.release();
    return rc;
}
```

tsar-mvs_amd/csrc/tsar_dev.h:

```cpp
#pragma once
#include <hip/hip_runtime.h>
#include <stdint.h>
#include <stdlib.h>

#include <string>
#include <vector>

#include "../../include/tsar.h"

#define TSAR_LUT_LINES 32
#define TSAR_LUT_TAPS 40
#define TSAR_LUT_MAX_CLASSES 144
#define TSAR_MAX_SELECTED 32

struct DevView {
    float K[9];
    float R[9];
    float t[3];
    float t_abs_lo;
    float A[9];
    float b[3];
    float t_abs_hi;
    const float* img;
    const uint32_t* quad;
    const uint2* dquad;
};

struct DevRef {
    float K[9];
    float Kinv[9];
    float Minv[9];
    float Rorig[9];
    float RorigInv[9];
    float P34[3];
    float C[3];
    float fx, f, alpha, baseline, depthMin, depthMax;
};

struct DevScene {
    int w, h;
    int n_sel;
    int hrad, vrad;
    int n_best, cost_comb;
    int refine_steps;
    int quad_pitch;
    int use_quad;
    float min_disp, max_disp;
    uint32_t flags;
    uint32_t seed_lo, seed_hi;
    int k_sparse;
    DevRef ref;
    int sel[TSAR_MAX_VIEWS];
    DevView view[TSAR_MAX_VIEWS];
    int lut_classes;
    int lut_row_major;
    int lut_chunk;
    int lut_pad_taps;
    int lut_d2[TSAR_LUT_MAX_CLASSES];
    uint32_t tap_row[TSAR_LUT_LINES * TSAR_LUT_TAPS + 8];
    const float* geom_depth[TSAR_MAX_VIEWS];
    float geom_back[TSAR_MAX_VIEWS][12];
    float geom_weight, geom_clip, geom_clip_sq;
    int geom_on;
};

#define TSAR_V_GEOM 16777216
#define TSAR_V_REDRAW 33554432

struct PlaneBuf {
    float* c;
    float4* n4;
};

struct KernelTimer {
    std::string name;
    int launches = 0;
    float total_ms = 0.f;
    std::vector<std::pair<hipEvent_t, hipEvent_t>> pending;
};

struct ScratchArena {
    char* base = nullptr;
    size_t cap = 0;
    size_t wanted = 0;
};

struct tsar_ctx {
    int device = 0;
    hipStream_t stream = nullptr;
    std::string err;
    tsar_params params{};
    bool have_params = false, have_views = false, have_state = false;
    int w = 0, h = 0, n_views = 0;
    DevScene hscene{};
    DevScene* dscene = nullptr;
    std::vector<float*> img;
    std::vector<uint32_t*> quad;
    std::vector<uint2*> dquad;
    PlaneBuf buf[2]{};
    float *ratio = nullptr, *depth = nullptr, *scale = nullptr, *lrdiff = nullptr, *confid = nullptr, *fakedepth = nullptr;
    int32_t *beview = nullptr, *canny = nullptr;
    float4* out4 = nullptr;
    bool have_out = false;
    bool cost_consistent = false;
    int n_regions = 0;
    float *region_text = nullptr, *region_size = nullptr;
    float4* region_n4 = nullptr;
    int exact_sqrt_probe = 0;
    int exact_div_probe = 0;
    int sweeps_done = 0;
    int32_t* memo_cand = nullptr;
    uint32_t* memo_seq = nullptr;
    uint32_t* changed_seq = nullptr;
    uint32_t launch_seq = 0;
    uint32_t memo_valid_from = 1;
    int call_launch = 0;
    int memo_mode = 1;
    int compact_from = 6;
    std::vector<tsar_camera> cams;
    bool views_u8 = false;
    float4* resize4 = nullptr;
    bool have_resize = false;
    const float* final_text = nullptr;
    std::vector<float*> geom_maps;
    bool rescoring = false;
    int variant = 2;
    bool mix_gather = true;
    bool buffer_gather = true;
    int strip_w = -1;
    int buffer_from = 1;
    int force_block = 0;
    int lut_mode = 1;
    int ransac_wgs = 8;
    int ransac_chain = 8;
    int ransac_lookahead = 0;
    int ransac_poll_limit = 1 << 15;
    bool ransac_cooperative = true;
    bool ransac_force_fallback = false;
    bool trace_host = false;
#ifdef TSAR_EXPERIMENTS
    size_t lds_pad = 0;
#endif
    bool timing = false;
    std::vector<KernelTimer> timers;
    ScratchArena scratch;
};

struct ScratchScope {
    tsar_ctx* ctx;
    size_t used = 0, need = 0;
    std::vector<void*> extra;
    explicit ScratchScope(tsar_ctx* c) : ctx(c) {}
    void* alloc(size_t bytes) {
        bytes = ((bytes ? bytes : 4) + 255) & ~(size_t)255;
        need += bytes;
        if (used + bytes <= ctx->scratch.cap) { void* p = ctx->scratch.base + used; used += bytes; return p; }
        void* p = nullptr;
        if (hipMalloc(&p, bytes) != hipSuccess) return nullptr;
        extra.push_back(p);
        return p;
    }
    void release() {
        for (void* p : extra) hipFree(p);
        extra.clear();
        if (need > ctx->scratch.cap) {
            const bool again = ctx->scratch.wanted > ctx->scratch.cap;
            if (need > ctx->scratch.wanted) ctx->scratch.wanted = need;
            if (again) {
                if (ctx->scratch.base) hipFree(ctx->scratch.base);
                ctx->scratch.base = nullptr;
                ctx->scratch.cap = 0;
                void* p = nullptr;
                if (hipMalloc(&p, ctx->scratch.wanted) == hipSuccess) { ctx->scratch.base = (char*)p; ctx->scratch.cap = ctx->scratch.wanted; }
            }
        }
        used = need = 0;
    }
    ~ScratchScope() { release(); }
};

#define TSAR_HIP_TRY(ctx, expr)                                                                       \
    do {                                                                                              \
        hipError_t e_ = (expr);                                                                       \
        if (e_ != hipSuccess) {                                                                       \
            (ctx)->err = std::string(#expr) + ": " + hipGetErrorString(e_);                           \
            return TSAR_ERR_HIP;                                                                      \
        }                                                                                             \
    } while (0)

struct ScopedKernelTimer {
    tsar_ctx* ctx;
    int ti = -1;
    hipEvent_t e0 = nullptr, e1 = nullptr;
    ScopedKernelTimer(tsar_ctx* c, const char* name);
    ~ScopedKernelTimer();
};

int launch_build_quad(tsar_ctx* ctx, const float* img, uint32_t* quad, int w, int h, int* nonintegral_flag);
int launch_expand_u8(tsar_ctx* ctx, const uint8_t* in, float* out, size_t n);
int launch_build_dquad(tsar_ctx* ctx, const uint32_t* quad, uint2* dquad, int w, int h);
int launch_pm_init(tsar_ctx* ctx);
bool probe_d16_hi_zeroes(tsar_ctx* ctx);
int launch_pm_sweep(tsar_ctx* ctx, int colour, const PlaneBuf& same_in, const PlaneBuf& other, const PlaneBuf& same_out,
                    uint32_t stream_id, int do_prop, int do_refine);
int launch_pm_sweep_lut(tsar_ctx* ctx, int need, int colour, const PlaneBuf& same_in, const PlaneBuf& other, const PlaneBuf& same_out, uint32_t stream_id,
                        int do_prop, int do_refine);
int launch_pm_full_lut(tsar_ctx* ctx, int need, bool init, const float4* planes, float* c, float4* n, int32_t* bv, float* rt);
int lut_chunk_taps(int taps_per_line);
static inline bool lut_path_forced(const tsar_ctx* ctx) { return ctx->lut_mode == 2; }
static inline bool lut_path_applies(const tsar_ctx* ctx) {
    const bool off = ctx->lut_mode == 0;
    const DevScene& hs = ctx->hscene;
    const bool d16_ok = (hs.flags & TSAR_FLAG_STRICT_DIV) || (ctx->variant & 8);
    return !off && d16_ok && hs.use_quad && hs.lut_classes > 0;
}
int launch_pm_sweep_experiment(tsar_ctx* ctx, int colour, const PlaneBuf& same_in, const PlaneBuf& other, const PlaneBuf& same_out, uint32_t stream_id,
                               int do_prop, int do_refine, int* launched);
int launch_pm_cost_planes(tsar_ctx* ctx, const float4* planes, float* cost, int32_t* beview, float* ratio);
int launch_pm_rescore(tsar_ctx* ctx, const float4* planes, float* cost, float4* n, int32_t* beview, float* ratio);
int launch_pm_upsample(tsar_ctx* ctx, const float4* coarse, int cw, int ch);
int launch_pm_upsample_merge(tsar_ctx* ctx, const float4* coarse, int cw, int ch);
int launch_pm_upsample_lut(tsar_ctx* ctx, int need, bool merge, const float4* coarse, int cw, int ch);
int launch_pyr_down(tsar_ctx* ctx, const float* src, int w, int h, void* dst, bool u8);
int launch_geom_pyramid(tsar_ctx* ctx, const float* src, int w, int h, float* dst);
int launch_pyramid_planes(tsar_ctx* ctx, const float4* src, int w, int h, float4* dst);
int launch_get_disp(tsar_ctx* ctx, const float* depth_in, const float* normal_world);
int launch_compute_disp(tsar_ctx* ctx);
int launch_compute_disp_final(tsar_ctx* ctx, const float4* resize4, const float* text);
int launch_depth_to_plane(tsar_ctx* ctx);
int launch_getview(tsar_ctx* ctx);
int launch_lrdiff(tsar_ctx* ctx);
int launch_selftest_divide(tsar_ctx* ctx, const float* X, const float* Y, const float* Z, size_t n, float* u, float* v, int ieee);
int launch_sweep_census(tsar_ctx* ctx, int colour, unsigned long long* dout);
int launch_selftest_divide_random(tsar_ctx* ctx, int log2_pairs, uint64_t seed, int mode, int guarded, unsigned long long* dcounts);
int launch_selftest_sqrt(tsar_ctx* ctx, int mode, uint64_t seed, unsigned long long* dcounts);
int launch_update_scale(tsar_ctx* ctx);
int launch_fake_depth(tsar_ctx* ctx);
int launch_split_out4(tsar_ctx* ctx, float* depth, float* normal3);
int launch_label_range(tsar_ctx* ctx, const int32_t* labels, size_t n, int32_t* lo, int32_t* hi);
```

Baseline: 47.23.

## Prune refinement candidates early with a partial-window NCC bound test

Adds an early-rejection test to the radius-5 per-view cost loop during the first refinement steps. After some of the window rows are accumulated, a Cauchy-Schwarz style bound checks whether the candidate can still beat the current cost, and if not it exits with the max cost. If any lane pruned a view but the candidate still came out cheaper than the current cost, the whole wave recomputes without pruning so results stay exact. It is on by default from sweep 3, only in BEST_N=1 fast mode, and adds extra accumulators plus a census selftest; if the bound is loose or recomputes are frequent, the added work may cost more than it saves.

```diff
diff --git a/include/tsar.h b/include/tsar.h
--- a/include/tsar.h
+++ b/include/tsar.h
@@ -167,6 +167,8 @@
 int tsar_selftest_divide_random(tsar_ctx* ctx, int log2_triples, uint64_t seed, int mode, int guarded, uint64_t* mismatches_out,
                                 uint64_t* outside_guard_out);
 int tsar_selftest_sweep_census(tsar_ctx* ctx, int colour, uint64_t* out8);
+int tsar_selftest_prune_census(tsar_ctx* ctx, int colour, uint64_t* out32);
+int tsar_selftest_refine_steps(tsar_ctx* ctx, int n);
 int tsar_selftest_sweep_repeat(tsar_ctx* ctx, int colour, void* memo_dev, uint64_t* out8);
 int tsar_selftest_slic_stage(tsar_ctx* ctx, int stage, int w, int h, int mw, int mh, const tsar_slic_settings* s, const void* in0,
                              const void* in1, void* inout);
diff --git a/tsar-mvs_amd/api.py b/tsar-mvs_amd/api.py
--- a/tsar-mvs_amd/api.py
+++ b/tsar-mvs_amd/api.py
@@ -64,7 +64,7 @@
     "tsar_set_region_planes", "tsar_fake_depth", "tsar_fill_textureless",
     "tsar_default_slic_settings", "tsar_slic", "tsar_default_fusion_params", "tsar_fuse", "tsar_fuse_ctx",
     "tsar_host_alloc", "tsar_host_free", "tsar_device_alloc", "tsar_device_free", "tsar_device_write", "tsar_peer_copy", "tsar_enable_kernel_timing", "tsar_reset_kernel_timing", "tsar_get_kernel_timing",
-    "tsar_selftest_divide", "tsar_selftest_divide_random", "tsar_selftest_sqrt", "tsar_selftest_sweep_census", "tsar_selftest_sweep_repeat", "tsar_selftest_slic_stage",
+    "tsar_selftest_divide", "tsar_selftest_divide_random", "tsar_selftest_sqrt", "tsar_selftest_sweep_census", "tsar_selftest_prune_census", "tsar_selftest_refine_steps", "tsar_selftest_sweep_repeat", "tsar_selftest_slic_stage",
 ]
 
 _lib = None
@@ -150,6 +150,8 @@
     L.tsar_selftest_divide.argtypes = [C.c_void_p, C.c_void_p, C.c_void_p, C.c_void_p, C.c_size_t, C.c_void_p, C.c_void_p, C.c_int]
     L.tsar_selftest_sweep_census.argtypes = [C.c_void_p, C.c_int, C.POINTER(C.c_uint64)]
     L.tsar_selftest_sweep_repeat.argtypes = [C.c_void_p, C.c_int, C.c_void_p, C.POINTER(C.c_uint64)]
+    L.tsar_selftest_prune_census.argtypes = [C.c_void_p, C.c_int, C.POINTER(C.c_uint64)]
+    L.tsar_selftest_refine_steps.argtypes = [C.c_void_p, C.c_int]
     L.tsar_selftest_sqrt.argtypes = [C.c_void_p, C.c_int, C.c_uint64, C.POINTER(C.c_uint64)]
     L.tsar_selftest_divide_random.argtypes = [C.c_void_p, C.c_int, C.c_uint64, C.c_int, C.c_int, C.POINTER(C.c_uint64), C.POINTER(C.c_uint64)]
     L.tsar_selftest_slic_stage.argtypes = [C.c_void_p, C.c_int, C.c_int, C.c_int, C.c_int, C.c_int, C.POINTER(SlicSettings), C.c_void_p, C.c_void_p, C.c_void_p]
@@ -407,6 +409,17 @@
         self._chk(self.L.tsar_selftest_sweep_census(self._ctx, colour, out))
         keys = ("waves", "arms_any_lane", "max_lane_survivors", "max_lane_survivors_nodup", "lane_survivors", "lane_survivors_nodup", "pixels", "arms_present")
         return dict(zip(keys, [int(v) for v in out]))
+
+    def selftest_refine_steps(self, n: int):
+        self._chk(self.L.tsar_selftest_refine_steps(self._ctx, n))
+
+    def selftest_prune_census(self, colour: int) -> dict:
+        out = (C.c_uint64 * 32)()
+        self._chk(self.L.tsar_selftest_prune_census(self._ctx, colour, out))
+        keys = ("pairs", "rej_row3", "rej_row4", "rej_row5", "wave_pairs", "wave_pairs_all_rejected_row4", "wave_pairs_clamp_free", "accepted")
+        f32 = lambda v: float(np.array([int(v)], dtype=np.uint32).view(np.float32)[0])
+        return {"steps": [dict(zip(keys, [int(v) for v in out[8 * s:8 * s + 8]])) for s in range(3)],
+                "violations": int(out[28]), "min_gap": f32(out[29]), "min_gap_over_margin": f32(out[30]), "rejected_production": int(out[31])}
 
     def selftest_divide_random(self, log2_triples: int, seed: int, mode: int, guarded: bool = True):
         bad, out = C.c_uint64(0), C.c_uint64(0)
diff --git a/tsar-mvs_amd/csrc/pm_core.h b/tsar-mvs_amd/csrc/pm_core.h
--- a/tsar-mvs_amd/csrc/pm_core.h
+++ b/tsar-mvs_amd/csrc/pm_core.h
@@ -187,7 +187,7 @@
 
 template <int NB, int HR, bool STRICT, bool QUAD, int V = 0, int BLK = PM_BLOCK>
 DEVFN float multiview_cost(const DevScene* __restrict__ sc, const typename TileOf<QUAD>::type* tile, int tw, int own, const float* wts, const PixelRef& pr,
-                           int x, int y, const float4& n4, int& beview, float& ratio) {
+                           int x, int y, const float4& n4, int& beview, float& ratio, bool prune = false, float cost_now = 0.f, bool* pruned_any = nullptr) {
     constexpr bool GEOM = (V & TSAR_V_GEOM) != 0;
     constexpr int VT = V & ~(TSAR_V_GEOM | TSAR_V_REDRAW);
     float best[NB];
@@ -204,8 +204,11 @@
         vi_next = sc->sel[i + 1 < num ? i + 1 : i];
         float c;
         if constexpr ((VT & 1024) != 0) c = view_cost_lut<STRICT, (VT >> 11) & 7, (VT & 131072) != 0 && !STRICT, (VT & 2097152) != 0 && !STRICT>(sc, sc->view[vi], tile, tw, own, wts, pr, x, y, n4);
-        else if constexpr (QUAD && HR == 5 && r5_production_variant(VT))
-            c = view_cost_r5<STRICT, (VT & 128) != 0 && !STRICT, (VT & 8) != 0, (VT & 131072) != 0, (VT & 2097152) != 0, BLK>(sc, sc->view[vi], tile, tw, own, wts, pr, x, y, n4);
+        else if constexpr (QUAD && HR == 5 && r5_production_variant(VT)) {
+            uint32_t pv = 0;
+            c = view_cost_r5<STRICT, (VT & 128) != 0 && !STRICT, (VT & 8) != 0, (VT & 131072) != 0, (VT & 2097152) != 0, BLK>(sc, sc->view[vi], tile, tw, own, wts, pr, x, y, n4, prune, cost_now, &pv);
+            if (prune && pv) *pruned_any = true;
+        }
 #ifdef TSAR_EXPERIMENTS
         else if constexpr (QUAD && HR == 5 && r5_diag_variant(VT))
             c = view_cost_r5<false, true, true, true, true, BLK, (VT & 4194304) ? 1 : 2>(sc, sc->view[vi], tile, tw, own, wts, pr, x, y, n4);
diff --git a/tsar-mvs_amd/csrc/pm_sweep_impl.h b/tsar-mvs_amd/csrc/pm_sweep_impl.h
--- a/tsar-mvs_amd/csrc/pm_sweep_impl.h
+++ b/tsar-mvs_amd/csrc/pm_sweep_impl.h
@@ -189,6 +189,9 @@
     float deltaZ = sc->max_disp / 2.0f;
     const float fb = rf.f * rf.baseline;
     const int n_ref = do_refine ? sc->refine_steps : 0;
+    constexpr bool PRUNE_CAP = !STRICT && QUAD && HR == 5 && NB == 2 && (V & TSAR_V_GEOM) == 0 && (V & 128) != 0 && r5_production_variant(V);
+    bool prune_ok = false;
+    if constexpr (PRUNE_CAP) prune_ok = (do_refine & 2) != 0 && sc->prune != 0 && sc->cost_comb == TSAR_COMB_BEST_N && sc->n_best == 1;
 
     if constexpr (!CMP) {
         if (work) {
@@ -228,7 +231,19 @@
                     deltaZ = deltaZ / 10.0f;
                 }
                 int bv; float rt;
-                const float cost_t = multiview_cost<NB, HR, STRICT, QUAD, V, BLK>(sc, tile, tw, own, wts, pr, x, y, n_t, bv, rt);
+                float cost_t;
+                if constexpr (PRUNE_CAP) {
+                    bool prune = prune_ok && h >= 8 && h - 8 < 2;
+#pragma unroll 1
+                    for (;;) {
+                        bool pruned_any = false;
+                        cost_t = multiview_cost<NB, HR, STRICT, QUAD, V, BLK>(sc, tile, tw, own, wts, pr, x, y, n_t, bv, rt, prune, cost_now, &pruned_any);
+                        if (!prune || !__any(pruned_any && cost_t < cost_now)) break;
+                        prune = false;
+                    }
+                } else {
+                    cost_t = multiview_cost<NB, HR, STRICT, QUAD, V, BLK>(sc, tile, tw, own, wts, pr, x, y, n_t, bv, rt);
+                }
                 if (cost_t < cost_now) {
                     cost_now = cost_t; n_now = n_t; depth_now = depth_t;
                     ratio_w = rt; beview_w = bv; wrote = true;
@@ -348,7 +363,18 @@
             const float* ewts = LUTW ? wts_base : wts_base + etid;
             int bv = -1;
             float rt = 0.f, cost_t = TSAR_MAXCOST;
-            if (go) cost_t = multiview_cost<NB, HR, STRICT, QUAD, V, BLK>(sc, tile, tw, eown, ewts, epr, ex, ey, n_t, bv, rt);
+            if constexpr (PRUNE_CAP) {
+                bool prune = prune_ok && it >= trips && it - trips < 2;
+#pragma unroll 1
+                for (;;) {
+                    bool pruned_any = false;
+                    if (go) cost_t = multiview_cost<NB, HR, STRICT, QUAD, V, BLK>(sc, tile, tw, eown, ewts, epr, ex, ey, n_t, bv, rt, prune, cost_now, &pruned_any);
+                    if (!prune || !__any(go && pruned_any && cost_t < cost_now)) break;
+                    prune = false;
+                }
+            } else {
+                if (go) cost_t = multiview_cost<NB, HR, STRICT, QUAD, V, BLK>(sc, tile, tw, eown, ewts, epr, ex, ey, n_t, bv, rt);
+            }
             if (it < trips) {
                 arms_of_trip(lo, [&](int a, int j, bool has) {
                     const float c = __int_as_float(__builtin_amdgcn_ds_bpermute((j & 63) << 2, __float_as_int(cost_t)));
@@ -423,12 +449,13 @@
             lds += 6 * (size_t)BLK;
         }
     }
+    const int refine_arg = do_refine ? 1 | ((ctx->prune_on && ctx->sweeps_done >= ctx->prune_from) ? 2 : 0) : 0;
     if (lds > 64 * 1024) TSAR_HIP_TRY(ctx, hipFuncSetAttribute((const void*)kern, hipFuncAttributeMaxDynamicSharedMemorySize, (int)lds));
     {
         ScopedKernelTimer tm(ctx, (V & TSAR_V_GEOM) ? "pm_sweep_geom" : "pm_sweep");
         ScopedKernelTimer tm_packed(ctx, packed ? "pm_sweep_packed" : nullptr);
         hipLaunchKernelGGL(kern, dim3(n_tiles), dim3(BLK), lds, ctx->stream, ctx->dscene, colour, same_in.c, same_in.n4, other.c,
-                           other.n4, same_out.c, same_out.n4, ctx->ratio, ctx->beview, stream_id, do_prop, do_refine, tiles_x, n_tiles,
+                           other.n4, same_out.c, same_out.n4, ctx->ratio, ctx->beview, stream_id, do_prop, refine_arg, tiles_x, n_tiles,
                            ctx->cost_consistent ? 1 : 0, strip_width(ctx->strip_w, tiles_x), ctx->final_text, memo);
     }
     TSAR_HIP_TRY(ctx, hipGetLastError());
diff --git a/tsar-mvs_amd/csrc/pm_tap_r5.h b/tsar-mvs_amd/csrc/pm_tap_r5.h
--- a/tsar-mvs_amd/csrc/pm_tap_r5.h
+++ b/tsar-mvs_amd/csrc/pm_tap_r5.h
@@ -1,8 +1,33 @@
 #pragma once
 
-template <bool STRICT, bool ROW, bool D16, bool BUF, bool MIX, int BLK, int DIAG = 0>
+#define PRUNE_VMIN 4.0f
+#define PRUNE_MARGIN_K 6e-5f
+#define PRUNE_MARGIN_MAX 0.03f
+#define PRUNE_SRR_MIN 0.002f
+#define PRUNE_SLACK_R1 0.03f
+#define PRUNE_SLACK_RHS 1.01f
+#define PRUNE_ROWS 12
+DEVFN bool prune_reject(float A, float B, float C, float p0, float p1, float p2, float W, float iw, float Gr, float cost_now, float& margin_out) {
+    const float ip = __builtin_amdgcn_rcpf(p0);
+    const float a = A * ip;
+    const float Sss = B - A * a;
+    const float Srr = p2 - p1 * (p1 * ip);
+    const float Ssr = C - a * p1;
+    const float Wr = W * 1.00001f - p0;
+    const float mmax = (A + Wr * 255.5f) * iw;
+    const float Gs = 1.0f + (mmax * mmax) * W * __builtin_amdgcn_rcpf(Sss);
+    const float margin = PRUNE_MARGIN_K * (Gr + Gs);
+    const float rho = (1.0f - cost_now) - margin;
+    const bool ok = Sss >= PRUNE_VMIN * W && Srr >= PRUNE_SRR_MIN * p2 && margin <= PRUNE_MARGIN_MAX && rho >= 0.0f;
+    const float R1 = Sss - (Ssr * Ssr) * __builtin_amdgcn_rcpf(Srr);
+    const float M = fmaxf(a, 255.0f - a) + 0.5f;
+    margin_out = margin;
+    return ok && (R1 - PRUNE_SLACK_R1 * Sss) > ((1.0f - rho * rho) * PRUNE_SLACK_RHS) * (Sss + Wr * (M * M));
+}
+
+template <bool STRICT, bool ROW, bool D16, bool BUF, bool MIX, int BLK, int DIAG = 0, bool CENSUS = false>
 DEVFN float view_cost_r5(const DevScene* __restrict__ sc, const DevView& vw, const unsigned short* tile, int tw, int own, const float* wts,
-                         const PixelRef& pr, int x, int y, const float4& n4) {
+                         const PixelRef& pr, int x, int y, const float4& n4, bool prune = false, float cost_now = 0.f, uint32_t* pruned = nullptr) {
     static_assert(!(STRICT && ROW), "the row-wise walk changes the summation order: fast mode only");
     static_assert(!MIX || (BUF && !STRICT), "the half-float difference texture serves the fast arithmetic's blend through buffer loads");
     const int w = sc->w, h = sc->h, qp = sc->quad_pitch;
@@ -68,9 +93,11 @@
         asm volatile("" : "+s"(rsrc));
     }
     typedef float f32x2 __attribute__((ext_vector_type(2)));
-    auto line6 = [&](int i, auto clamp_tag, auto unr_tag) {
+    float p0 = 0.f, p1 = 0.f, p2 = 0.f;
+    auto line6 = [&](int i, auto clamp_tag, auto unr_tag, auto prn_tag) {
         constexpr bool CLAMP = decltype(clamp_tag)::value;
         constexpr bool UNR = decltype(unr_tag)::value;
+        constexpr bool PRN = decltype(prn_tag)::value;
         static_assert(!UNR || (ROW && D16), "the unrolled form is written for the row-wise walk with D16 window loads");
         const float xi = (float)((ROW ? y : x) + i);
         const float bx = STRICT ? H[0] * xi : fma_(H[ROW ? 1 : 0], xi, H[2]), by = STRICT ? H[3] * xi : fma_(H[ROW ? 4 : 3], xi, H[5]),
@@ -200,17 +227,55 @@
             sum_src_src = fma_(ws, s, sum_src_src);
             if (STRICT) sum_ref_src = fma_(wt * r, s, sum_ref_src);
             else sum_ref_src = fma_(ws, r, sum_ref_src);
+            if (PRN) {
+                const float wr = wt * r;
+                p0 += wt;
+                p1 += wr;
+                p2 = fma_(wr, r, p2);
+            }
         }
     };
-    if (need_clamp) {
+    bool walked = false;
+    if constexpr (ROW && !STRICT && DIAG == 0) {
+        if (prune) {
+            walked = true;
+            const float W = __builtin_amdgcn_rcpf(pr.inv_wsum);
+            const float Gr = 1.0f + (pr.mean_ref * pr.mean_ref) * __builtin_amdgcn_rcpf(pr.var_ref);
+            const bool can = pr.var_ref >= PRUNE_VMIN;
+            bool out = false;
+            uint32_t seen = 0;
+            float mg_first = 0.f;
+            auto walk = [&](auto clamp_tag) {
 #pragma unroll 1
-        for (int i = -5; i <= 5; i += 2) line6(i, std::true_type(), std::false_type());
+                for (int i = -5; i <= 5; i += 2) {
+                    line6(i, clamp_tag, std::false_type(), std::true_type());
+                    if (CENSUS ? (i >= -1 && i <= 3) : ((PRUNE_ROWS >> ((i + 5) >> 1)) & 1) != 0) {
+                        asm volatile("; partial-window test");
+                        float mg;
+                        const bool rej = prune_reject(sum_src, sum_src_src, sum_ref_src, p0, p1, p2, W, pr.inv_wsum, Gr, cost_now, mg) && can;
+                        if (CENSUS) {
+                            if (rej && !seen) mg_first = mg;
+                            seen |= rej ? 1u << ((i + 1) >> 1) : 0u;
+                        } else if (rej) { out = true; break; }
+                    }
+                }
+            };
+            if (need_clamp) walk(std::true_type());
+            else walk(std::false_type());
+            if (CENSUS) { pruned[0] = seen | (need_clamp ? 0u : 8u); pruned[1] = __float_as_uint(mg_first); }
+            else if (out) { *pruned = 1u; return TSAR_MAXCOST; }
+        }
+    }
+    if (walked) {
+    } else if (need_clamp) {
+#pragma unroll 1
+        for (int i = -5; i <= 5; i += 2) line6(i, std::true_type(), std::false_type(), std::false_type());
     } else if constexpr (MIX) {
 #pragma unroll
-        for (int i = -5; i <= 5; i += 2) line6(i, std::false_type(), std::true_type());
+        for (int i = -5; i <= 5; i += 2) line6(i, std::false_type(), std::true_type(), std::false_type());
     } else {
 #pragma unroll 1
-        for (int i = -5; i <= 5; i += 2) line6(i, std::false_type(), std::false_type());
+        for (int i = -5; i <= 5; i += 2) line6(i, std::false_type(), std::false_type(), std::false_type());
     }
     sum_src *= pr.inv_wsum;
     sum_src_src *= pr.inv_wsum;
diff --git a/tsar-mvs_amd/csrc/selftest_kernels.hip b/tsar-mvs_amd/csrc/selftest_kernels.hip
--- a/tsar-mvs_amd/csrc/selftest_kernels.hip
+++ b/tsar-mvs_amd/csrc/selftest_kernels.hip
@@ -210,3 +210,121 @@
     TSAR_HIP_TRY(ctx, hipGetLastError());
     return TSAR_OK;
 }
+
+__global__ __launch_bounds__(256) void prune_census_kernel(const DevScene* __restrict__ sc, int colour, const float* __restrict__ c, const float4* __restrict__ n4,
+                                                           uint32_t stream_id, int tiles_x, unsigned long long* out) {
+    extern __shared__ __attribute__((aligned(16))) unsigned char lds_raw[];
+    constexpr int BLK = 256, RW = PM_RW, RH = 2 * BLK / RW;
+    const int tw = RW + 10, th = RH + 10;
+    unsigned short* tile = (unsigned short*)lds_raw;
+    float* wts = (float*)(lds_raw + tile_bytes<true>(tw, th)) + threadIdx.x;
+    const int tix = blockIdx.x % tiles_x, tiy = blockIdx.x / tiles_x;
+    const int ty0 = tiy * RH, tx0 = tix * RW;
+    stage_ref_tile<RH, unsigned short, BLK, RW>(sc, tile, tx0, ty0, 5, 5, 0);
+    __syncthreads();
+    const int ly = threadIdx.x >> 4, k = threadIdx.x & 15;
+    const int y = ty0 + ly;
+    const int lx = 2 * k + ((colour + y) & 1);
+    const int x = tx0 + lx;
+    const int w = sc->w, h = sc->h;
+    const bool mine = x < w && y < h;
+    const int p = mine ? y * w + x : 0;
+    const int own = (ly + 5) * tw + lx + 5;
+    PixelRef pr;
+    pr.inv_wsum = 1.f; pr.mean_ref = 0.f; pr.var_ref = 0.f; pr.textured = false;
+    if (mine) pr = hoist_reference<5, unsigned short, BLK>(tile, tw, own, wts, 5, 5);
+    const bool work = mine && pr.textured;
+    float cost_now = work ? c[p] : 0.f;
+    float4 n_now = work ? n4[p] : make_float4(0.f, 0.f, -1.f, 1.f);
+    const DevRef& rf = sc->ref;
+    float vv[3] = {0.f, 0.f, 1.f};
+    float depth_now = 1.f;
+    if (work) { depth_now = plane_depth(rf, n_now, x, y); view_vector(rf, x, y, vv); }
+    float deltaN = 1.0f, deltaZ = sc->max_disp / 2.0f;
+    const float fb = rf.f * rf.baseline;
+    const int n_ref = min(sc->refine_steps, 3);
+    unsigned long long viol = 0, prod = 0;
+    float min_gap = __builtin_inff(), min_rel = __builtin_inff();
+    for (int s = 0; s < n_ref; s++) {
+        float4 n_t = n_now;
+        float depth_t = depth_now;
+        if (work) {
+            const Rand4 rn = philox_uniform4((uint32_t)p, stream_id, (uint32_t)s, sc->seed_lo, sc->seed_hi);
+            const float disp = fb / depth_now;
+            const float minDelta = -fminf(deltaZ, sc->min_disp + disp);
+            const float maxDelta = fminf(deltaZ, sc->max_disp - disp);
+            const float dz = between(rn.u[0], minDelta, maxDelta);
+            const float dispOut = fminf(fmaxf(disp + dz, sc->min_disp), sc->max_disp);
+            depth_t = fb / dispOut;
+            float nt[3];
+            nt[0] = n_now.x + between(rn.u[1], -deltaN, deltaN);
+            nt[1] = n_now.y + between(rn.u[2], -deltaN, deltaN);
+            nt[2] = n_now.z + between(rn.u[3], -deltaN, deltaN);
+            const float inv = 1.0f / sqrtf(dot3(nt, nt));
+            nt[0] *= inv; nt[1] *= inv; nt[2] *= inv;
+            if (dot3(nt, vv) > 0.0f) { nt[0] = -nt[0]; nt[1] = -nt[1]; nt[2] = -nt[2]; }
+            n_t.x = nt[0]; n_t.y = nt[1]; n_t.z = nt[2];
+            n_t.w = plane_offset(rf, nt, x, y, depth_t);
+        }
+        deltaN = deltaN / 4.0f;
+        deltaZ = deltaZ / 10.0f;
+        float cmin = TSAR_MAXCOST;
+        unsigned long long pairs = 0, r3 = 0, r4 = 0, r5 = 0, wv = 0, wv_all = 0, wv_free = 0;
+        for (int i = 0; i < sc->n_sel; i++) {
+            uint32_t pv[2] = {0u, 0u};
+            float cv = TSAR_MAXCOST;
+            if (work) cv = view_cost_r5<false, true, true, false, false, BLK, 0, true>(sc, sc->view[sc->sel[i]], tile, tw, own, wts, pr, x, y, n_t, true, cost_now, pv);
+            cv = fminf(cv, TSAR_MAXCOST);
+            const uint32_t m = work ? pv[0] & 7u : 0u;
+            if (work) {
+                pairs++;
+                r3 += m & 1u; r4 += (m & 3u) ? 1 : 0; r5 += m ? 1 : 0;
+                if (m) {
+                    if (cv < cost_now) viol++;
+                    min_gap = fminf(min_gap, cv - cost_now);
+                    min_rel = fminf(min_rel, (cv - cost_now) / __uint_as_float(pv[1]));
+                    if ((m & 3u) && s < 2) prod++;
+                }
+                cmin = fminf(cmin, cv);
+            }
+            if (__any(work)) {
+                wv++;
+                if (!__any(work && !(m & 3u))) wv_all++;
+                if (__any(pv[0] & 8u)) wv_free++;
+            }
+        }
+        const bool acc = work && cmin < cost_now;
+        if (acc) { cost_now = cmin; n_now = n_t; depth_now = depth_t; }
+        unsigned long long accn = acc ? 1 : 0;
+        for (int o = 32; o; o >>= 1) {
+            pairs += __shfl_xor(pairs, o); r3 += __shfl_xor(r3, o); r4 += __shfl_xor(r4, o); r5 += __shfl_xor(r5, o); accn += __shfl_xor(accn, o);
+        }
+        if ((threadIdx.x & 63) == 0) {
+            unsigned long long* o8 = out + 8 * s;
+            atomicAdd(&o8[0], pairs); atomicAdd(&o8[1], r3); atomicAdd(&o8[2], r4); atomicAdd(&o8[3], r5);
+            atomicAdd(&o8[4], wv); atomicAdd(&o8[5], wv_all); atomicAdd(&o8[6], wv_free); atomicAdd(&o8[7], accn);
+        }
+    }
+    if (viol) atomicAdd(&out[28], viol);
+    if (prod) atomicAdd(&out[31], prod);
+    if (min_gap >= 0.0f && min_gap < __builtin_inff()) atomicMin(&out[29], (unsigned long long)__float_as_uint(min_gap));
+    if (min_rel >= 0.0f && min_rel < __builtin_inff()) atomicMin(&out[30], (unsigned long long)__float_as_uint(min_rel));
+}
+
+int launch_prune_census(tsar_ctx* ctx, int colour, unsigned long long* dout) {
+    const DevScene& hs = ctx->hscene;
+    if (!(hs.use_quad && hs.hrad == 5 && hs.vrad == 5 && ctx->variant == 250 && !(hs.flags & (TSAR_FLAG_STRICT_DIV | TSAR_FLAG_TEX_FILTER_8BIT)))) {
+        ctx->err = "the prune census runs fast mode's box-11 loop on 8-bit imagery (variant 250)";
+        return TSAR_ERR_INVALID;
+    }
+    const int tiles_x = (hs.w + 31) / 32, tiles_y = (hs.h + 15) / 16;
+    const size_t lds = tile_bytes<true>(PM_RW + 10, 16 + 10) + sizeof(float) * 36 * 256;
+    const unsigned long long big = 0x7f800000ull;
+    TSAR_HIP_TRY(ctx, hipMemcpyAsync(dout + 29, &big, 8, hipMemcpyHostToDevice, ctx->stream));
+    TSAR_HIP_TRY(ctx, hipMemcpyAsync(dout + 30, &big, 8, hipMemcpyHostToDevice, ctx->stream));
+    TSAR_HIP_TRY(ctx, hipStreamSynchronize(ctx->stream));
+    hipLaunchKernelGGL(prune_census_kernel, dim3(tiles_x * tiles_y), dim3(256), lds, ctx->stream, ctx->dscene, colour, ctx->buf[0].c, ctx->buf[0].n4,
+                       1u + (uint32_t)ctx->sweeps_done, tiles_x, dout);
+    TSAR_HIP_TRY(ctx, hipGetLastError());
+    return TSAR_OK;
+}
diff --git a/tsar-mvs_amd/csrc/tsar_api.hip b/tsar-mvs_amd/csrc/tsar_api.hip
--- a/tsar-mvs_amd/csrc/tsar_api.hip
+++ b/tsar-mvs_amd/csrc/tsar_api.hip
@@ -184,6 +184,7 @@
     sc.max_disp = sc.ref.f * sc.ref.baseline / ctx->params.depth_min;
     int steps = 0;
     for (float dz = sc.max_disp / 2.0f; dz >= 0.01f; dz = dz / 10.0f) steps++;
+    if (ctx->refine_cap >= 0 && steps > ctx->refine_cap) steps = ctx->refine_cap;
     sc.refine_steps = steps;
 }
 
@@ -199,6 +200,7 @@
     sc.vrad = init_radius ? p.box_vsize / 2 : (p.box_vsize - 1) / 2;
     sc.n_best = p.n_best;
     sc.cost_comb = p.cost_comb;
+    sc.prune = ctx->prune_on ? 1 : 0;
     sc.flags = p.flags;
     sc.seed_lo = (uint32_t)p.seed;
     sc.seed_hi = (uint32_t)(p.seed >> 32);
@@ -246,6 +248,8 @@
     ctx->force_block = num("TSAR_BLOCK", 0);
     ctx->memo_mode = num("TSAR_MEMO", 1);
     ctx->compact_from = num("TSAR_COMPACT_FROM", 6);
+    ctx->prune_on = on("TSAR_PRUNE", true);
+    ctx->prune_from = num("TSAR_PRUNE_FROM", 3);
     ctx->lut_mode = num("TSAR_LUT", 1);
     ctx->ransac_wgs = num("TSAR_RANSAC_WGS", 8);
     ctx->ransac_chain = num("TSAR_RANSAC_CHAIN", 8);
@@ -1226,6 +1230,32 @@
     scratch.release();
     return rc;
 }
+extern "C" int tsar_selftest_refine_steps(tsar_ctx* ctx, int n) {
+    CHECK_CTX(ctx);
+    NEED_VIEWS(ctx);
+    ctx->refine_cap = n;
+    int steps = 0;
+    for (float dz = ctx->hscene.max_disp / 2.0f; dz >= 0.01f; dz = dz / 10.0f) steps++;
+    if (n >= 0 && steps > n) steps = n;
+    ctx->hscene.refine_steps = steps;
+    return upload_scene(ctx);
+}
+extern "C" int tsar_selftest_prune_census(tsar_ctx* ctx, int colour, uint64_t* out32) {
+    CHECK_CTX(ctx);
+    NEED_VIEWS(ctx);
+    NEED_STATE(ctx);
+    if (!out32) return fail(ctx, TSAR_ERR_INVALID, "out32 is NULL");
+    ScratchScope scratch(ctx);
+    unsigned long long* dc = (unsigned long long*)scratch.alloc(32 * sizeof(unsigned long long));
+    if (!dc) { scratch.release(); return fail(ctx, TSAR_ERR_NOMEM, "device allocation failed"); }
+    int rc = TSAR_OK;
+    if (hipMemsetAsync(dc, 0, 256, ctx->stream) != hipSuccess) rc = fail(ctx, TSAR_ERR_HIP, "hipMemsetAsync failed");
+    if (rc == TSAR_OK) rc = launch_prune_census(ctx, colour & 1, dc);
+    if (rc == TSAR_OK && hipMemcpyAsync(out32, dc, 256, hipMemcpyDeviceToHost, ctx->stream) != hipSuccess) rc = fail(ctx, TSAR_ERR_HIP, "hipMemcpyAsync failed");
+    if (hipStreamSynchronize(ctx->stream) != hipSuccess && rc == TSAR_OK) rc = fail(ctx, TSAR_ERR_HIP, "hipStreamSynchronize failed");
+    scratch.release();
+    return rc;
+}
 extern "C" int tsar_selftest_sweep_census(tsar_ctx* ctx, int colour, uint64_t* out8) {
     CHECK_CTX(ctx);
     NEED_VIEWS(ctx);
diff --git a/tsar-mvs_amd/csrc/tsar_dev.h b/tsar-mvs_amd/csrc/tsar_dev.h
--- a/tsar-mvs_amd/csrc/tsar_dev.h
+++ b/tsar-mvs_amd/csrc/tsar_dev.h
@@ -62,6 +62,7 @@
     float geom_back[TSAR_MAX_VIEWS][12];
     float geom_weight, geom_clip, geom_clip_sq;
     int geom_on;
+    int prune;
 };
 
 #define TSAR_V_GEOM 16777216
@@ -116,6 +117,9 @@
     uint32_t memo_valid_from = 1;
     int call_launch = 0;
     int memo_mode = 1;
+    bool prune_on = true;
+    int prune_from = 3;
+    int refine_cap = -1;
     int compact_from = 6;
     std::vector<tsar_camera> cams;
     bool views_u8 = false;
@@ -232,6 +236,7 @@
 int launch_lrdiff(tsar_ctx* ctx);
 int launch_selftest_divide(tsar_ctx* ctx, const float* X, const float* Y, const float* Z, size_t n, float* u, float* v, int ieee);
 int launch_sweep_census(tsar_ctx* ctx, int colour, unsigned long long* dout);
+int launch_prune_census(tsar_ctx* ctx, int colour, unsigned long long* dout);
 int launch_selftest_divide_random(tsar_ctx* ctx, int log2_pairs, uint64_t seed, int mode, int guarded, unsigned long long* dcounts);
 int launch_selftest_sqrt(tsar_ctx* ctx, int mode, uint64_t seed, unsigned long long* dcounts);
 int launch_update_scale(tsar_ctx* ctx);
```

After: 47.55 (median of 6 runs). No clear change (+0.7%).
